# adriente/espm

Measured on AMD Instinct MI355X. Metric: MU iterations/sec, 2048ch x (512*512)px X, k=5 SmoothNMF, higher is better.
Workload: dtype f32; 1 GPU; 2048ch x (512x512)px, k=5, SmoothNMF simplex_H + Laplacian lambda=1, X stored ell, W/H fp32; n=2048, k=5, simplex_H=True, parallelism=single GPU, autotune=True, engine_policy=autotune='auto', as SmoothNMF(max_iter=10000).fit builds it, launch_plan=fused, units handed out dynamically

## Files before the change

### espm_amd/_lib.py

```python
from __future__ import annotations

import ctypes as C
import os

import torch

_HERE = os.path.dirname(os.path.abspath(__file__))
LIB_PATH = os.environ.get("ESPM_MU_LIB", os.path.join(_HERE, "lib", "libespm_mu.so"))

from . import _abi

_HEADER_TEXT = _abi.header_text()
_D = _abi.parse_defines(_HEADER_TEXT)
OK, EINVAL, ENOSOLUTION, EHIP, EUNSUPPORTED = 0, -1, -2, -3, -4
X_F32, X_BF16, X_U8, X_ELL = 0, 1, 2, 3
F64_X_U8, F64_X_BF16, F64_X_F32, F64_X_F64 = (_D["ESPM_F64_X_" + n] for n in ("U8", "BF16", "F32", "F64"))
F64_MAX_K, F64_MAXIT = _D["ESPM_F64_MAX_K"], _D["ESPM_F64_MAXIT"]
F64S_MAX_COUNT, F64S_MAX_N, F64S_WBLOCK = _D["ESPM_F64S_MAX_COUNT"], _D["ESPM_F64S_MAX_N"], _D["ESPM_F64S_WBLOCK"]
SRC_F32, SRC_F64 = 0, 1
LAYOUT_CM, LAYOUT_PM = 0, 1
ABI_VERSION = _D["ESPM_MU_ABI_VERSION"]
XCHG_HANDLE_BYTES = _D["ESPM_XCHG_HANDLE_BYTES"]
ELL_TILE, ELL_PB, ELL_PBITS, ELL_LDS_MAX = _D["ESPM_ELL_TILE"], _D["ESPM_ELL_PB"], _D["ESPM_ELL_PBITS"], _D["ESPM_ELL_LDS_MAX"]
ELL_STREAM_BYTES = _D["ESPM_ELL_STREAM_BYTES"]
ELL_BUCKETS = _D["ESPM_ELL_BUCKETS"]
ELL_HEAVY_MIN, ELL_HEAVY_MAX = _D["ESPM_ELL_HEAVY_MIN"], _D["ESPM_ELL_HEAVY_MAX"]
ELL_UNIT_ROWS, ELL_UNIT_MAX_N, ELL_PAIR_MAX_K = _D["ESPM_ELL_UNIT_ROWS"], _D["ESPM_ELL_UNIT_MAX_N"], _D["ESPM_ELL_PAIR_MAX_K"]
KP, PPAD, NPAD = _D["ESPM_KP"], _D["ESPM_PPAD"], _D["ESPM_NPAD"]
MAX_K = KP
HP_STRIDE, HS_STRIDE, HI_STRIDE = 8 + 2 * KP, 2 * KP, _D["ESPM_HI_STRIDE"]
HS_ROWSUM, HS_MAX = 0, KP
WIDE_MAX_K = 16
WIDEST_MAX_K = 32
TAIL_DEFER, TAIL_RIDE = _D["ESPM_TAIL_DEFER"], _D["ESPM_TAIL_RIDE"]
HI_KLX, HI_REG, HI_LAP, HI_SUMY, HI_BAD, HI_REL_W, HI_REL_H = (_D["ESPM_HI_" + n] for n in ("KLX", "REG", "LAP", "SUMY", "BAD", "REL_W", "REL_H"))

_vp, _i32, _i64, _f32 = C.c_void_p, C.c_int32, C.c_int64, C.c_float


class MUState(C.Structure):
    _fields_ = _abi.parse_struct(_HEADER_TEXT)

    def __init__(self, *args, **kw):
        super().__init__(*args, **kw)
        self.struct_size = C.sizeof(type(self))
        self.abi_version = ABI_VERSION


_SP = C.POINTER(MUState)
SYMBOLS = {
    "espm_mu_version": (C.c_char_p, []),
    "espm_mu_last_error": (C.c_char_p, []),
    "espm_mu_state_size": (C.c_size_t, []),
    "espm_mu_abi_version": (C.c_int, []),
    "espm_mu_state_layout": (C.c_char_p, []),
    "espm_mu_query": (C.c_int, [_SP]),
    "espm_mu_w_update_is_local": (C.c_int, [_SP]),
    "espm_mu_w_update_tail": (C.c_int, [_SP, C.c_int, C.c_int, _vp]),
    "espm_mu_pack_x": (C.c_int, [_vp, C.c_int, C.c_int, _i64, C.c_int, C.c_int, _vp, _vp, C.c_int, C.c_int, C.c_int, C.c_int, C.c_int, _vp]),
    "espm_mu_ell_count": (C.c_int, [_SP, _vp, _vp, _vp, _vp, _vp]),
    "espm_mu_ell_count_hist": (C.c_int, [_SP, _vp, _vp, _vp, _vp, _vp, _vp, _vp]),
    "espm_mu_ell_fill_hist": (C.c_int, [_SP, _vp, _vp, _vp, _vp, _vp, _vp, _vp, _vp, _vp, _vp]),
    "espm_mu_ell_plan": (C.c_int, [_SP, _vp, _vp, _vp, _vp, _vp, _vp, _vp, _vp]),
    "espm_mu_ell_fill": (C.c_int, [_SP, _vp, _vp, _vp, _vp, _vp, _vp, _vp, _vp]),
    "espm_mu_ell_heavy_count": (C.c_int, [_SP, _vp, C.c_int, C.c_int, _i64, _vp, _vp, _vp, _vp]),
    "espm_mu_ell_heavy_fill": (C.c_int, [_SP, _vp, C.c_int, C.c_int, _i64, _vp, _vp, _vp]),
    "espm_mu_hstat": (C.c_int, [_SP, C.c_int, _vp]),
    "espm_mu_build_gw": (C.c_int, [_SP, C.c_int, _vp]),
    "espm_mu_step_h": (C.c_int, [_SP, C.c_int, C.c_int, _vp]),
    "espm_mu_h_finalize": (C.c_int, [_SP, C.c_int, C.c_int, _vp]),
    "espm_mu_loss_only": (C.c_int, [_SP, C.c_int, C.c_int, _vp]),
    "espm_mu_w_accum": (C.c_int, [_SP, _vp]),
    "espm_mu_step_hw": (C.c_int, [_SP, C.c_int, _vp]),
    "espm_mu_fused_applies": (C.c_int, [_SP]),
    "espm_mu_w_reduce": (C.c_int, [_SP, _vp]),
    "espm_mu_w_reduce_finalize": (C.c_int, [_SP, C.c_int, C.c_int, _vp]),
    "espm_mu_w_finish": (C.c_int, [_SP, C.c_int, C.c_int, C.c_int, _vp]),
    "espm_mu_iterate_timed": (C.c_int, [_SP, C.c_int, _vp, _vp, _vp]),
    "espm_mu_iterate": (C.c_int, [_SP, C.c_int, C.c_int, _vp]),
    "espm_mu_shard_record_bytes": (C.c_size_t, [_SP]),
    "espm_mu_shard_pack": (C.c_int, [_SP, C.c_int, _vp, _vp]),
    "espm_mu_shard_combine": (C.c_int, [_SP, _vp, C.c_int, C.c_int, _vp]),
    "espm_mu_shard_combine_finish": (C.c_int, [_SP, _vp, C.c_int, C.c_int, C.c_int, _vp]),
    "espm_mu_w_reduce_finish": (C.c_int, [_SP, C.c_int, C.c_int, C.c_int, _vp]),
    "espm_mu_w_reduce_pack": (C.c_int, [_SP, C.c_int, C.c_int, _vp, _vp]),
    "espm_xchg_create": (C.c_int, [C.c_int, C.c_int, C.c_size_t, C.POINTER(_vp)]),
    "espm_xchg_handle": (C.c_int, [_vp, _vp]),
    "espm_xchg_connect": (C.c_int, [_vp, _vp]),
    "espm_xchg_staging": (_vp, [_vp]),
    "espm_xchg_records": (_vp, [_vp, C.c_int]),
    "espm_xchg_post": (C.c_int, [_vp, C.c_uint32, _vp]),
    "espm_xchg_wait": (C.c_int, [_vp, C.c_uint32, _vp]),
    "espm_xchg_timeouts": (C.c_int, [_vp, C.POINTER(C.c_uint32)]),
    "espm_xchg_set_order": (C.c_int, [_vp, C.c_int]),
    "espm_xchg_order": (C.c_int, [_vp]),
    "espm_xchg_destroy": (C.c_int, [_vp]),
    "espm_mu_shard_exchange_finish": (C.c_int, [_SP, _vp, C.c_uint32, C.c_int, C.c_int, _vp]),
    "espm_mu_iterate_sharded": (C.c_int, [_SP, _vp, C.POINTER(C.c_uint32), C.c_int, C.c_int, _vp]),
    "espm_mu_linesearch_terms": (C.c_int, [_SP, C.c_int, C.c_int, _vp, _vp]),
    "espm_mu_linesearch_terms_sharded": (C.c_int, [_SP, C.c_int, C.c_int, _vp, _vp, _vp, _vp]),
    "espm_surrogate_terms": (C.c_int, [_vp, _vp, C.c_int, C.c_int, C.c_int64, C.c_int, C.c_int, C.c_int, _vp, C.c_int, _vp, _vp]),
    "espm_dichotomy_simplex_acc": (C.c_int, [C.c_double, _vp, _vp, C.c_int, C.c_int, C.c_int, C.c_double, C.c_double, C.c_int, _vp, _vp, _vp]),
    "espm_dichotomy_simplex_pg": (C.c_int, [_vp, C.c_int, C.c_int, C.c_double, C.c_double, C.c_int, _vp, _vp]),
    "espm_mu_l2_step_h": (C.c_int, [_SP, C.c_int, _vp, _vp, C.c_int, _vp]),
    "espm_mu_l2_step_w": (C.c_int, [_SP, C.c_int, _vp, _vp, _vp, C.c_int, _vp]),
    "espm_mu_l2_w_partials": (C.c_int, [_SP, _vp, _vp, C.c_int, _vp]),
    "espm_mu_l2_w_finish": (C.c_int, [_SP, C.c_int, _vp, _vp, _vp]),
    "espm_simplex_root_f32": (C.c_int, [_vp, _vp, C.c_int, C.c_int, C.c_float, C.c_float, C.c_int, C.c_int, _vp, _vp, _vp, _vp]),
    "espm_dichotomy_simplex": (C.c_int, [_vp, _vp, C.c_int, C.c_int, C.c_int, C.c_double, C.c_double, C.c_int, _vp, _vp, _vp]),
    "espm_mu_laplacian": (C.c_int, [_vp, C.c_int, C.c_int, C.c_int, _i64, _vp, _vp]),
    "espm_lu_pl_scratch_bytes": (C.c_size_t, [C.c_int, C.c_int, C.c_int]),
    "espm_lu_pl": (C.c_int, [_vp, C.c_int, C.c_int, C.c_int, _i64, _vp, _vp, C.c_size_t, _vp]),
    "espm_f64_scratch_doubles": (_i64, [C.c_int, C.c_int, C.c_int, _i64]),
    "espm_f64_gw": (C.c_int, [_vp, _vp, C.c_int, C.c_int, C.c_int, C.c_double, _vp, _vp, _vp, _vp]),
    "espm_f64_hstat": (C.c_int, [_vp, C.c_int, C.c_int, C.c_double, _vp, _vp, _vp]),
    "espm_f64_h_pass": (C.c_int, [_vp, C.c_int, C.c_int, C.c_int, C.c_double, _vp, _vp, _vp, _vp, C.c_int, _vp, _vp, C.c_double,
                                  C.c_double, C.c_double, C.c_int, C.c_int, C.c_double, C.c_int, _vp, _vp, _vp, _vp, _vp, _vp, _vp]),
    "espm_f64_bisect": (C.c_int, [_vp, _vp, C.c_int, C.c_int, C.c_double, C.c_double, C.c_int, _vp, _vp, _vp, _vp, _vp]),
    "espm_f64_rel": (C.c_int, [_vp, _vp, _i64, C.c_double, _vp, _vp, _vp]),
    "espm_f64_w_accum": (C.c_int, [_vp, C.c_int, C.c_int, C.c_int, C.c_double, _vp, _vp, C.c_int, C.c_double, _vp, _vp, _vp]),
    "espm_f64_w_finish": (C.c_int, [_vp, _vp, _vp, C.c_int, C.c_int, C.c_int, _vp, _vp, C.c_int, _vp, C.c_int, C.c_double, C.c_double,
                                    C.c_int, _vp, _vp, _vp, _vp]),
    "espm_f64_sparse_scratch_doubles": (_i64, [C.c_int, C.c_int, C.c_int]),
    "espm_f64_sparse_h_pass": (C.c_int, [_vp, _vp, _vp, C.c_int, _vp, C.c_int, C.c_int, C.c_double, _vp, _vp, _vp, _vp, C.c_int, _vp, _vp,
                                         C.c_double, C.c_double, C.c_double, C.c_int, C.c_int, C.c_double, C.c_int, _vp, _vp, _vp, _vp,
                                         _vp, _vp, _vp]),
    "espm_f64_sparse_w_accum": (C.c_int, [_vp, _vp, _vp, _vp, _vp, C.c_int, C.c_int, C.c_double, _vp, _vp, C.c_int, C.c_double, _vp, _vp,
                                          _vp]),
}


class EspmError(RuntimeError):
    """HIP runtime failure or unsupported configuration reported by libespm_mu."""


class LostPeerError(EspmError):
    """A sharded fit's one-shot record exchange gave up waiting for a peer: the iterates since then are not valid
    (MUEngine.history raises it on every rank at the same read-back; the estimator restarts on the collective transport)."""


def _load(path=LIB_PATH):
    if not os.path.exists(path):
        raise ImportError(
            f"{path} is missing: the HIP library is required (no CPU fallback). Build it with "
            "`python -c 'import __graft_entry__ as g; g.build()'` at the repository root.")
    lib = C.CDLL(path)
    for name, (res, args) in SYMBOLS.items():
        fn = getattr(lib, name)
        fn.restype, fn.argtypes = res, args
    theirs, ours = lib.espm_mu_state_layout().decode(), _abi.layout_string(MUState)
    if lib.espm_mu_state_size() != C.sizeof(MUState) or lib.espm_mu_abi_version() != ABI_VERSION or theirs != ours:
        raise ImportError(f"{path} was built from another include/espm_mu.h (ABI {lib.espm_mu_abi_version()} / {lib.espm_mu_state_size()} bytes "
                          f"against {ABI_VERSION} / {C.sizeof(MUState)}): rebuild it with `python -c 'import __graft_entry__ as g; g.build()'`")
    return lib


lib = _load()


def last_error(which=None) -> str:
    return (which or lib).espm_mu_last_error().decode()


def check(rc: int, which=None) -> None:
    if rc == OK:
        return
    msg = last_error(which)
    if rc == ENOSOLUTION:
        raise ValueError(msg)
    if rc == EINVAL:
        raise ValueError(msg)
    if rc == EUNSUPPORTED:
        raise NotImplementedError(msg)
    raise EspmError(msg)


class Variant:

    def __init__(self, handle, kp, min_k, max_k):
        self.lib, self.KP, self.MIN_K, self.MAX_K = handle, kp, min_k, max_k
        self.HP_STRIDE, self.HS_STRIDE, self.HS_MAX = 8 + 2 * kp, 2 * kp, kp

    def check(self, rc):
        check(rc, self.lib)


_narrow = Variant(lib, KP, 1, MAX_K)
_wide = None
_widest = None
WIDE_LIB_PATH = os.environ.get("ESPM_MU_WIDE_LIB", os.path.join(_HERE, "lib", "libespm_mu_wide.so"))
WIDEST_LIB_PATH = os.environ.get("ESPM_MU_WIDEST_LIB", os.path.join(_HERE, "lib", "libespm_mu_wide32.so"))


def variant(k) -> Variant:
    global _wide, _widest
    if k <= MAX_K:
        return _narrow
    if k > WIDEST_MAX_K:
        raise NotImplementedError(f"n_components = {k}: the kernels are built for 1..{WIDEST_MAX_K} components")
    if k <= WIDE_MAX_K:
        if _wide is None:
            _wide = Variant(_load(WIDE_LIB_PATH), 16, MAX_K + 1, WIDE_MAX_K)
        return _wide
    if _widest is None:
        _widest = Variant(_load(WIDEST_LIB_PATH), 32, WIDE_MAX_K + 1, WIDEST_MAX_K)
    return _widest
```

### espm_amd/csrc/mu_api.hip

```cpp
#include <vector>
#include <stdarg.h>
#include <stdio.h>

#include "mu_common.hpp"
#include "mu_xchg.hpp"

namespace espm {

static thread_local char g_err[512] = "";

int set_error(int code, const char* fmt, ...) {
  va_list ap;
  va_start(ap, fmt);
  vsnprintf(g_err, sizeof(g_err), fmt, ap);
  va_end(ap);
  return code;
}

int check_hip(hipError_t e, const char* what) {
  if (e == hipSuccess) return ESPM_OK;
  return set_error(ESPM_EHIP, "%s: %s", what, hipGetErrorString(e));
}

static int roundup(int v, int m) { return (v + m - 1) / m * m; }

#define ESPM_MU_STATE_FIELDS(F) \
  F(struct_size) F(abi_version) F(n) F(m) F(k) F(p) F(nx) F(ny) F(n_pad) F(p_pad) F(x_dtype) F(tile_px) F(nblk_w) \
  F(x_tile) F(n_cm) F(h_variant) F(p_total) F(simplex_h) F(simplex_w) F(grid_mode) F(compute_loss) F(lambda_l) \
  F(sigma_l) F(eps_reg) F(log_shift) F(dicotomy_tol) F(rel_tol) F(xscale) F(gw_floor) F(x_cm) F(x_pm) F(g) \
  F(colsum_g) F(w) F(gw_s) F(colsum_gw) F(gw_a) F(gw_p) F(h) F(h_t) F(mu) F(fixed_h) F(fixed_w) F(simplex_rows) \
  F(halo_top) F(halo_bot) F(hpart) F(hstat) F(a_slab) F(a) F(w_scratch) F(hist) F(hist_len) F(cur) F(it) F(ell_h) \
  F(ell_h_off) F(ell_klc) F(ell_w) F(ell_w_off) F(chan_perm) F(ell_cbits) F(n_cg) F(pix_perm) F(g_t) F(breg_sr_px) \
  F(breg_sr_ch) F(h_rule) F(pg_gamma_w) F(pg_q) F(ell_fill_px) F(ell_fill_num) F(ell_fill_n) F(tail_mode) F(no_fused) \
  F(ell_pb) F(ell_stream) F(ell_hv_n) F(ell_hv_npx) F(ell_hv_ngrp) F(ell_hv_px) F(ell_hv_px_off) F(ell_hv_pm) F(ell_hv_klc) F(ell_hv_kl) \
  F(ell_hv_grp) F(ell_hv_grp_off) F(ell_hv_wm)

static int check_abi(const espm_mu_state* st) {
  ESPM_REQUIRE(st != nullptr, "state is NULL");
  ESPM_REQUIRE(st->struct_size == (uint32_t)sizeof(espm_mu_state) && st->abi_version == (uint32_t)ESPM_MU_ABI_VERSION,
               "espm_mu_state of %u bytes, ABI %u handed to a library built for %zu bytes, ABI %d: the binding's copy of the layout has drifted",
               st->struct_size, st->abi_version, sizeof(espm_mu_state), ESPM_MU_ABI_VERSION);
  return ESPM_OK;
}

static int check_state(const espm_mu_state* st) {
  if (int rc = check_abi(st)) return rc;
  ESPM_REQUIRE(st->n >= 1 && st->p >= 1, "n=%d, p=%d must be >= 1", st->n, st->p);
  if (st->k < ESPM_MIN_K || st->k > ESPM_MAX_K)
    return set_error(ESPM_EUNSUPPORTED, "k=%d: this build supports %d..%d components", st->k, ESPM_MIN_K, ESPM_MAX_K);
  ESPM_REQUIRE(st->n_pad == roundup(st->n, ESPM_NPAD) && st->p_pad == roundup(st->p, ESPM_PPAD),
               "n_pad/p_pad (%d, %d) do not match n, p (%d, %d); call espm_mu_query", st->n_pad, st->p_pad, st->n,
               st->p);
  ESPM_REQUIRE(st->x_dtype >= ESPM_X_F32 && st->x_dtype <= ESPM_X_ELL, "bad x_dtype %d", st->x_dtype);
  if (st->x_dtype == ESPM_X_ELL) {
    ESPM_REQUIRE(st->ell_h && st->ell_h_off && st->ell_klc && st->ell_w && st->ell_w_off && st->chan_perm && st->pix_perm,
                 "the sparse count store needs ell_h, ell_h_off, ell_klc, ell_w, ell_w_off, chan_perm and pix_perm");
    ESPM_REQUIRE((st->tile_px == 64 || st->tile_px == 128 || st->tile_px == 256 || st->tile_px == ESPM_ELL_TILE) &&
                     st->ell_pb == 2 * st->tile_px && st->nblk_w == (st->p + st->ell_pb - 1) / st->ell_pb &&
                     st->n_cg == (st->n + 63) / 64 && st->h_variant == 0,
                 "sparse count store: tile_px must be 64..%d, ell_pb 2 tile_px, nblk_w ceil(p / ell_pb), n_cg ceil(n / 64); call espm_mu_query",
                 ESPM_ELL_TILE);
  }
  ESPM_REQUIRE(st->ell_stream == 0 || (st->ell_stream == 1 && st->x_dtype == ESPM_X_ELL), "ell_stream=%d: 0, or 1 with the sparse store", st->ell_stream);
  ESPM_REQUIRE(st->ell_fill_n >= 0 && (st->ell_fill_n == 0 || (st->x_dtype == ESPM_X_ELL && st->ell_fill_px && st->ell_fill_num)),
               "ell_fill_n=%d needs the sparse store, ell_fill_px and ell_fill_num", st->ell_fill_n);
  ESPM_REQUIRE(st->ell_hv_n >= 0 && (st->ell_hv_n == 0 || (st->x_dtype == ESPM_X_ELL && st->h_rule == 0 && !st->breg_sr_px && st->ell_hv_npx >= 1 &&
                                                          st->ell_hv_npx <= st->ell_hv_n && st->ell_hv_ngrp >= 1 && st->ell_hv_ngrp <= st->ell_hv_n &&
                                                          st->ell_hv_px && st->ell_hv_px_off && st->ell_hv_pm && st->ell_hv_klc && st->ell_hv_kl &&
                                                          st->ell_hv_grp && st->ell_hv_grp_off && st->ell_hv_wm && st->ell_fill_num)),
               "ell_hv_n=%d needs the sparse store with the default H rule, 1 <= ell_hv_npx, ell_hv_ngrp <= ell_hv_n, every ell_hv_* array and "
               "ell_fill_num", st->ell_hv_n);
  ESPM_REQUIRE(st->grid_mode == 0 || (st->nx >= 1 && st->ny >= 1 && st->nx * st->ny == st->p),
               "grid %d x %d does not match p=%d", st->nx, st->ny, st->p);
  ESPM_REQUIRE(st->xscale > 0.f, "xscale must be positive");
  ESPM_REQUIRE(st->n_cm == roundup(st->n, ESPM_NCM), "n_cm must be roundup(n, %d)", ESPM_NCM);
  ESPM_REQUIRE((st->breg_sr_px == nullptr) == (st->breg_sr_ch == nullptr), "breg_sr_px and breg_sr_ch come together");
  ESPM_REQUIRE(!st->breg_sr_px || (st->m == 0 && !st->simplex_w && st->n <= 4096),
               "the Bregman variant is built for G = identity without simplex_W (and n <= 4096)");
  ESPM_REQUIRE(st->h_rule == 0 || ((st->h_rule == 1 || st->h_rule == 2) && !st->breg_sr_px), "h_rule must be 0, 1 or 2 (1, 2 not with the Bregman variant)");
  ESPM_REQUIRE(!(st->pg_gamma_w > 0.f) || (!st->simplex_w && !st->breg_sr_px && (st->m == 0 || (long)st->m * st->k <= 8192)),
               "the projected-gradient W step has no simplex over W (updates.py:368-369), no Bregman variant, and needs M k <= 8192 with a dictionary");
  ESPM_REQUIRE(st->h_variant == 0, "h_variant %d is not built (the matrix-core H-step was retired, DESIGN.md)", st->h_variant);
  ESPM_REQUIRE(st->x_tile >= 64 && ESPM_PPAD % st->x_tile == 0 && st->x_tile % st->tile_px == 0,
               "x_tile=%d must divide %d and be a multiple of tile_px=%d", st->x_tile, ESPM_PPAD, st->tile_px);
  ESPM_REQUIRE(st->m >= 0, "m must be >= 0");
  ESPM_REQUIRE(st->m == 0 || (st->g && st->colsum_g), "m=%d needs g and colsum_g", st->m);
  if (st->log_shift > 0.f && st->simplex_h && (double)st->k * (double)st->log_shift >= 1.0)
    return set_error(ESPM_ENOSOLUTION, "No solution exists! (k * log_shift >= 1)");
  return ESPM_OK;
}

static int nblk_h(const espm_mu_state* st) { return (st->p + st->tile_px - 1) / st->tile_px; }

static int ell_pre_h(const espm_mu_state* st, int src, hipStream_t s) {
  const int ld = st->ell_fill_n + (st->ell_hv_n > 0 ? st->ell_hv_npx : 0);
  if (st->ell_fill_n > 0)
    if (int rc = launch_ell_fill_num(st->gw_s, st->h[src], st->ell_fill_px, st->ell_fill_n, st->n, st->k, st->p_pad, st->log_shift,
                                     st->ell_fill_num, s, ld))
      return rc;
  return st->ell_hv_n > 0 ? launch_ell_hv_h(st, src, ld, s) : ESPM_OK;
}

static int ell_post(const espm_mu_state* st, int hnew, bool w, bool loss, hipStream_t s) {
  if (st->ell_hv_n <= 0) return ESPM_OK;
  if (hnew >= 0) return launch_ell_hv_post(st, st->h[hnew], (size_t)st->p_pad, 1, w, loss, s);
  return launch_ell_hv_post(st, st->h_t, 1, ESPM_KP, w, loss, s);
}

static bool fused_ok(const espm_mu_state* st) {
  return ESPM_MIN_K <= 8 && st->x_dtype == ESPM_X_ELL && st->h_rule == 0 && st->no_fused != 1 &&
         (st->ell_pb >= ESPM_FUSED_MIN_PB || st->nblk_w >= ESPM_FUSED_MIN_BLOCKS || st->no_fused == 3) &&
         fused_ell_lds_bytes(st->n_pad, st->k, st->ell_pb) <= ESPM_ELL_LDS_MAX;
}
static HStepArgs fused_h_args(const espm_mu_state* st, int src) {
  HStepArgs a = make_h_args(st, src, 1);
  a.rec_nb = nblk_h(st);
  return a;
}

}

using namespace espm;

extern "C" {

const char* espm_mu_version(void) { return "espm_mu 0.3 (gfx950)"; }
const char* espm_mu_last_error(void) { return g_err; }

size_t espm_mu_state_size(void) { return sizeof(espm_mu_state); }
int espm_mu_abi_version(void) { return ESPM_MU_ABI_VERSION; }

const char* espm_mu_state_layout(void) {
  static char text[4096];
  static bool done = false;
  if (!done) {
    size_t len = 0;
#define F(name)                                                                                                      \
  len += (size_t)snprintf(text + len, sizeof(text) - len, #name ":%zu:%zu;", offsetof(espm_mu_state, name), \
                          sizeof(((espm_mu_state*)nullptr)->name));
    ESPM_MU_STATE_FIELDS(F)
#undef F
    done = true;
  }
  return text;
}

int espm_mu_query(espm_mu_state* st) {
  if (int rc = check_abi(st)) return rc;
  ESPM_REQUIRE(st->n >= 1 && st->p >= 1, "n=%d, p=%d must be >= 1", st->n, st->p);
  st->n_pad = roundup(st->n, ESPM_NPAD);
  st->p_pad = roundup(st->p, ESPM_PPAD);
  int cus = 256;
  int dev = 0;
  hipDeviceProp_t prop;
  if (hipGetDevice(&dev) == hipSuccess && hipGetDeviceProperties(&prop, dev) == hipSuccess &&
      prop.multiProcessorCount > 0)
    cus = prop.multiProcessorCount;
  const int big = 256;
  st->tile_px = (ESPM_KP <= 16 && (st->p + big - 1) / big >= 2 * cus) ? big : 128;
  st->x_tile = st->tile_px;
  st->n_cm = roundup(st->n, ESPM_NCM);
  st->h_variant = 0;
  st->n_cg = (st->n + 63) / 64;
  st->ell_pb = 0;
  if (st->x_dtype == ESPM_X_ELL) {
    st->tile_px = ESPM_ELL_TILE;
    while (st->tile_px > 64 && (st->p + st->tile_px - 1) / st->tile_px < 2 * cus) st->tile_px /= 2;
    st->x_tile = st->tile_px;
    st->ell_pb = 2 * st->tile_px;
    st->nblk_w = (st->p + st->ell_pb - 1) / st->ell_pb;
    st->ell_cbits = 1;
    while ((1 << st->ell_cbits) < st->n) ++st->ell_cbits;
    if (st->ell_cbits > 14) return set_error(ESPM_EUNSUPPORTED, "sparse count store: n=%d needs more than 14 index bits", st->n);
    return ESPM_OK;
  }
  const int ychunks = (st->x_dtype != ESPM_X_F32 && ESPM_MIN_K <= 8) ? (st->n_pad + 2047) / 2048 : (st->n_pad + 1023) / 1024;
  int target = (2 * cus + ychunks - 1) / ychunks;
  int by_px = (st->p + 15) / 16;
  int nb = target < by_px ? target : by_px;
  if (nb < 1) nb = 1;
  const int ppb = (st->p + nb - 1) / nb;
  st->nblk_w = (st->p + ppb - 1) / ppb;
  return ESPM_OK;
}

int espm_mu_pack_x(const void* src, int src_dtype, int src_layout, int64_t ld, int n, int p, void* x_cm, void* x_pm,
                   int x_dtype, int n_pad, int p_pad, int x_tile, int n_cm, espm_stream_t stream) {
  ESPM_REQUIRE(src && x_pm, "pack_x: NULL pointer");
  ESPM_REQUIRE(n >= 1 && p >= 1 && n_pad == roundup(n, ESPM_NPAD) && p_pad == roundup(p, ESPM_PPAD),
               "pack_x: bad shape n=%d p=%d n_pad=%d p_pad=%d", n, p, n_pad, p_pad);
  ESPM_REQUIRE(src_dtype == ESPM_SRC_F32 || src_dtype == ESPM_SRC_F64, "pack_x: bad src_dtype %d", src_dtype);
  ESPM_REQUIRE(src_layout == ESPM_LAYOUT_CM || src_layout == ESPM_LAYOUT_PM, "pack_x: bad layout %d", src_layout);
  ESPM_REQUIRE(ld >= (src_layout == ESPM_LAYOUT_CM ? p : n), "pack_x: leading dimension too small");
  ESPM_REQUIRE(x_tile >= 64 && ESPM_PPAD % x_tile == 0, "pack_x: x_tile %d must divide %d", x_tile, ESPM_PPAD);
  ESPM_REQUIRE(n_cm == roundup(n, ESPM_NCM), "pack_x: n_cm must be roundup(n, %d)", ESPM_NCM);
  return launch_pack_x(src, src_dtype, src_layout, ld, n, p, x_cm, x_pm, x_dtype, n_pad, p_pad, x_tile, n_cm,
                       static_cast<hipStream_t>(stream));
}

static int check_ell_geometry(const espm_mu_state* st) {
  if (int rc = check_abi(st)) return rc;
  ESPM_REQUIRE(st->x_dtype == ESPM_X_ELL && st->n >= 1 && st->p >= 1 && st->n_pad == roundup(st->n, ESPM_NPAD) &&
                   st->p_pad == roundup(st->p, ESPM_PPAD) && st->n_cg == (st->n + 63) / 64 &&
                   st->ell_pb == 2 * st->tile_px && st->nblk_w == (st->p + st->ell_pb - 1) / st->ell_pb && st->ell_cbits >= 1 &&
                   st->ell_cbits <= 14 && (1 << st->ell_cbits) >= st->n &&
                   (st->tile_px == 64 || st->tile_px == 128 || st->tile_px == 256 || st->tile_px == ESPM_ELL_TILE),
               "sparse store builder: set x_dtype = ESPM_X_ELL and call espm_mu_query first");
  return ESPM_OK;
}

int espm_mu_ell_count_hist(const espm_mu_state* st, const void* x_pm_u8, int32_t* cnt_px, int32_t* cnt_bc, float* ell_klc, uint8_t* bkt_px,
                           uint8_t* bkt_bc, espm_stream_t stream) {
  if (int rc = check_ell_geometry(st)) return rc;
  ESPM_REQUIRE(x_pm_u8 && cnt_px && cnt_bc && ell_klc, "ell_count: NULL pointer");
  ESPM_REQUIRE((bkt_px == nullptr) == (bkt_bc == nullptr), "ell_count: the two histograms come together");
  return launch_ell_count(static_cast<const uint8_t*>(x_pm_u8), st->n, st->n_pad, st->p, st->p_pad, st->ell_cbits, st->n_cg,
                          st->nblk_w, st->ell_pb, cnt_px, cnt_bc, ell_klc, static_cast<hipStream_t>(stream), bkt_px, bkt_bc);
}

int espm_mu_ell_count(const espm_mu_state* st, const void* x_pm_u8, int32_t* cnt_px, int32_t* cnt_bc, float* ell_klc,
                      espm_stream_t stream) {
  return espm_mu_ell_count_hist(st, x_pm_u8, cnt_px, cnt_bc, ell_klc, nullptr, nullptr, stream);
}

int espm_mu_ell_plan(const espm_mu_state* st, const int32_t* cnt_px, const int32_t* cnt_bc, int32_t* chan_perm,
                     int32_t* pix_perm, int32_t* ell_h_off, int32_t* ell_w_off, int64_t* rows, espm_stream_t stream) {
  if (int rc = check_ell_geometry(st)) return rc;
  ESPM_REQUIRE(cnt_px && cnt_bc && chan_perm && pix_perm && ell_h_off && ell_w_off && rows, "ell_plan: NULL pointer");
  return launch_ell_plan(cnt_px, cnt_bc, st->n, st->n_cg, st->nblk_w, st->p_pad, st->tile_px, chan_perm, pix_perm, ell_h_off,
                         ell_w_off, reinterpret_cast<long long*>(rows), static_cast<hipStream_t>(stream));
}

int espm_mu_ell_fill(const espm_mu_state* st, const void* x_pm_u8, const int32_t* chan_perm, const int32_t* pix_perm,
                     const int32_t* ell_h_off, const int32_t* ell_w_off, uint32_t* ell_h, uint32_t* ell_w,
                     espm_stream_t stream) {
  return espm_mu_ell_fill_hist(st, x_pm_u8, chan_perm, pix_perm, ell_h_off, ell_w_off, ell_h, ell_w, nullptr, nullptr, stream);
}

int espm_mu_ell_fill_hist(const espm_mu_state* st, const void* x_pm_u8, const int32_t* chan_perm, const int32_t* pix_perm,
                          const int32_t* ell_h_off, const int32_t* ell_w_off, uint32_t* ell_h, uint32_t* ell_w, const uint8_t* bkt_px,
                          const uint8_t* bkt_bc, espm_stream_t stream) {
  if (int rc = check_ell_geometry(st)) return rc;
  ESPM_REQUIRE((bkt_px == nullptr) == (bkt_bc == nullptr), "ell_fill: the two histograms come together");
  ESPM_REQUIRE(x_pm_u8 && chan_perm && pix_perm && ell_h_off && ell_w_off && ell_h && ell_w, "ell_fill: NULL pointer");
  ESPM_REQUIRE(!st->x_cm || st->n_cm == roundup(st->n, ESPM_NCM), "ell_fill: x_cm is set but n_cm=%d is not n rounded up to %d", st->n_cm, ESPM_NCM);
  return launch_ell_fill(static_cast<const uint8_t*>(x_pm_u8), st->n, st->n_pad, st->p, st->p_pad, st->ell_cbits, st->n_cg,
                         st->nblk_w, st->tile_px, st->ell_pb, chan_perm, pix_perm, ell_h_off, ell_w_off, ell_h, ell_w,
                         static_cast<hipStream_t>(stream), static_cast<const uint8_t*>(st->x_cm), st->n_cm, bkt_px, bkt_bc);
}

int espm_mu_ell_heavy_count(const espm_mu_state* st, const void* x, int src_dtype, int src_layout, int64_t ld, uint8_t* x_pm_u8,
                            uint8_t* x_cm_u8, int32_t* cnt_px, espm_stream_t stream) {
  if (int rc = check_ell_geometry(st)) return rc;
  ESPM_REQUIRE(x && x_pm_u8 && cnt_px, "ell_heavy_count: NULL pointer");
  ESPM_REQUIRE(src_dtype == ESPM_SRC_F32 || src_dtype == ESPM_SRC_F64, "ell_heavy_count: bad src_dtype %d", src_dtype);
  ESPM_REQUIRE(src_layout == ESPM_LAYOUT_CM || src_layout == ESPM_LAYOUT_PM, "ell_heavy_count: bad layout %d", src_layout);
  ESPM_REQUIRE(ld >= (src_layout == ESPM_LAYOUT_CM ? st->p : st->n), "ell_heavy_count: ld=%lld too small", (long long)ld);
  ESPM_REQUIRE(!x_cm_u8 || st->n_cm == roundup(st->n, ESPM_NCM), "ell_heavy_count: x_cm is set but n_cm=%d is not n rounded up to %d", st->n_cm, ESPM_NCM);
  return launch_ell_hv_count(x, src_dtype, src_layout, ld, st->n, st->p, st->n_pad, st->n_cm, x_pm_u8, x_cm_u8, cnt_px,
                             static_cast<hipStream_t>(stream));
}

int espm_mu_ell_heavy_fill(const espm_mu_state* st, const void* x, int src_dtype, int src_layout, int64_t ld, const int32_t* px_off,
                           int32_t* hv_pm, espm_stream_t stream) {
  if (int rc = check_ell_geometry(st)) return rc;
  ESPM_REQUIRE(x && px_off && hv_pm, "ell_heavy_fill: NULL pointer");
  ESPM_REQUIRE(src_dtype == ESPM_SRC_F32 || src_dtype == ESPM_SRC_F64, "ell_heavy_fill: bad src_dtype %d", src_dtype);
  ESPM_REQUIRE(src_layout == ESPM_LAYOUT_CM || src_layout == ESPM_LAYOUT_PM, "ell_heavy_fill: bad layout %d", src_layout);
  ESPM_REQUIRE(ld >= (src_layout == ESPM_LAYOUT_CM ? st->p : st->n), "ell_heavy_fill: ld=%lld too small", (long long)ld);
  return launch_ell_hv_fill(x, src_dtype, src_layout, ld, st->n, st->p, px_off, hv_pm, static_cast<hipStream_t>(stream));
}

int espm_mu_hstat(const espm_mu_state* st, int which, espm_stream_t stream) {
  if (int rc = check_state(st)) return rc;
  ESPM_REQUIRE(which == 0 || which == 1, "which must be 0/1");
  return launch_hstat(st->h[which], st->k, st->p, st->p_pad, st->hstat[which], static_cast<hipStream_t>(stream));
}

static bool w_update_is_local(const espm_mu_state* st) {
  return st->m == 0 && !st->simplex_w && st->n >= 64 && st->w_scratch != nullptr;
}
static bool w_simplex_split(const espm_mu_state* st) {
  return st->m == 0 && st->simplex_w && !st->simplex_rows && !st->breg_sr_ch && !(st->pg_gamma_w > 0.f) && st->n >= 64 &&
         st->w_scratch != nullptr && st->n_pad % 32 == 0 && st->no_fused != 1;
}
static double* simplex_bparts(const espm_mu_state* st) {
  return reinterpret_cast<double*>(st->w_scratch) + 3 * (size_t)st->k * ((st->n_pad + 31) / 32);
}
static int w_simplex_reduce_update(const espm_mu_state* st, int src, int slot, const HFinalizeArgs* fin, WTailArgs* defer_tail, hipStream_t s);

static WFinishArgs finish_args(const espm_mu_state* st, int src, int hsrc, int slot, int update_w) {
  WFinishArgs a;
  a.g = st->m > 0 ? st->g : nullptr;
  a.g_t = st->m > 0 ? st->g_t : nullptr;
  a.colsum_g = st->colsum_g;
  a.w_old = st->w[src];
  a.w_new = update_w ? st->w[1 - src] : st->w[src];
  a.a = st->a;
  a.hstat = st->hstat[hsrc];
  a.fixed_w = st->fixed_w;
  a.simplex_rows = st->simplex_rows;
  a.scratch = st->w_scratch;
  a.breg_sr = st->breg_sr_ch;
  a.pg_gamma_w = st->pg_gamma_w;
  a.pg_q = (st->pg_q && st->pg_gamma_w > 0.f && slot >= 0) ? st->pg_q + 2 * (size_t)slot + 1 : nullptr;
  a.gw_s = st->gw_s;
  a.colsum_gw = st->colsum_gw;
  a.gw_a = nullptr;
  a.gw_p = nullptr;
  a.n_cm = st->n_cm;
  a.hist_slot = (slot >= 0 && st->hist) ? st->hist + (size_t)slot * ESPM_HI_STRIDE : nullptr;
  a.n = st->n;
  a.m = st->m;
  a.k = st->k;
  a.n_pad = st->n_pad;
  a.simplex_w = st->simplex_w;
  a.update_w = update_w;
  a.log_shift = st->log_shift;
  a.tol = ESPM_W_DICOTOMY_TOL;
  a.rel_tol = st->rel_tol;
  a.xscale = st->xscale;
  a.gw_floor = st->gw_floor;
  return a;
}

static int w_simplex_reduce_update(const espm_mu_state* st, int src, int slot, const HFinalizeArgs* fin, WTailArgs* defer_tail, hipStream_t s) {
  if (st->log_shift > 0.f && (double)st->n * (double)st->log_shift >= 1.0)
    return set_error(ESPM_ENOSOLUTION, "No solution exists! (rows * log_shift >= 1)");
  double* bparts = simplex_bparts(st);
  if (int rc = launch_w_reduce(st->a_slab, st->a, st->nblk_w, st->k * st->n_pad, fin, s, st->w[src], bparts, st->n, st->k, st->n_pad)) return rc;
  return launch_w_simplex_update(finish_args(st, src, 1 - src, slot + 1, 1), st->a, bparts, (double)ESPM_W_DICOTOMY_TOL, s, defer_tail);
}

int espm_mu_build_gw(const espm_mu_state* st, int which, espm_stream_t stream) {
  if (int rc = check_state(st)) return rc;
  ESPM_REQUIRE(which == 0 || which == 1, "which must be 0/1");
  return launch_w_finish(finish_args(st, which, 0, -1, 0), static_cast<hipStream_t>(stream));
}

int espm_mu_step_h(const espm_mu_state* st, int src, int write_h, espm_stream_t stream) {
  if (int rc = check_state(st)) return rc;
  ESPM_REQUIRE(src == 0 || src == 1, "src must be 0/1");
  if (st->x_dtype == ESPM_X_ELL) {
    HStepArgs a = make_h_args(st, src, write_h);
    if (st->tail_mode & ESPM_TAIL_RIDE) {
      ESPM_REQUIRE(st->it >= 1 && (w_update_is_local(st) || w_simplex_split(st)), "tail_mode: no local W update produced state %d", st->it);
      a.tail = make_w_tail_args(finish_args(st, 1 - src, src, st->it, 1));
      a.cs_parts = a.tail.parts;
      a.cs_nbk = a.tail.nbk;
      a.tail_on = 1;
    }
    if (int rc = ell_pre_h(st, src, static_cast<hipStream_t>(stream))) return rc;
    if (int rc = launch_h_ell(a, nblk_h(st), static_cast<hipStream_t>(stream))) return rc;
    return ell_post(st, -1, false, true, static_cast<hipStream_t>(stream));
  }
  return dispatch_h_step(make_h_args(st, src, write_h), st->x_dtype, st->tile_px, nblk_h(st),
                         static_cast<hipStream_t>(stream));
}

static HFinalizeArgs finalize_args(const espm_mu_state* st, int src, int slot, bool write_hstat) {
  HFinalizeArgs a;
  a.hpart = st->hpart;
  a.colsum_gw = st->colsum_gw;
  a.hstat_in = st->hstat[src];
  a.hstat_out = write_hstat ? st->hstat[1 - src] : nullptr;
  a.hist_slot = st->hist + (size_t)slot * ESPM_HI_STRIDE;
  a.nblk = nblk_h(st);
  a.k = st->k;
  a.compute_loss = st->compute_loss;
  a.have_prev = st->it > 0;
  a.xscale = st->xscale;
  a.pg_q = (st->pg_q && st->h_rule == 2 && write_hstat) ? st->pg_q + 2 * (size_t)slot : nullptr;
  return a;
}

int espm_mu_h_finalize(const espm_mu_state* st, int src, int slot, espm_stream_t stream) {
  if (int rc = check_state(st)) return rc;
  ESPM_REQUIRE(src == 0 || src == 1, "src must be 0/1");
  ESPM_REQUIRE(slot >= 0 && slot < st->hist_len, "history slot %d outside [0, %d)", slot, st->hist_len);
  return launch_h_finalize(finalize_args(st, src, slot, true), static_cast<hipStream_t>(stream));
}

static int h_finalize_loss_only(const espm_mu_state* st, int src, int slot, hipStream_t stream) {
  return launch_h_finalize(finalize_args(st, src, slot, false), stream);
}

int espm_mu_loss_only(const espm_mu_state* st, int src, int slot, espm_stream_t stream) {
  if (int rc = check_state(st)) return rc;
  ESPM_REQUIRE(slot >= 0 && slot < st->hist_len, "history slot %d outside [0, %d)", slot, st->hist_len);
  if (int rc = espm_mu_step_h(st, src, 0, stream)) return rc;
  return h_finalize_loss_only(st, src, slot, static_cast<hipStream_t>(stream));
}

int espm_mu_w_accum(const espm_mu_state* st, espm_stream_t stream) {
  if (int rc = check_state(st)) return rc;
  ESPM_REQUIRE(st->nblk_w >= 1, "nblk_w must be >= 1");
  if (st->x_dtype == ESPM_X_ELL) {
    if (int rc = launch_w_ell(make_w_args(st), st->k, st->nblk_w, static_cast<hipStream_t>(stream))) return rc;
    return ell_post(st, -1, true, false, static_cast<hipStream_t>(stream));
  }
  return dispatch_w_accum(make_w_args(st), st->k, st->x_dtype, st->nblk_w, static_cast<hipStream_t>(stream));
}

int espm_mu_fused_applies(const espm_mu_state* st) {
  if (check_state(st)) return 0;
  return fused_ok(st) ? 1 : 0;
}

int espm_mu_step_hw(const espm_mu_state* st, int src, espm_stream_t stream) {
  if (int rc = check_state(st)) return rc;
  ESPM_REQUIRE(src == 0 || src == 1, "src must be 0/1");
  if (!fused_ok(st)) {
    if (int rc = espm_mu_step_h(st, src, 1, stream)) return rc;
    return espm_mu_w_accum(st, stream);
  }
  hipStream_t s = static_cast<hipStream_t>(stream);
  HStepArgs a = fused_h_args(st, src);
  if (st->tail_mode & ESPM_TAIL_RIDE) {
    ESPM_REQUIRE(st->it >= 1 && (w_update_is_local(st) || w_simplex_split(st)), "tail_mode: no local W update produced state %d", st->it);
    a.tail = make_w_tail_args(finish_args(st, 1 - src, src, st->it, 1));
    a.cs_parts = a.tail.parts;
    a.cs_nbk = a.tail.nbk;
    a.tail_on = 1;
  }
  if (int rc = ell_pre_h(st, src, s)) return rc;
  if (int rc = launch_fused_ell(a, make_w_args(st), st->nblk_w, s, st->no_fused == 2, st->ell_stream)) return rc;
  return ell_post(st, 1 - src, true, true, s);
}

int espm_mu_w_reduce(const espm_mu_state* st, espm_stream_t stream) {
  if (int rc = check_state(st)) return rc;
  return launch_w_reduce(st->a_slab, st->a, st->nblk_w, st->k * st->n_pad, nullptr, static_cast<hipStream_t>(stream));
}

int espm_mu_w_reduce_finalize(const espm_mu_state* st, int src, int slot, espm_stream_t stream) {
  if (int rc = check_state(st)) return rc;
  ESPM_REQUIRE(src == 0 || src == 1, "src must be 0/1");
  ESPM_REQUIRE(slot >= 0 && slot < st->hist_len, "history slot %d outside [0, %d)", slot, st->hist_len);
  const HFinalizeArgs fin = finalize_args(st, src, slot, true);
  return launch_w_reduce(st->a_slab, st->a, st->nblk_w, st->k * st->n_pad, &fin, static_cast<hipStream_t>(stream));
}

int espm_mu_w_finish(const espm_mu_state* st, int src, int hsrc, int slot, espm_stream_t stream) {
  if (int rc = check_state(st)) return rc;
  ESPM_REQUIRE((src == 0 || src == 1) && (hsrc == 0 || hsrc == 1), "src/hsrc must be 0/1");
  ESPM_REQUIRE(slot < st->hist_len, "history slot %d outside [0, %d)", slot, st->hist_len);
  if (st->simplex_w && st->log_shift > 0.f) {
    const double rows = st->m > 0 ? st->m : st->n;
    if (!st->simplex_rows && rows * (double)st->log_shift >= 1.0)
      return set_error(ESPM_ENOSOLUTION, "No solution exists! (rows * log_shift >= 1)");
  }
  return launch_w_finish(finish_args(st, src, hsrc, slot, 1), static_cast<hipStream_t>(stream));
}

int espm_mu_w_reduce_finish(const espm_mu_state* st, int src, int slot, int with_finalize, espm_stream_t stream) {
  if (int rc = check_state(st)) return rc;
  ESPM_REQUIRE(src == 0 || src == 1, "src must be 0/1");
  ESPM_REQUIRE(slot >= 0 && slot + 1 < st->hist_len, "history slot %d + 1 outside [0, %d)", slot, st->hist_len);
  hipStream_t s = static_cast<hipStream_t>(stream);
  const HFinalizeArgs fin = finalize_args(st, src, slot, true);
  WTailArgs left_out;
  if (w_update_is_local(st)) {
    return launch_w_reduce_update(finish_args(st, src, 1 - src, slot + 1, 1), st->a_slab, (size_t)st->k * st->n_pad * sizeof(float),
                                  st->nblk_w, st->a, with_finalize ? st->hpart : nullptr, nblk_h(st), with_finalize ? nullptr : st->hstat[1 - src],
                                  0, nullptr, with_finalize ? &fin : nullptr, s,
                                  (st->tail_mode & ESPM_TAIL_DEFER) ? &left_out : nullptr);
  }
  if (w_simplex_split(st))
    return w_simplex_reduce_update(st, src, slot, with_finalize ? &fin : nullptr, (st->tail_mode & ESPM_TAIL_DEFER) ? &left_out : nullptr, s);
  if (int rc = launch_w_reduce(st->a_slab, st->a, st->nblk_w, st->k * st->n_pad, with_finalize ? &fin : nullptr, s)) return rc;
  return espm_mu_w_finish(st, src, 1 - src, slot + 1, stream);
}

int espm_mu_shard_combine_finish(const espm_mu_state* st, const void* records, int world, int src, int slot,
                                 espm_stream_t stream) {
  if (int rc = check_state(st)) return rc;
  ESPM_REQUIRE(records && world >= 1 && (src == 0 || src == 1), "shard_combine_finish: bad arguments");
  ESPM_REQUIRE(slot >= 0 && slot + 1 < st->hist_len, "history slot %d + 1 outside [0, %d)", slot, st->hist_len);
  WTailArgs left_out;
  if (w_update_is_local(st)) {
    return launch_w_reduce_update(finish_args(st, src, 1 - src, slot + 1, 1), records, espm_mu_shard_record_bytes(st), world, st->a,
                                  nullptr, 0, nullptr, (size_t)st->k * st->n_pad * sizeof(float), st->hstat[1 - src], nullptr,
                                  static_cast<hipStream_t>(stream), (st->tail_mode & ESPM_TAIL_DEFER) ? &left_out : nullptr);
  }
  if (w_simplex_split(st)) {
    if (st->log_shift > 0.f && (double)st->n * (double)st->log_shift >= 1.0)
      return set_error(ESPM_ENOSOLUTION, "No solution exists! (rows * log_shift >= 1)");
    double* bparts = simplex_bparts(st);
    if (int rc = launch_shard_combine(records, world, espm_mu_shard_record_bytes(st), st->k * st->n_pad, st->a, st->hstat[1 - src],
                                      static_cast<hipStream_t>(stream), st->w[src], bparts, st->n, st->k, st->n_pad))
      return rc;
    return launch_w_simplex_update(finish_args(st, src, 1 - src, slot + 1, 1), st->a, bparts, (double)ESPM_W_DICOTOMY_TOL,
                                   static_cast<hipStream_t>(stream), (st->tail_mode & ESPM_TAIL_DEFER) ? &left_out : nullptr);
  }
  if (int rc = espm_mu_shard_combine(st, records, world, 1 - src, stream)) return rc;
  return espm_mu_w_finish(st, src, 1 - src, slot + 1, stream);
}

int espm_mu_w_update_is_local(const espm_mu_state* st) {
  if (check_state(st)) return 0;
  return w_update_is_local(st) ? 1 : 0;
}

int espm_mu_w_update_tail(const espm_mu_state* st, int src, int slot, espm_stream_t stream) {
  if (int rc = check_state(st)) return rc;
  ESPM_REQUIRE((src == 0 || src == 1) && slot >= 0 && slot + 1 < st->hist_len && (w_update_is_local(st) || w_simplex_split(st)), "w_update_tail: bad arguments");
  return launch_w_update_tail(make_w_tail_args(finish_args(st, src, 1 - src, slot + 1, 1)), static_cast<hipStream_t>(stream));
}

static int iterate_impl(espm_mu_state* st, int n_iter, int final_loss, espm_stream_t stream, hipEvent_t* ev);

int espm_mu_iterate(espm_mu_state* st, int n_iter, int final_loss, espm_stream_t stream) { return iterate_impl(st, n_iter, final_loss, stream, nullptr); }

int espm_mu_iterate_timed(espm_mu_state* st, int n_iter, float* first_ms, float* rest_ms, espm_stream_t stream) {
  if (int rc = check_state(st)) return rc;
  ESPM_REQUIRE(n_iter >= 1 && n_iter <= 4096 && first_ms && rest_ms, "iterate_timed: 1..4096 iterations, two host arrays of that length");
  hipStream_t s = static_cast<hipStream_t>(stream);
  std::vector<hipEvent_t> ev((size_t)3 * n_iter, nullptr);
  int rc = ESPM_OK;
  for (size_t i = 0; i < ev.size() && !rc; ++i) rc = check_hip(hipEventCreate(&ev[i]), "iterate_timed: event");
  if (!rc) rc = iterate_impl(st, n_iter, 0, stream, ev.data());
  if (!rc) rc = check_hip(hipStreamSynchronize(s), "iterate_timed: synchronize");
  for (int i = 0; i < n_iter && !rc; ++i) {
    rc = check_hip(hipEventElapsedTime(first_ms + i, ev[3 * i], ev[3 * i + 1]), "iterate_timed: elapsed");
    if (!rc) rc = check_hip(hipEventElapsedTime(rest_ms + i, ev[3 * i + 1], ev[3 * i + 2]), "iterate_timed: elapsed");
  }
  for (hipEvent_t e : ev)
    if (e) (void)hipEventDestroy(e);
  return rc;
}

static int iterate_impl(espm_mu_state* st, int n_iter, int final_loss, espm_stream_t stream, hipEvent_t* ev) {
  if (int rc = check_state(st)) return rc;
  ESPM_REQUIRE(n_iter >= 0, "n_iter must be >= 0");
  ESPM_REQUIRE(st->it + n_iter < st->hist_len, "history too short: it=%d + %d >= %d", st->it, n_iter, st->hist_len);
  hipStream_t s = static_cast<hipStream_t>(stream);
  const bool split = w_simplex_split(st);
  const bool defer = st->x_dtype == ESPM_X_ELL && (w_update_is_local(st) || split) && !(st->pg_q && st->pg_gamma_w > 0.f);
  const bool fused = fused_ok(st);
  bool pending = false;
  WTailArgs tail;
  for (int i = 0; i < n_iter; ++i) {
    const int cur = st->cur, slot = st->it;
    int rc;
    if (defer) {
      HStepArgs a = fused ? fused_h_args(st, cur) : make_h_args(st, cur, 1);
      if ((rc = ell_pre_h(st, cur, s))) return rc;
      if (pending) {
        a.cs_parts = tail.parts;
        a.cs_nbk = tail.nbk;
        a.tail_on = 1;
        a.tail = tail;
      }
      if (ev && (rc = check_hip(hipEventRecord(ev[3 * i], s), "iterate_timed: record"))) return rc;
      if (fused) {
        if ((rc = launch_fused_ell(a, make_w_args(st), st->nblk_w, s, st->no_fused == 2, st->ell_stream))) return rc;
        if ((rc = ell_post(st, 1 - cur, true, true, s))) return rc;
        if (ev && (rc = check_hip(hipEventRecord(ev[3 * i + 1], s), "iterate_timed: record"))) return rc;
      } else {
        if ((rc = launch_h_ell(a, nblk_h(st), s))) return rc;
        if ((rc = ell_post(st, -1, false, true, s))) return rc;
        if (ev && (rc = check_hip(hipEventRecord(ev[3 * i + 1], s), "iterate_timed: record"))) return rc;
        if ((rc = espm_mu_w_accum(st, stream))) return rc;
      }
      const HFinalizeArgs fin = finalize_args(st, cur, slot, true);
      if (split) {
        if ((rc = w_simplex_reduce_update(st, cur, slot, &fin, &tail, s))) return rc;
      } else if ((rc = launch_w_reduce_update(finish_args(st, cur, 1 - cur, slot + 1, 1), st->a_slab, (size_t)st->k * st->n_pad * sizeof(float),
                                              st->nblk_w, st->a, st->hpart, nblk_h(st), nullptr, 0, nullptr, &fin, s, &tail))) {
        return rc;
      }
      if (ev && (rc = check_hip(hipEventRecord(ev[3 * i + 2], s), "iterate_timed: record"))) return rc;
      pending = true;
    } else {
      if (ev && (rc = check_hip(hipEventRecord(ev[3 * i], s), "iterate_timed: record"))) return rc;
      if ((rc = espm_mu_step_hw(st, cur, stream))) return rc;
      if (ev && (rc = check_hip(hipEventRecord(ev[3 * i + 1], s), "iterate_timed: record"))) return rc;
      if ((rc = espm_mu_w_reduce_finish(st, cur, slot, 1, stream))) return rc;
      if (ev && (rc = check_hip(hipEventRecord(ev[3 * i + 2], s), "iterate_timed: record"))) return rc;
    }
    st->cur = 1 - cur;
    st->it = slot + 1;
  }
  if (pending)
    if (int rc = launch_w_update_tail(tail, s)) return rc;
  if (final_loss) return espm_mu_loss_only(st, st->cur, st->it, stream);
  return ESPM_OK;
}

int espm_mu_shard_exchange_finish(const espm_mu_state* st, espm_xchg* x, uint32_t seq, int src, int slot, espm_stream_t stream) {
  if (int rc = check_state(st)) return rc;
  ESPM_REQUIRE(x && (src == 0 || src == 1), "shard_exchange_finish: bad arguments");
  ESPM_REQUIRE(slot >= 0 && slot + 1 < st->hist_len, "history slot %d + 1 outside [0, %d)", slot, st->hist_len);
  ESPM_REQUIRE(x->record_bytes == espm_mu_shard_record_bytes(st), "shard_exchange_finish: the exchange was created for records of %zu bytes, the state packs %zu",
               x->record_bytes, espm_mu_shard_record_bytes(st));
  if (!w_update_is_local(st) && st->no_fused != 1) {
    const WFinishArgs f = finish_args(st, src, 1 - src, slot + 1, 1);
    if (w_gsplit_applies(f)) {
      HFinalizeArgs fin = finalize_args(st, src, slot, true);
      double* local = reinterpret_cast<double*>(x->mailbox + (size_t)(seq & 1u) * x->world * x->record_bytes + (size_t)x->rank * x->record_bytes +
                                                (size_t)st->k * st->n_pad * 4);
      fin.hstat_out = local;
      if (int rc = launch_w_reduce(st->a_slab, st->a, st->nblk_w, st->k * st->n_pad, &fin, static_cast<hipStream_t>(stream))) return rc;
      const int with_halo_g = st->grid_mode && st->lambda_l != 0.f;
      return launch_w_gxchg_update(f, x, seq, local, st->hstat[1 - src], st->h[1 - src], st->nx, st->ny, st->p_pad, with_halo_g,
                                   static_cast<hipStream_t>(stream));
    }
  }
  if (w_simplex_split(st) && nblk_h(st) > 0) {
    if (st->log_shift > 0.f && (double)st->n * (double)st->log_shift >= 1.0)
      return set_error(ESPM_ENOSOLUTION, "No solution exists! (rows * log_shift >= 1)");
    const HFinalizeArgs fin = finalize_args(st, src, slot, true);
    WTailArgs left_out;
    const int with_halo = st->grid_mode && st->lambda_l != 0.f;
    double* bparts = simplex_bparts(st);
    if (int rc = launch_w_exchange_update(finish_args(st, src, 1 - src, slot + 1, 1), st->a_slab, (size_t)st->k * st->n_pad * sizeof(float), st->nblk_w,
                                          st->a, st->hstat[1 - src], fin, x, seq, st->h[1 - src], st->nx, st->ny, st->p_pad, with_halo,
                                          static_cast<hipStream_t>(stream), nullptr, bparts))
      return rc;
    return launch_w_simplex_update(finish_args(st, src, 1 - src, slot + 1, 1), st->a, bparts, (double)ESPM_W_DICOTOMY_TOL,
                                   static_cast<hipStream_t>(stream), (st->tail_mode & ESPM_TAIL_DEFER) ? &left_out : nullptr);
  }
  if (!w_update_is_local(st) || st->no_fused == 1) {
    if (int rc = espm_mu_w_reduce_pack(st, src, slot, x->staging, stream)) return rc;
    if (int rc = espm_xchg_post(x, seq, stream)) return rc;
    if (int rc = espm_xchg_wait(x, seq, stream)) return rc;
    return espm_mu_shard_combine_finish(st, espm_xchg_records(x, (int)(seq & 1u)), x->world, src, slot, stream);
  }
  const HFinalizeArgs fin = finalize_args(st, src, slot, true);
  WTailArgs left_out;
  const int with_halo = st->grid_mode && st->lambda_l != 0.f;
  return launch_w_exchange_update(finish_args(st, src, 1 - src, slot + 1, 1), st->a_slab, (size_t)st->k * st->n_pad * sizeof(float), st->nblk_w,
                                  st->a, st->hstat[1 - src], fin, x, seq, st->h[1 - src], st->nx, st->ny, st->p_pad, with_halo,
                                  static_cast<hipStream_t>(stream), (st->tail_mode & ESPM_TAIL_DEFER) ? &left_out : nullptr);
}

int espm_mu_iterate_sharded(espm_mu_state* st, espm_xchg* x, uint32_t* seq, int n_iter, int final_loss, espm_stream_t stream) {
  if (int rc = check_state(st)) return rc;
  ESPM_REQUIRE(x && seq && n_iter >= 0, "iterate_sharded: bad arguments");
  ESPM_REQUIRE(st->it + n_iter < st->hist_len, "history too short: it=%d + %d >= %d", st->it, n_iter, st->hist_len);
  ESPM_REQUIRE(x->record_bytes == espm_mu_shard_record_bytes(st), "iterate_sharded: the exchange was created for records of %zu bytes, the state packs %zu",
               x->record_bytes, espm_mu_shard_record_bytes(st));
  const bool defer = st->x_dtype == ESPM_X_ELL && (w_update_is_local(st) || w_simplex_split(st)) && !(st->pg_q && st->pg_gamma_w > 0.f);
  const bool with_halo = st->grid_mode && st->lambda_l != 0.f;
  const size_t off_top = (size_t)st->k * st->n_pad * 4 + ESPM_HS_STRIDE * 8, off_bot = off_top + (size_t)st->k * (st->ny > 0 ? st->ny : 0) * 4;
  bool pending = (st->tail_mode & ESPM_TAIL_RIDE) != 0;
  int rc = ESPM_OK;
  for (int i = 0; i < n_iter && !rc; ++i) {
    const int cur = st->cur, slot = st->it;
    st->tail_mode = pending ? ESPM_TAIL_RIDE : 0;
    rc = espm_mu_step_hw(st, cur, stream);
    st->tail_mode = 0;
    const uint32_t s = ++*seq;
    const unsigned char* recs = static_cast<const unsigned char*>(espm_xchg_records(x, (int)(s & 1u)));
    st->tail_mode = defer ? ESPM_TAIL_DEFER : 0;
    if (!rc) rc = espm_mu_shard_exchange_finish(st, x, s, cur, slot, stream);
    st->tail_mode = 0;
    pending = defer;
    if (with_halo) {
      st->halo_top = x->rank > 0 ? reinterpret_cast<const float*>(recs + (size_t)(x->rank - 1) * x->record_bytes + off_bot) : nullptr;
      st->halo_bot = x->rank < x->world - 1 ? reinterpret_cast<const float*>(recs + (size_t)(x->rank + 1) * x->record_bytes + off_top) : nullptr;
    }
    st->cur = 1 - cur;
    st->it = slot + 1;
  }
  if (rc) return rc;
  if (pending)
    if ((rc = espm_mu_w_update_tail(st, 1 - st->cur, st->it - 1, stream))) return rc;
  if (final_loss) return espm_mu_loss_only(st, st->cur, st->it, stream);
  return ESPM_OK;
}

int espm_dichotomy_simplex(const double* num, const double* den, int k, int p, int den_cols, double log_shift,
                           double tol, int maxit, double* nu_out, int32_t* status_out, espm_stream_t stream) {
  ESPM_REQUIRE(num && den && nu_out && status_out, "dichotomy: NULL pointer");
  ESPM_REQUIRE(k >= 1 && p >= 1 && (den_cols == 1 || den_cols == p), "dichotomy: bad shape k=%d p=%d den_cols=%d", k,
               p, den_cols);
  if (log_shift > 0 && (double)k * log_shift >= 1.0) return set_error(ESPM_ENOSOLUTION, "No solution exists!");
  return launch_dichotomy(num, den, k, p, den_cols, log_shift, tol, maxit, nu_out, status_out,
                          static_cast<hipStream_t>(stream));
}

int espm_simplex_root_f32(const float* num, const float* den, int k, int p, float log_shift, float tol, int maxit, int fast_exit,
                          float* delta_out, float* e_out, int32_t* status_out, espm_stream_t stream) {
  ESPM_REQUIRE(num && den && delta_out && e_out && status_out, "simplex_root_f32: NULL pointer");
  ESPM_REQUIRE(k >= ESPM_MIN_K && k <= ESPM_MAX_K && p >= 1, "simplex_root_f32: bad shape k=%d p=%d (this library: %d..%d components)", k, p, ESPM_MIN_K, ESPM_MAX_K);
  if (log_shift > 0 && (double)k * log_shift >= 1.0) return set_error(ESPM_ENOSOLUTION, "No solution exists!");
  return launch_simplex_root_f32(num, den, k, p, log_shift, tol, maxit, fast_exit, delta_out, e_out, status_out, static_cast<hipStream_t>(stream));
}

int espm_surrogate_terms(const float* h_old, const float* h_new, int k, int p, int64_t ld, int nx, int ny, int grid_mode, double* part,
                         int part_doubles, double* out, espm_stream_t stream) {
  ESPM_REQUIRE(h_old && h_new && part && out && k >= 1 && k <= ESPM_KP && p >= 1 && ld >= p, "surrogate_terms: bad arguments");
  ESPM_REQUIRE(!grid_mode || (nx >= 1 && ny >= 1 && (int64_t)nx * ny == p), "surrogate_terms: grid %d x %d does not match p=%d", nx, ny, p);
  ESPM_REQUIRE(part_doubles >= (4 + ESPM_KP) * ((p + 511) / 512), "surrogate_terms: scratch of %d doubles is too small", part_doubles);
  return launch_linesearch_terms(h_old, h_new, k, p, (int)ld, nx, ny, grid_mode, nullptr, nullptr, nullptr, nullptr, part, out,
                                 static_cast<hipStream_t>(stream));
}

// ... 121 lines not shown
```

### espm_amd/csrc/mu_common.hpp

```cpp
#pragma once
#include <hip/hip_runtime.h>
#include <stdint.h>

#include "espm_mu.h"

namespace espm {

constexpr int KP = ESPM_KP;
static_assert(KP == 8 || KP == 16 || KP == 32, "ESPM_KP: 8, 16 or 32");
static_assert(ESPM_MIN_K >= 1 && ESPM_MAX_K <= KP && ESPM_MIN_K <= ESPM_MAX_K, "ESPM_MIN_K .. ESPM_MAX_K must fit the stride");

#if ESPM_MIN_K <= 8
#define ESPM_K_CASES(X) X(1) X(2) X(3) X(4) X(5) X(6) X(7) X(8)
#elif ESPM_MIN_K <= 16
#define ESPM_K_CASES(X) X(9) X(10) X(11) X(12) X(13) X(14) X(15) X(16)
#else
#define ESPM_K_CASES(X) X(17) X(18) X(19) X(20) X(21) X(22) X(23) X(24) X(25) X(26) X(27) X(28) X(29) X(30) X(31) X(32)
#endif

__device__ __forceinline__ void store_row_kp(float* dst, const float (&row)[KP]) {
#pragma unroll
  for (int q = 0; q < KP / 4; ++q)
    reinterpret_cast<float4*>(dst)[q] = make_float4(row[4 * q], row[4 * q + 1], row[4 * q + 2], row[4 * q + 3]);
}
// ... 391 lines not shown
      y[u] = i < mk ? a.w_old[i] : 1.f;
    }
#pragma unroll
    for (int u = 0; u < 8; ++u) rel = fmaxf(rel, fabsf(x[u] - y[u]) / (x[u] + shift));
  }
  double r1[1] = {(double)rel};
  block_reduce<1, 0>(r1, scratch);
  if (tid == 0) a.hist_slot[ESPM_HI_REL_W] = r1[0];
}

template <typename T>
__device__ __forceinline__ T fast_rcp(T x);
template <>
__device__ __forceinline__ float fast_rcp<float>(float x) { return __builtin_amdgcn_rcpf(x); }
template <>
__device__ __forceinline__ double fast_rcp<double>(double x) { return 1.0 / x; }

template <typename T, int K>
__device__ __forceinline__ bool simplex_root(const T (&num)[K], const T (&den)[K], int k, T eps, T tol,
                                             int maxit, T& delta, T (&e)[K], bool fast_exit = false) {
  T nmax = 0, dmin_all = INFINITY, dstar = INFINITY, nsum = 0;
  bool ok = true;
#pragma unroll
  for (int i = 0; i < K; ++i) {
    if (i < k) {
      ok = ok && (num[i] >= 0) && (den[i] >= 0);
      if (num[i] > 0) dstar = fmin(dstar, den[i]);
      nmax = fmax(nmax, num[i]);
      dmin_all = fmin(dmin_all, den[i]);
      nsum += num[i];
    }
  }
  ok = ok && (nsum > 0) && (nsum < (T)INFINITY);
  if (!ok) {
    delta = 0;
#pragma unroll
    for (int i = 0; i < K; ++i) e[i] = i < k ? den[i] : (T)1;
    return false;
  }
  T lo = 0;
#pragma unroll
  for (int i = 0; i < K; ++i) {
    e[i] = i < k ? den[i] - dstar : (T)1;
    if (i < k && num[i] > 0) lo = fmax(lo, num[i] / 2 - e[i]);
  }
  T hi = (T)(2 * k) * nmax + (dstar - dmin_all);
  T x = fmax(lo, fmin(dstar, hi)), dxold = hi - lo;
  const bool fast = fast_exit && (T)(4 * K) * eps <= (T)1e-3 * tol;
  for (int it = 0; it < maxit; ++it) {
    T f = -1, fp = 0, fpp = 0;
#pragma unroll
    for (int i = 0; i < K; ++i) {
      if (i < k) {
        T inv = fast_rcp<T>(x + e[i]);
        T t = num[i] > 0 ? num[i] * inv : (T)0;
        if (t > eps) {
          const T u = t * inv;
          f += t;
          fp -= u;
          if (fast_exit) fpp += u * inv;
        } else {
          f += eps;
        }
      }
    }
    if (fabs(f) <= tol) break;
    if (f > 0) lo = x; else hi = x;
    T dx = fp < 0 ? -f * fast_rcp<T>(fp) : (T)0;
    T xn = x + dx;
    bool newton = true;
    if (!(fp < 0) || !(xn > lo && xn < hi) || fabs(dx) > (T)0.5 * fabs(dxold)) {
      dx = (hi - lo) / 2;
      xn = lo + dx;
      newton = false;
    }
    dxold = dx;
    if (xn == x) break;
    x = xn;
    if (fast && newton && (T)4 * f * f * fpp <= tol * fp * fp) break;
  }
  delta = x;
  return true;
}

__device__ __forceinline__ float hq_root(float s, float q) {
  const float r = __builtin_amdgcn_sqrtf(fmaf(s, s, q));
  return s >= 0.f ? q * __builtin_amdgcn_rcpf(r + s) : r - s;
}
template <int K>
__device__ __forceinline__ bool simplex_root_hq(float a, const float (&b)[K], const float (&c)[K], float eps, int maxit, float& nu) {
  bool ok = a > 0.f;
  float bmax = -INFINITY, bsum = 0.f;
#pragma unroll
  for (int i = 0; i < K; ++i) {
    ok = ok && c[i] >= 0.f && b[i] == b[i];
    bmax = fmaxf(bmax, b[i] * b[i] * __builtin_amdgcn_rcpf(a) + 2.f * a + 2.f * (b[i] + c[i]));
    bsum += b[i];
  }
  nu = 0.f;
  if (!ok) return false;
  float hi = (float)K * bmax * 1.5f + 1e-3f;
  float lo = -(2.f * a + bsum) * (1.1f / (float)K) - 1e-3f;
  const float target = 2.f * a, floor_g = 2.f * a * eps;
  float x = fminf(fmaxf(0.f, lo), hi), dxold = hi - lo;
  for (int it = 0; it < maxit; ++it) {
    float f = -target, fp = 0.f;
#pragma unroll
    for (int i = 0; i < K; ++i) {
      const float s = b[i] + x, q = 4.f * a * c[i];
      const float r = __builtin_amdgcn_sqrtf(fmaf(s, s, q));
      const float g = s >= 0.f ? q * __builtin_amdgcn_rcpf(r + s) : r - s;
      if (g > floor_g) {
        f += g;
        fp -= g * __builtin_amdgcn_rcpf(r);
      } else {
        f += floor_g;
      }
    }
    if (fabsf(f) <= 4e-7f * target) break;
    if (f > 0.f) lo = x; else hi = x;
    float dx = fp < 0.f ? -f * __builtin_amdgcn_rcpf(fp) : 0.f;
    float xn = x + dx;
    if (!(fp < 0.f) || !(xn > lo && xn < hi) || fabsf(dx) > 0.5f * fabsf(dxold)) {
      dx = (hi - lo) * 0.5f;
      xn = lo + dx;
    }
    dxold = dx;
    if (xn == x) break;
    x = xn;
  }
  nu = x;
  return true;
}

__device__ __forceinline__ float stencil_hl(const float* hrow, const float* halo_top, const float* halo_bot,
                                            int q, int nx, int ny, float hc) {
  const int i = q / ny, j = q - i * ny;
  float acc = 0.f;
  int deg = 0;
  if (j > 0) { acc += hrow[q - 1]; ++deg; }
  if (j < ny - 1) { acc += hrow[q + 1]; ++deg; }
  if (i > 0) { acc += hrow[q - ny]; ++deg; }
  else if (halo_top) { acc += halo_top[j]; ++deg; }
  if (i < nx - 1) { acc += hrow[q + ny]; ++deg; }
  else if (halo_bot) { acc += halo_bot[j]; ++deg; }
  return (float)deg * hc - acc;
}

struct HStepArgs {
  const void* x_cm;
  const void* x_pm;
  int mfma;
  const float* gw_s;
  const double* colsum_gw;
  const float* h_in;
  float* h_out;
  float* h_t;
  const float* mu;
  const float* fixed_h;
  const float* halo_top;
  const float* halo_bot;
  const double* hstat_in;
  double* hpart;
  int n, k, p, nx, ny, p_pad;
  int x_tile;
  int n_cm;
  const void* gw_a;
  const float* gw_p;
  int simplex_h, grid_mode, compute_loss, write_h;
  int have_prev;
  float lambda_l, sigma_l, eps_reg, log_shift, tol, xscale, rel_tol;
  double inv_count;
  const uint32_t* ell;
  const int32_t* ell_off;
  const float* ell_klc;
  const int32_t* ell_pix;
  int ell_bits, n_pad;
  int ell_tp;
  const float* l2_m;
  const float* breg_sr;
  int h_rule;
  const float* fill_num;
  int fill_n;
  const double* cs_parts;
  int cs_nbk, cs_lds_off, tail_on;
  WTailArgs tail;
  int rec_nb;
};
struct HFinalizeArgs {
  const double* hpart;
  const double* colsum_gw;
  const double* hstat_in;
  double* hstat_out;
  double* hist_slot;
  int nblk, k, compute_loss, have_prev;
  float xscale;
  double* pg_q;
};
__host__ __device__ inline int ell_pbits(int pb) {
  int b = 6;
  while ((1 << b) < pb) ++b;
  return b;
}
struct WAccumArgs {
  const void* x_pm;
  const void* x_cm;
  int x_tile, n_cm, p_pad, mfma;
  const float* gw_s;
  const float* h_t;
  float* a_slab;
  int n_pad, p, ppb;
  const uint32_t* ell;
  const int32_t* ell_off;
  const int32_t* chan_perm;
  int n_cg;
  int pb, pbits;
  int l2;
};
struct WFinishArgs {
  const float* g;
  const float* g_t;
  const float* colsum_g;
  const float* w_old;
  float* w_new;
  const float* a;
  const double* hstat;
  const float* fixed_w;
  const int32_t* simplex_rows;
  float* scratch;
  const float* breg_sr;
  float pg_gamma_w;
  double* pg_q;
  float* gw_s;
  double* colsum_gw;
  void* gw_a;
  float* gw_p;
  double* hist_slot;
  int n, m, k, n_pad, n_cm, simplex_w, update_w;
  float log_shift, tol, rel_tol, xscale, gw_floor;
};


__device__ __forceinline__ void h_finalize_body(const HFinalizeArgs& a, double* scratch) {
  constexpr int NV = ESPM_HP_NSCALAR + 2 * KP + 1;
  constexpr int V_RELH = 4 + KP, V_MAX = 5 + KP, V_RELW = 5 + 2 * KP;
  double v[NV];
#pragma unroll
  for (int i = 0; i < NV; ++i) v[i] = 0.0;
  v[V_RELW] = -1.0;
  const size_t nb = a.nblk;
  constexpr int U = KP > 8 ? 1 : 4;
  for (int b0 = threadIdx.x; b0 < a.nblk; b0 += U * 256) {
    double t[U][ESPM_HP_RELH + 1], tw[U];
#pragma unroll
    for (int u = 0; u < U; ++u) {
      const int b = b0 + u * 256;
#pragma unroll
      for (int i = 0; i <= ESPM_HP_RELH; ++i) t[u][i] = b < a.nblk ? a.hpart[i * nb + b] : 0.0;
      tw[u] = b < a.nblk ? a.hpart[(size_t)ESPM_HP_RELW * nb + b] : -1.0;
    }
#pragma unroll
    for (int u = 0; u < U; ++u) {
#pragma unroll
      for (int i = 0; i < 4 + KP; ++i) v[i] += t[u][i];
      v[V_RELH] = fmax(v[V_RELH], t[u][ESPM_HP_RELH]);
      v[V_RELW] = fmax(v[V_RELW], tw[u]);
#pragma unroll
      for (int i = 0; i < KP; ++i) v[V_MAX + i] = fmax(v[V_MAX + i], t[u][ESPM_HP_MAX + i]);
    }
  }
  block_reduce<NV, 4 + KP>(v, scratch);
  if (a.pg_q) {
    double q1[1] = {0.0};
    for (int b = threadIdx.x; b < a.nblk; b += 256) q1[0] += a.hpart[(size_t)ESPM_HP_PGQ * nb + b];
    block_reduce<1, 1>(q1, scratch);
    if (threadIdx.x == 0) *a.pg_q = q1[0];
  }
  if (threadIdx.x == 0) {
    double sumy = 0.0;
    for (int kk = 0; kk < a.k; ++kk) sumy += a.colsum_gw[kk] * a.hstat_in[ESPM_HS_ROWSUM + kk];
    if (a.compute_loss) a.hist_slot[ESPM_HI_KLX] = (double)a.xscale * 0.6931471805599453 * v[ESPM_HP_KL];
    a.hist_slot[ESPM_HI_REG] = v[ESPM_HP_REG];
    a.hist_slot[ESPM_HI_LAP] = v[ESPM_HP_LAP];
    a.hist_slot[ESPM_HI_SUMY] = sumy;
    a.hist_slot[ESPM_HI_BAD] = v[ESPM_HP_BAD];
    if (a.have_prev) a.hist_slot[ESPM_HI_REL_H] = v[V_RELH];
    if (v[V_RELW] >= 0.0) a.hist_slot[ESPM_HI_REL_W] = v[V_RELW];
    if (a.hstat_out) {
      for (int kk = 0; kk < KP; ++kk) {
        a.hstat_out[ESPM_HS_ROWSUM + kk] = v[ESPM_HP_ROWSUM + kk];
        a.hstat_out[ESPM_HS_MAX + kk] = v[V_MAX + kk];
      }
    }
  }
}

constexpr int H_FINALIZE_NV = ESPM_HP_NSCALAR + 2 * KP + 1;
constexpr int H_FINALIZE_JOBS = H_FINALIZE_NV + 2;
__device__ __forceinline__ void h_finalize_one(const HFinalizeArgs& a, int job, double* scratch) {
  constexpr int NV = H_FINALIZE_NV, V_RELH = 4 + KP, V_MAX = 5 + KP, V_RELW = 5 + 2 * KP;
  const size_t nb = a.nblk;
  if (job == NV) {
    if (threadIdx.x == 0) {
      double sumy = 0.0;
      for (int kk = 0; kk < a.k; ++kk) sumy += a.colsum_gw[kk] * a.hstat_in[ESPM_HS_ROWSUM + kk];
      a.hist_slot[ESPM_HI_SUMY] = sumy;
    }
    return;
  }
  if (job == NV + 1) {
    if (a.pg_q) {
      double q1[1] = {0.0};
      for (int b = threadIdx.x; b < a.nblk; b += 256) q1[0] += a.hpart[(size_t)ESPM_HP_PGQ * nb + b];
      block_reduce<1, 1>(q1, scratch);
      if (threadIdx.x == 0) *a.pg_q = q1[0];
    }
    return;
  }
  const bool is_sum = job < 4 + KP;
  const int field = is_sum ? job : (job == V_RELH ? ESPM_HP_RELH : (job == V_RELW ? ESPM_HP_RELW : ESPM_HP_MAX + (job - V_MAX)));
  double v[1] = {job == V_RELW ? -1.0 : 0.0};
  for (int b = threadIdx.x; b < a.nblk; b += 256) {
    const double t = a.hpart[(size_t)field * nb + b];
    v[0] = is_sum ? v[0] + t : fmax(v[0], t);
  }
  if (is_sum)
    block_reduce<1, 1>(v, scratch);
  else
    block_reduce<1, 0>(v, scratch);
  if (threadIdx.x != 0) return;
  if (job == ESPM_HP_KL) {
    if (a.compute_loss) a.hist_slot[ESPM_HI_KLX] = (double)a.xscale * 0.6931471805599453 * v[0];
  } else if (job == ESPM_HP_REG) {
    a.hist_slot[ESPM_HI_REG] = v[0];
  } else if (job == ESPM_HP_LAP) {
    a.hist_slot[ESPM_HI_LAP] = v[0];
  } else if (job == ESPM_HP_BAD) {
    a.hist_slot[ESPM_HI_BAD] = v[0];
  } else if (is_sum) {
    if (a.hstat_out) a.hstat_out[ESPM_HS_ROWSUM + (job - ESPM_HP_ROWSUM)] = v[0];
  } else if (job == V_RELH) {
    if (a.have_prev) a.hist_slot[ESPM_HI_REL_H] = v[0];
  } else if (job == V_RELW) {
    if (v[0] >= 0.0) a.hist_slot[ESPM_HI_REL_W] = v[0];
  } else {
    if (a.hstat_out) a.hstat_out[ESPM_HS_MAX + (job - V_MAX)] = v[0];
  }
}


inline HStepArgs make_h_args(const espm_mu_state* st, int src, int write_h) {
  HStepArgs a;
  a.x_cm = st->x_cm;
  a.x_pm = st->x_pm;
  a.mfma = st->no_fused == 0;
  a.gw_s = st->gw_s;
  a.colsum_gw = st->colsum_gw;
  a.h_in = st->h[src];
  a.h_out = st->h[1 - src];
  a.h_t = st->h_t;
  a.mu = st->mu;
  a.fixed_h = st->fixed_h;
  a.halo_top = st->grid_mode ? st->halo_top : nullptr;
  a.halo_bot = st->grid_mode ? st->halo_bot : nullptr;
  a.hstat_in = st->hstat[src];
  a.hpart = st->hpart;
  a.n = st->n;
  a.k = st->k;
  a.p = st->p;
  a.nx = st->nx;
  a.ny = st->ny;
  a.p_pad = st->p_pad;
  a.x_tile = st->x_tile;
  a.n_cm = st->n_cm;
  a.gw_a = st->gw_a;
  a.gw_p = st->gw_p;
  a.simplex_h = st->simplex_h;
  a.grid_mode = st->grid_mode;
  a.compute_loss = st->compute_loss;
  a.write_h = write_h;
  a.have_prev = st->it > 0;
  a.rel_tol = st->rel_tol;
  a.inv_count = 1.0 / ((double)st->k * (double)(st->p_total > 0 ? st->p_total : st->p));
  a.lambda_l = st->lambda_l;
  a.sigma_l = st->sigma_l;
  a.eps_reg = st->eps_reg;
  a.log_shift = st->log_shift;
  a.tol = st->dicotomy_tol;
  a.xscale = st->xscale;
  a.ell = st->ell_h;
  a.ell_off = st->ell_h_off;
  a.ell_klc = st->ell_klc;
  a.ell_pix = st->pix_perm;
  a.ell_bits = st->ell_cbits;
  a.ell_tp = st->tile_px;
  a.l2_m = nullptr;
  a.breg_sr = st->breg_sr_px;
  a.h_rule = st->h_rule;
  a.fill_n = st->ell_fill_n + (st->ell_hv_n > 0 ? st->ell_hv_npx : 0);
  a.fill_num = (st->x_dtype == ESPM_X_ELL && a.fill_n > 0) ? st->ell_fill_num : nullptr;
  a.cs_parts = nullptr;
  a.cs_nbk = a.cs_lds_off = a.tail_on = 0;
  a.rec_nb = 0;
  a.n_pad = st->n_pad;
  return a;
}

inline WAccumArgs make_w_args(const espm_mu_state* st) {
  WAccumArgs a;
  a.x_pm = st->x_pm;
  a.x_cm = st->x_cm;
  a.x_tile = st->x_tile;
  a.n_cm = st->n_cm;
  a.p_pad = st->p_pad;
  a.mfma = st->no_fused == 0;
  a.gw_s = st->gw_s;
  a.h_t = st->h_t;
  a.a_slab = st->a_slab;
  a.n_pad = st->n_pad;
  a.p = st->p;
  a.ppb = (st->p + st->nblk_w - 1) / st->nblk_w;
  a.ell = st->ell_w;
  a.ell_off = st->ell_w_off;
  a.chan_perm = st->chan_perm;
  a.n_cg = st->n_cg;
  a.pb = st->ell_pb > 0 ? st->ell_pb : ESPM_ELL_PB;
  a.pbits = ell_pbits(a.pb);
  a.l2 = 0;
  return a;
}

int dispatch_h_step(const HStepArgs& args, int x_dtype, int tile_px, int nblk, hipStream_t stream);
int launch_h_finalize(const HFinalizeArgs& args, hipStream_t stream);
int launch_h_ell(const HStepArgs& args, int nblk, hipStream_t stream);
int launch_fused_ell(const HStepArgs& h, const WAccumArgs& w, int nblk, hipStream_t stream, int static_units = 0, int stream_lists = 0);
size_t fused_ell_lds_bytes(int n_pad, int k, int pb);
int launch_ell_count(const uint8_t* x_pm, int n, int n_pad, int p, int p_pad, int cbits, int n_cg, int nblk, int pb,
                     int32_t* cnt_px, int32_t* cnt_bc, float* klc, hipStream_t stream, uint8_t* bkt_px = nullptr, uint8_t* bkt_bc = nullptr);
int launch_ell_plan(const int32_t* cnt_px, const int32_t* cnt_bc, int n, int n_cg, int nblk, int p_pad, int win,
                    int32_t* chan_perm, int32_t* pix_perm, int32_t* h_off, int32_t* w_off, long long* rows, hipStream_t stream);
int launch_ell_fill(const uint8_t* x_pm, int n, int n_pad, int p, int p_pad, int cbits, int n_cg, int nblk, int win, int pb,
                    const int32_t* chan_perm, const int32_t* pix_perm, const int32_t* h_off, const int32_t* w_off,
                    uint32_t* ell_h, uint32_t* ell_w, hipStream_t stream, const uint8_t* x_cm = nullptr, int n_cm = 0, const uint8_t* bkt_px = nullptr,
                    const uint8_t* bkt_bc = nullptr);
int launch_w_ell(const WAccumArgs& args, int k, int nblk, hipStream_t stream);
int launch_ell_fill_num(const float* gw_s, const float* h_in, const int32_t* fill_px, int fill_n, int n, int k, int p_pad, float fill,
                        float* fill_num, hipStream_t stream, int ld = 0);
int launch_ell_hv_count(const void* x, int src_dtype, int layout, int64_t ld, int n, int p, int n_pad, int n_cm, uint8_t* x8, uint8_t* x8c,
                        int32_t* cnt_px, hipStream_t stream);
int launch_ell_hv_fill(const void* x, int src_dtype, int layout, int64_t ld, int n, int p, const int32_t* px_off, int32_t* hv_pm,
                       hipStream_t stream);
int launch_ell_hv_h(const espm_mu_state* st, int src, int ld, hipStream_t stream);
int launch_ell_hv_post(const espm_mu_state* st, const float* h, size_t hs_k, size_t hs_p, bool w, bool loss, hipStream_t stream);
int dispatch_w_accum(const WAccumArgs& args, int k, int x_dtype, int nblk, hipStream_t stream);
int launch_w_reduce(const float* slab, float* out, int nblk, int total, const HFinalizeArgs* fused_finalize,
                    hipStream_t stream, const float* bw_old = nullptr, double* bparts = nullptr, int n = 0, int k = 0, int n_pad = 0);
int launch_w_simplex_update(const WFinishArgs& f, float* a_inout, const double* bparts, double tol, hipStream_t stream, WTailArgs* defer_tail);
int launch_w_reduce_pack(const float* slab, int nblk, int k, int n_pad, const HFinalizeArgs& fin_to_record,
                         const float* h_new, int nx, int ny, int p_pad, int with_halo, void* rec, hipStream_t stream);
int launch_w_finish(const WFinishArgs& args, hipStream_t stream);
int launch_gram(const float* m, int rows, int k, double* part, int part_cap, float* out, hipStream_t stream);
int launch_w_finish_l2(const float* a, int n, int n_pad, int m, int k, const float* g, const float* gtg, const float* hh, const float* w_old,
                       float* w_new, const float* fixed_w, float log_shift, hipStream_t stream);
int launch_w_reduce_update(const WFinishArgs& f, const void* src, size_t src_stride, int nsrc, float* a_out,
                           const double* hpart, int nblk_h, const double* hstat_rs, size_t rec_hstat_off, double* hstat_out,
                           const HFinalizeArgs* fused_finalize, hipStream_t stream, WTailArgs* defer_tail = nullptr);
int launch_w_update_tail(const WTailArgs& t, hipStream_t stream);
int launch_w_exchange_update(const WFinishArgs& f, const void* slabs, size_t slab_stride, int nslab, float* a_out, double* hstat_out,
                             const HFinalizeArgs& fin, const struct ::espm_xchg* xc, unsigned int seq, const float* h_new, int nx, int ny,
                             int p_pad, int with_halo, hipStream_t stream, WTailArgs* defer_tail, double* simplex_bparts = nullptr);
bool w_gsplit_applies(const WFinishArgs& args);
int launch_w_gxchg_update(const WFinishArgs& f, const struct ::espm_xchg* xc, unsigned int seq, const double* hstat_local, double* hstat_out,
                          const float* h_new, int nx, int ny, int p_pad, int with_halo, hipStream_t stream);
WTailArgs make_w_tail_args(const WFinishArgs& f);
int launch_pack_x(const void* src, int src_dtype, int src_layout, int64_t ld, int n, int p, void* x_cm, void* x_pm,
                  int x_dtype, int n_pad, int p_pad, int x_tile, int n_cm, hipStream_t stream);
int launch_hstat(const float* h, int k, int p, int p_pad, double* out, hipStream_t stream);
int launch_dichotomy(const double* num, const double* den, int k, int p, int den_cols, double eps, double tol,
                     int maxit, double* nu_out, int32_t* status, hipStream_t stream);
int launch_shard_pack(const float* a, const double* hstat, const float* h_new, int k, int n_pad, int nx, int ny,
                      int p_pad, int with_halo, void* rec, hipStream_t stream);
int launch_shard_combine(const void* recs, int world, size_t stride, int na, float* a_out, double* hstat_out,
                         hipStream_t stream, const float* bw_old = nullptr, double* bparts = nullptr, int n = 0, int k = 0, int n_pad = 0);
int launch_simplex_root_f32(const float* num, const float* den, int k, int p, float eps, float tol, int maxit, int fast_exit, float* delta_out,
                            float* e_out, int32_t* status, hipStream_t stream);
int launch_dichotomy_acc(double a, const double* b, const double* c, int k, int p, int b_cols, double eps, double tol, int maxit,
                         double* nu_out, int32_t* status, hipStream_t stream);
int launch_dichotomy_pg(const double* a, int k, int p, double eps, double tol, int maxit, double* nu_out, hipStream_t stream);
int launch_laplacian(const float* h, int k, int nx, int ny, int64_t ld, float* out, hipStream_t stream);
int launch_linesearch_terms(const float* h_old, const float* h_new, int k, int p, int p_pad, int nx, int ny, int grid_mode,
                            const float* old_top, const float* old_bot, const float* new_top, const float* new_bot,
                            double* part, double* out, hipStream_t stream);

}
```

### espm_amd/csrc/mu_fused.hip

```cpp
#include <stdlib.h>

#include "mu_fused_kernel.hpp"

#ifndef ESPM_ELL_UNR_H
#define ESPM_ELL_UNR_H 4
#endif
#ifndef ESPM_FUSED_SMALL_UNR_H
#define ESPM_FUSED_SMALL_UNR_H ESPM_ELL_UNR_H
#endif
#ifndef ESPM_FUSED_SMALL_UNR_W
#define ESPM_FUSED_SMALL_UNR_W ESPM_ELL_UNR_W
#endif
#ifndef ESPM_ELL_UNR_W
#define ESPM_ELL_UNR_W 4
#endif

#ifndef ESPM_FUSED_FULL_PERM_LDS
#define ESPM_FUSED_FULL_PERM_LDS 0
#endif
#define ESPM_FUSED_LDS_LIMIT (160 * 1024)
#ifndef ESPM_FUSED_SMALL_SEGS_DEFAULT
#define ESPM_FUSED_SMALL_SEGS_DEFAULT 0
#endif

// ... 8 lines not shown
    const char* env = getenv("ESPM_FUSED_PLAIN");
    return !(env && env[0] == '0');
  }();
  return on;
}
static int fused_env_small_segs() {
  static const int want = [] {
    const char* env = getenv("ESPM_FUSED_SMALL_SEGS");
    return env ? atoi(env) : ESPM_FUSED_SMALL_SEGS_DEFAULT;
  }();
  return want;
}

int launch_fused_plain(const FusedArgs& args, int k, bool loss, bool full, int nblk, size_t lds_bytes, hipStream_t stream);
int launch_fused_plain_stream(const FusedArgs& args, int k, bool loss, bool full, int nblk, size_t lds_bytes, hipStream_t stream);
#ifdef ESPM_PHASE_CLOCK
int phase_buffer_plain(unsigned long long* p);
int phase_buffer_plain_stream(unsigned long long* p);
#endif

#if ESPM_MIN_K <= 8
template <int K>
static int launch_fused_k(const FusedArgs& args_in, int nblk, hipStream_t stream) {
  FusedArgs args = args_in;
  const int pb = args.w.pb;
  const int tab_rows = args.h.n_pad > pb ? args.h.n_pad : pb;
  const bool full = pb == ESPM_ELL_PB;
  ESPM_REQUIRE(K <= 4 || tab_rows <= FixTab<K>::MAX_ROWS, "fused half-steps: a table of %d rows, at most %d from 5 components on", tab_rows, FixTab<K>::MAX_ROWS);
  const size_t red = (size_t)(ESPM_ELL_WTHREADS / 64 + 1) * (ESPM_HP_NSCALAR + 2 * K + 1) * sizeof(double);
  const size_t tail_scratch = (size_t)((ESPM_ELL_WTHREADS / 64 + 1) * (KP + 1) + 1) * sizeof(double);
  const size_t red_own = (size_t)(ESPM_ELL_WTHREADS / 64) * (ESPM_HP_NSCALAR + 2 * K + 1) * sizeof(double);
  auto part_of = [&](int segs) {
    size_t part = (size_t)segs * FusedGeom<K>::PROWS * pb * sizeof(float);
    if (red > part) part = red;
    if (tail_scratch > part) part = tail_scratch;
    return part;
  };
  size_t bytes = 0;
  auto layout = [&](size_t part, bool red_in_table) {
    const size_t tab_bytes = FixTab<K>::bytes(tab_rows);
    bytes = tab_bytes + part;
    args.cnt_lds_off = (int)bytes;
    bytes += 16 + ESPM_FUSED_MAX_UNITS * sizeof(float);
    args.meta_lds_off = (int)bytes;
    bytes += (size_t)(3 * (pb / 64) + 2 * args.w.n_cg + 1 + 3) / 4 * 16;
    args.perm_lds_off = (int)bytes;
    const size_t perm_bytes = (size_t)(pb + 64 * args.w.n_cg) * sizeof(int);
    args.perm_lds = pb != ESPM_ELL_PB || (ESPM_FUSED_FULL_PERM_LDS && bytes + perm_bytes + KP * sizeof(double) <= ESPM_FUSED_LDS_LIMIT);
    if (args.perm_lds) bytes += perm_bytes;
    args.red_lds_off = -1;
    const size_t hp_tab = FixTab<K>::bytes(pb);
    if (ESPM_FUSED_RED_ONE_BARRIER && red_in_table && hp_tab + red_own <= tab_bytes) {
      args.red_lds_off = (int)hp_tab;
    } else if (ESPM_FUSED_RED_ONE_BARRIER && bytes + red_own + 2 * KP * sizeof(double) <= ESPM_FUSED_LDS_LIMIT) {
      bytes = (bytes + 7) / 8 * 8;
      args.red_lds_off = (int)bytes;
      bytes += red_own;
    }
    if (args.h.cs_parts) {
      bytes = (bytes + 7) / 8 * 8;
      args.h.cs_lds_off = (int)bytes;
      bytes += 2 * KP * sizeof(double);
    }
  };
  args.h_segs = full ? FusedGeom<K>::S : ESPM_ELL_PB / pb;
  size_t part0 = part_of(args.h_segs);
  bool red_in_table = false;
  if (full) {
    for (int segs = FusedGeom<K>::S_MAX; segs > FusedGeom<K>::S; --segs) {
      bool ok = false;
      for (int rit = 0; rit < 2 && !ok; ++rit) {
        layout(part_of(segs), rit != 0);
        ok = bytes <= ESPM_FUSED_LDS_LIMIT && args.red_lds_off >= 0;
        if (ok) red_in_table = rit != 0;
      }
      if (ok) {
        args.h_segs = segs;
        part0 = part_of(segs);
        break;
      }
    }
  }
  const size_t slab = (size_t)K * args.w.n_pad * sizeof(float);
  args.slab_lds = 0;
  layout(part0, red_in_table);
  args.w_split = 0;
  if (ESPM_FUSED_SLAB_LDS && args.w.n_pad % 4 == 0) {
    if (slab > part0) {
      layout(slab, false);
      if (bytes > ESPM_FUSED_LDS_LIMIT || args.red_lds_off < 0) {
        layout(part0, red_in_table);
      } else {
        args.slab_lds = 1;
        const int want = fused_env_small_segs();
        const int fit = (int)(slab / ((size_t)FusedGeom<K>::PROWS * pb * sizeof(float)));
        int segs = want > 0 ? want : args.h_segs;
        if (segs > fit) segs = fit;
        if (segs > ESPM_FUSED_MAX_SEGS) segs = ESPM_FUSED_MAX_SEGS;
        if (segs > args.h_segs) args.h_segs = segs;
      }
    } else {
      args.slab_lds = args.red_lds_off >= 0;
      args.w_split = ESPM_FUSED_W_SPLIT && args.slab_lds && pb == ESPM_ELL_PB && 2 * slab <= part0;
    }
  }
  if (args.h.tail_on && !args.h.tail.pg_q) args.h.tail_on = 2;
  if (bytes > ((args.perm_lds && pb == ESPM_ELL_PB) || args.red_lds_off >= 0 ? ESPM_FUSED_LDS_LIMIT : ESPM_ELL_LDS_MAX))
    return set_error(ESPM_EUNSUPPORTED, "fused half-steps: %zu bytes of LDS exceed %d", bytes, ESPM_ELL_LDS_MAX);
  {
    const int NT = ESPM_ELL_WTHREADS;
    const int n_perm = args.perm_lds ? pb + 64 * args.w.n_cg : 0, n_woff = 2 * args.w.n_cg + 1;
    const bool staged_ok = args.h.n_pad <= 4 * NT && n_perm <= 4 * NT && n_woff <= NT && args.h.cs_nbk <= 64 && 2 * K <= NT / 64;
    const bool plain = ESPM_FUSED_PLAIN && fused_env_plain() && !args.h.fixed_h && !args.h.fill_num && !args.h.breg_sr && !args.h.l2_m &&
                       args.h.simplex_h && args.h.lambda_l != 0.f && args.h.grid_mode && args.h.have_prev && args.h.write_h && args.h.h_rule == 0 &&
                       args.h.tail_on != 1 && !args.static_units && args.slab_lds && !args.w_split && args.red_lds_off >= 0 && staged_ok &&
                       (args.perm_lds != 0) == (pb != ESPM_ELL_PB) && ESPM_FUSED_SMALL_THREADS == ESPM_ELL_WTHREADS;
    if (plain && args.stream_lists && pb == ESPM_ELL_PB) return launch_fused_plain_stream(args, K, args.h.compute_loss != 0, true, nblk, bytes, stream);
    if (plain) return launch_fused_plain(args, K, args.h.compute_loss != 0, pb == ESPM_ELL_PB, nblk, bytes, stream);
  }
  auto go = [&](auto kern, int threads) -> int {
    if (bytes > 64 * 1024)
      if (int rc = check_hip(hipFuncSetAttribute(reinterpret_cast<const void*>(kern), hipFuncAttributeMaxDynamicSharedMemorySize, (int)bytes),
                             "fused half-steps"))
        return rc;
    hipLaunchKernelGGL(kern, dim3(nblk + (args.h.tail_on == 1 ? 1 : 0)), dim3(threads), bytes, stream, args);
    return check_hip(hipGetLastError(), "fused half-steps launch");
  };
  if (pb == ESPM_ELL_PB)
    return args.h.compute_loss ? go(mu_fused_ell_kernel<K, true, ESPM_ELL_UNR_H, ESPM_ELL_UNR_W, ESPM_ELL_WTHREADS, true>, ESPM_ELL_WTHREADS)
                               : go(mu_fused_ell_kernel<K, false, ESPM_ELL_UNR_H, ESPM_ELL_UNR_W, ESPM_ELL_WTHREADS, true>, ESPM_ELL_WTHREADS);
  return args.h.compute_loss ? go(mu_fused_ell_kernel<K, true, ESPM_FUSED_SMALL_UNR_H, ESPM_FUSED_SMALL_UNR_W, ESPM_FUSED_SMALL_THREADS, false>, ESPM_FUSED_SMALL_THREADS)
                             : go(mu_fused_ell_kernel<K, false, ESPM_FUSED_SMALL_UNR_H, ESPM_FUSED_SMALL_UNR_W, ESPM_FUSED_SMALL_THREADS, false>, ESPM_FUSED_SMALL_THREADS);
}
#endif

size_t fused_ell_lds_bytes(int n_pad, int k, int pb) {
  if (pb < 128 || pb > ESPM_ELL_PB || (pb & (pb - 1))) return (size_t)-1;
  const int tab_rows = n_pad > pb ? n_pad : pb;
  const bool fixed = k > 4 && k >= ESPM_FIXTAB_MIN_K;
  if (fixed && tab_rows > ESPM_TAB2_BASE / 16) return (size_t)-1;
  const int wb = k <= 4 ? 0 : (k == 5 ? 1 : (k == 6 ? 2 : 4));
  const size_t tab_bytes = fixed ? (size_t)ESPM_TAB2_BASE + (size_t)16 * tab_rows : (size_t)(4 + wb) * 4 * tab_rows;
  const int seg = pb == ESPM_ELL_PB ? (k <= 4 ? 4 : (k <= 6 ? 3 : 2)) : ESPM_ELL_PB / pb;
  const int n_cg = (n_pad + 63) / 64;
  size_t part = (size_t)seg * k * pb * 4;
  const size_t red = (size_t)(ESPM_ELL_WTHREADS / 64 + 1) * (ESPM_HP_NSCALAR + 2 * k + 1) * sizeof(double);
  const size_t tail_scratch = (size_t)((ESPM_ELL_WTHREADS / 64 + 1) * (KP + 1) + 1) * sizeof(double);
  if (red > part) part = red;
  if (tail_scratch > part) part = tail_scratch;
  return tab_bytes + part + 16 + ESPM_FUSED_MAX_UNITS * sizeof(float) + (size_t)(3 * (pb / 64) + 2 * n_cg + 4) / 4 * 16 + 2 * KP * sizeof(double) + 8 +
         (pb != ESPM_ELL_PB ? (size_t)(pb + 64 * n_cg) * sizeof(int) : 0);
}

int launch_fused_ell(const HStepArgs& h, const WAccumArgs& w, int nblk, hipStream_t stream, int static_units, int stream_lists) {
  ESPM_REQUIRE(h.ell && h.ell_off && h.ell_klc && h.ell_pix && w.ell && w.ell_off && w.chan_perm, "fused half-steps: the sparse store's lists are missing");
  ESPM_REQUIRE(w.pb >= 128 && w.pb <= ESPM_ELL_PB && (w.pb & (w.pb - 1)) == 0 && 2 * h.ell_tp == w.pb && h.h_rule == 0 && h.write_h && !h.l2_m,
               "fused half-steps: blocks of two H tiles (tile_px=%d, ell_pb=%d), the default H rule, write_h", h.ell_tp, w.pb);
  ESPM_REQUIRE(nblk == (h.p + w.pb - 1) / w.pb && w.n_cg >= 1, "fused half-steps: nblk_w=%d must be ceil(p / %d)", nblk, w.pb);
  FusedArgs fa;
  fa.h = h;
  fa.w = w;
  fa.static_units = static_units;
  fa.stream_lists = stream_lists;
  switch (h.k) {
#if ESPM_MIN_K <= 8
#define ESPM_X(KK) case KK: return launch_fused_k<KK>(fa, nblk, stream);
    ESPM_K_CASES(ESPM_X)
#undef ESPM_X
#endif
  }
  return set_error(ESPM_EUNSUPPORTED, "fused half-steps: k=%d not built", h.k);
}

}

#ifdef ESPM_PHASE_CLOCK
extern "C" int espm_debug_phase_buffer(void* dev_ptr) {
  unsigned long long* p = static_cast<unsigned long long*>(dev_ptr);
  if (int rc = espm::phase_buffer_plain(p)) return rc;
  if (int rc = espm::phase_buffer_plain_stream(p)) return rc;
  return espm::check_hip(hipMemcpyToSymbol(HIP_SYMBOL(espm::espm_phase_buf), &p, sizeof(p)), "phase buffer");
}
#endif
```

### espm_amd/csrc/mu_fused_kernel.hpp

```cpp
#pragma once
#include "mu_ell_kernel.hpp"

#ifndef ESPM_FUSED_SMALL_THREADS
#define ESPM_FUSED_SMALL_THREADS 1024
#endif
#ifndef ESPM_FUSED_SMALL_PREFETCH
#define ESPM_FUSED_SMALL_PREFETCH 1
#endif
#ifndef ESPM_FUSED_CUT2
#define ESPM_FUSED_CUT2 60
#endif
#ifndef ESPM_FUSED_FIRST_PREFETCH
#define ESPM_FUSED_FIRST_PREFETCH 1
#endif
#ifndef ESPM_FUSED_FULL_PREFETCH
#define ESPM_FUSED_FULL_PREFETCH 1
#endif
#ifndef ESPM_FUSED_RED_ONE_BARRIER
#define ESPM_FUSED_RED_ONE_BARRIER 1
#endif
#ifndef ESPM_FUSED_SMALL_PRIO
#define ESPM_FUSED_SMALL_PRIO 4
#endif
#ifndef ESPM_FUSED_FULL_PRIO
#define ESPM_FUSED_FULL_PRIO 12
#endif
#ifndef ESPM_FUSED_PROLOGUE_BATCH
#define ESPM_FUSED_PROLOGUE_BATCH 1
#endif

#ifndef ESPM_FUSED_SUM_BATCHED
#define ESPM_FUSED_SUM_BATCHED 1
#endif
#ifndef ESPM_FUSED_SLAB_LDS
#define ESPM_FUSED_SLAB_LDS 1
#endif
#ifndef ESPM_FUSED_MAX_SEGS
#define ESPM_FUSED_MAX_SEGS 8
#endif
#ifndef ESPM_FUSED_SMALL_SKEW
#define ESPM_FUSED_SMALL_SKEW 0
#endif
#ifndef ESPM_FUSED_W_SPLIT
#define ESPM_FUSED_W_SPLIT 0
#endif
#ifndef ESPM_FUSED_SLAB_WT
#define ESPM_FUSED_SLAB_WT 1
#endif

namespace espm {

struct FusedArgs {
  HStepArgs h;
  WAccumArgs w;
  int cnt_lds_off;
  int meta_lds_off;
  int perm_lds_off;
  int static_units;
  int red_lds_off;
  int perm_lds;
  int h_segs;
  int w_split;
  int stream_lists;
  int slab_lds;
};

#ifndef ESPM_FUSED_CUT4_A
#define ESPM_FUSED_CUT4_A 45
#endif
#ifndef ESPM_FUSED_CUT4_B
#define ESPM_FUSED_CUT4_B 75
#endif
#ifndef ESPM_FUSED_CUT4_C
#define ESPM_FUSED_CUT4_C 92
#endif
#define ESPM_FUSED_MAX_UNITS 64
template <int K>
struct FusedGeom {
  static constexpr int S = K <= 4 ? 4 : (K <= 6 ? 3 : 2);
  static constexpr int S_MAX = K <= 6 ? 4 : 3;
  static constexpr int PROWS = K;
  static constexpr int MIN_SPLIT = 48;
  static __device__ __forceinline__ int seg_begin(int len, int s) {
    if (len < MIN_SPLIT) return s == 0 ? 0 : len;
    constexpr int cut4[5] = {0, ESPM_FUSED_CUT4_A, ESPM_FUSED_CUT4_B, ESPM_FUSED_CUT4_C, 100}, cut3[4] = {0, 45, 80, 100}, cut2[3] = {0, ESPM_FUSED_CUT2, 100};
    const int c = S == 4 ? cut4[s] : (S == 3 ? cut3[s] : cut2[s]);
    return (int)((long)len * c / 100);
  }
  static __device__ __forceinline__ int seg_begin_rt(int len, int s, int segs) {
    if (len < MIN_SPLIT) return s == 0 ? 0 : len;
    constexpr int cut4[5] = {0, ESPM_FUSED_CUT4_A, ESPM_FUSED_CUT4_B, ESPM_FUSED_CUT4_C, 100}, cut3[4] = {0, 45, 80, 100}, cut2[3] = {0, ESPM_FUSED_CUT2, 100};
    const int c = segs == 4 ? cut4[s] : (segs == 3 ? cut3[s] : cut2[s]);
    return (int)((long)len * c / 100);
  }
  static __device__ __forceinline__ int seg_begin_even(int len, int s, int segs) {
    if (len < MIN_SPLIT) return s == 0 ? 0 : len;
    if constexpr (ESPM_FUSED_SMALL_SKEW != 0) {
      if (segs > 1) return (int)(((long)len * s * (100L * segs + (long)ESPM_FUSED_SMALL_SKEW * (segs - s))) / (100L * segs * segs));
    }
    return (int)((long)len * s / segs);
  }
};

template <int K, bool LOSS, int UNR_H, int UNR_W, int NT, bool FULL, bool PLAIN = false, bool STREAM = false>
__global__ __launch_bounds__(NT) void mu_fused_ell_kernel(const FusedArgs fa) {
  static_assert(!FULL || NT == ESPM_ELL_WTHREADS, "full geometry: 1024 threads");
  static_assert(FULL || !STREAM, "streamed lists: the full geometry (an image below it fits the last-level cache)");
  static_assert(ESPM_ELL_PB == 2 * ESPM_ELL_TILE && ESPM_ELL_WTHREADS == ESPM_ELL_PB, "full geometry: a workgroup is two H tiles, one thread per pixel");
  const int PB = FULL ? ESPM_ELL_PB : fa.w.pb;
  const int PBITS = FULL ? ESPM_ELL_PBITS : fa.w.pbits;
  const int TP = PB / 2;
  const int GPT_SHIFT = PBITS - 7;
  constexpr int PROWS = FusedGeom<K>::PROWS;
  constexpr bool S_RT = FULL && FusedGeom<K>::S_MAX > FusedGeom<K>::S;
  const int S = (FULL && !S_RT) ? FusedGeom<K>::S : fa.h_segs;
  constexpr int PF = FULL ? ESPM_FUSED_FULL_PREFETCH : ESPM_FUSED_SMALL_PREFETCH;
  constexpr bool WALK_PP = FULL && K <= ESPM_ELL_WALK_PP_MAX_K;
  constexpr int PRIO = FULL ? (K >= 5 ? ESPM_FUSED_FULL_PRIO : 0) : ESPM_FUSED_SMALL_PRIO;
  const int NGRP = PB / 64;
  const HStepArgs& a = fa.h;
  extern __shared__ __attribute__((aligned(16))) float smem[];
  float* tab = smem;
  ell_table_at_lds_zero(tab);
  ESPM_PHASE_STAMP(0);
  ESPM_PHASE_WHERE();
  const int tab_rows = a.n_pad > PB ? a.n_pad : PB;
  float* part = smem + FixTab<K>::bytes(tab_rows) / sizeof(float);
  int* cnt = reinterpret_cast<int*>(reinterpret_cast<unsigned char*>(smem) + fa.cnt_lds_off);
  float* ukl = reinterpret_cast<float*>(cnt + 4);
  if (!PLAIN && a.tail_on == 1 && blockIdx.x == gridDim.x - 1) {
    w_tail_body<(10 * ESPM_ELL_WTHREADS) / NT>(a.tail, reinterpret_cast<double*>(smem));
    ESPM_PHASE_STAMP(7);
    return;
  }
  double* cs_lds = a.cs_parts ? reinterpret_cast<double*>(reinterpret_cast<unsigned char*>(smem) + a.cs_lds_off) : nullptr;
  int* meta = reinterpret_cast<int*>(reinterpret_cast<unsigned char*>(smem) + fa.meta_lds_off);
  int* lpix = reinterpret_cast<int*>(reinterpret_cast<unsigned char*>(smem) + fa.perm_lds_off);
  int* lchan = lpix + PB;
  const bool perm_lds = PLAIN ? !FULL : (!FULL || fa.perm_lds);
  const bool spread = a.tail_on == 2 && cs_lds;
  constexpr int RW = 2;
  const int rw_n = a.tail.n * a.tail.k, rw_per = (rw_n + (int)gridDim.x - 1) / (int)gridDim.x;
  const int rw_lo = min(rw_n, (int)blockIdx.x * rw_per), rw_hi = min(rw_n, rw_lo + rw_per);
  const bool rw_staged = rw_per <= RW * NT;
  float rwn[RW], rwo[RW];
#pragma unroll
  for (int u = 0; u < RW; ++u) rwn[u] = rwo[u] = 1.f;
  constexpr bool OWN_H = PLAIN && !FULL && ESPM_FUSED_SMALL_SKEW != 0;
  constexpr bool PREF_W = PLAIN && !FULL && K <= 6 && ESPM_FUSED_FIRST_PREFETCH != 0;
  const int wave_id = __builtin_amdgcn_readfirstlane((int)(threadIdx.x >> 6));
  bool staged = false;
  if constexpr (ESPM_FUSED_PROLOGUE_BATCH) {
    constexpr int TR = 4, PC = 4;
    const int n_perm = perm_lds ? PB + 64 * fa.w.n_cg : 0, n_woff = 2 * fa.w.n_cg + 1;
    staged = PLAIN || (a.n_pad <= TR * NT && n_perm <= PC * NT && n_woff <= NT && a.cs_nbk <= 64 && 2 * K <= NT / 64);
    if (staged) {
      float4 tlo[TR], thi[TR];
#pragma unroll
      for (int i = 0; i < TR; ++i) {
        const int r = threadIdx.x + i * NT;
        const float* src = a.gw_s + (size_t)min(r, a.n_pad - 1) * KP;
        tlo[i] = *reinterpret_cast<const float4*>(src);
        thi[i] = K > 4 ? *reinterpret_cast<const float4*>(src + 4) : make_float4(0.f, 0.f, 0.f, 0.f);
      }
      int pv[PC];
#pragma unroll
      for (int i = 0; i < PC; ++i) {
        const int j = threadIdx.x + i * NT;
        pv[i] = 0;
        if (j < n_perm) pv[i] = j < PB ? a.ell_pix[(size_t)blockIdx.x * PB + j] : fa.w.chan_perm[(size_t)blockIdx.x * fa.w.n_cg * 64 + (j - PB)];
      }
      int mh = 0, mw = 0;
      if ((int)threadIdx.x < 3 * NGRP) {
        const int gi = threadIdx.x / 3, j = threadIdx.x - 3 * gi;
        const bool tile_ok = blockIdx.x * PB + (gi >> GPT_SHIFT) * TP < a.p_pad;
        mh = tile_ok ? a.ell_off[2 * (blockIdx.x * NGRP + gi) + j] : 0;
      }
      if ((int)threadIdx.x < n_woff) mw = fa.w.ell_off[(size_t)2 * blockIdx.x * fa.w.n_cg + threadIdx.x];
      double csv = 0.0;
      const int cw = threadIdx.x >> 6;
      if (cs_lds && cw < K && (int)(threadIdx.x & 63) < a.cs_nbk) csv = a.cs_parts[(size_t)cw * a.cs_nbk + (threadIdx.x & 63)];
      if (spread && cw >= K && cw < 2 * K && (int)(threadIdx.x & 63) < a.cs_nbk)
        csv = a.cs_parts[(size_t)K * a.cs_nbk + (size_t)(cw - K) * a.cs_nbk + (threadIdx.x & 63)];
      if (spread && rw_staged) {
#pragma unroll
        for (int u = 0; u < RW; ++u) {
          const int i = rw_lo + (int)threadIdx.x + u * NT;
          rwn[u] = i < rw_hi ? a.tail.w_new[i] : 1.f;
          rwo[u] = i < rw_hi ? a.tail.w_old[i] : 1.f;
        }
      }
#pragma unroll
      for (int i = 0; i < TR; ++i) {
        const int r = threadIdx.x + i * NT;
        if (r < a.n_pad) FixTab<K>::put(tab, a.n_pad, r, tlo[i], thi[i]);
      }
#pragma unroll
      for (int i = 0; i < PC; ++i) {
        const int j = threadIdx.x + i * NT;
        if (j < n_perm) lpix[j] = pv[i];
      }
      if ((int)threadIdx.x < 3 * NGRP) meta[threadIdx.x] = mh;
      if ((int)threadIdx.x < n_woff) meta[3 * NGRP + threadIdx.x] = mw;
      if (cs_lds && cw < (spread ? 2 * K : K)) {
        csv = wave_sum(csv);
        if ((threadIdx.x & 63) == 0) (cw < K ? cs_lds : cs_lds + KP - K)[cw] = csv;
      }
      if (threadIdx.x == 0) {
        cnt[0] = OWN_H ? NT / 64 : 0;
        cnt[1] = PREF_W ? NT / 64 : 0;
      }
    }
  }
  if (!PLAIN && !staged) {
    if (cs_lds) {
      for (int kk = threadIdx.x >> 6; kk < (spread ? 2 * K : K); kk += NT / 64) {
        double v = 0.0;
        for (int j = threadIdx.x & 63; j < a.cs_nbk; j += 64) v += a.cs_parts[(size_t)kk * a.cs_nbk + j];
        v = wave_sum(v);
        if ((threadIdx.x & 63) == 0) (kk < K ? cs_lds : cs_lds + KP - K)[kk] = v;
      }
    }
    for (int r = threadIdx.x; r < a.n_pad; r += NT) FixTab<K>::put_row(tab, a.n_pad, r, a.gw_s + (size_t)r * KP);
    if (threadIdx.x == 0) cnt[0] = cnt[1] = 0;
    if ((int)threadIdx.x < 3 * NGRP) {
      const int gi = threadIdx.x / 3, j = threadIdx.x - 3 * gi;
      const bool tile_ok = blockIdx.x * PB + (gi >> GPT_SHIFT) * TP < a.p_pad;
      meta[threadIdx.x] = tile_ok ? a.ell_off[2 * (blockIdx.x * NGRP + gi) + j] : 0;
    }
    for (int i = threadIdx.x; i <= 2 * fa.w.n_cg; i += NT) meta[3 * NGRP + i] = fa.w.ell_off[(size_t)2 * blockIdx.x * fa.w.n_cg + i];
    if (perm_lds) {
      for (int i = threadIdx.x; i < PB; i += NT) lpix[i] = a.ell_pix[(size_t)blockIdx.x * PB + i];
      for (int i = threadIdx.x; i < 64 * fa.w.n_cg; i += NT) lchan[i] = fa.w.chan_perm[(size_t)blockIdx.x * fa.w.n_cg * 64 + i];
    }
  }
  __syncthreads();
  ESPM_PHASE_STAMP(1);
  float relw = -1.f;
  if (spread) {
    if (blockIdx.x == 0 && threadIdx.x < KP) a.tail.colsum_gw[threadIdx.x] = (int)threadIdx.x < K ? cs_lds[threadIdx.x] : 0.0;
    if (a.tail.hist_slot) {
      double sw = 0.0;
#pragma unroll
      for (int kk = 0; kk < K; ++kk) sw += cs_lds[KP + kk];
      const float shift = (float)((double)a.tail.rel_tol * (sw / (double)rw_n));
      relw = 0.f;
      if (rw_staged && (PLAIN || staged)) {
#pragma unroll
        for (int u = 0; u < RW; ++u)
          if (rw_lo + (int)threadIdx.x + u * NT < rw_hi) relw = fmaxf(relw, fabsf(rwn[u] - rwo[u]) / (rwn[u] + shift));
      } else {
        for (int i = rw_lo + (int)threadIdx.x; i < rw_hi; i += NT) {
          const float x = a.tail.w_new[i], y = a.tail.w_old[i];
          relw = fmaxf(relw, fabsf(x - y) / (x + shift));
        }
      }
    }
  }
  const int lane = threadIdx.x & 63;
  const int blk0 = blockIdx.x * PB;
  int own_next[2] = {(int)(threadIdx.x >> 6), (int)(threadIdx.x >> 6)};
  auto next_unit = [&](int which) {
    if (!PLAIN && fa.static_units) {
      const int u = own_next[which];
      own_next[which] += NT / 64;
      return __builtin_amdgcn_readfirstlane(u);
    }
    int u = 0;
    if (lane == 0) u = __hip_atomic_fetch_add(cnt + which, 1, __ATOMIC_RELAXED, __HIP_MEMORY_SCOPE_WORKGROUP);
    return __builtin_amdgcn_readfirstlane(u);
  };

  for (int u = OWN_H ? wave_id : next_unit(0); u < NGRP * S; u = next_unit(0)) {
    const int seg = u / NGRP, gi = u - seg * NGRP;
    const int grp = blk0 / 64 + gi;
    float acc[K];
#pragma unroll
    for (int kk = 0; kk < K; ++kk) acc[kk] = 0.f;
    float kl = 0.f;
    int lp = lane;
    if (blk0 + (gi >> GPT_SHIFT) * TP < a.p_pad) {
      lp = perm_lds ? lpix[gi * 64 + lane] : a.ell_pix[grp * 64 + lane];
      const int beg = meta[3 * gi], mid = meta[3 * gi + 1] - beg, len = meta[3 * gi + 2] - beg;
      const int x0 = FULL ? (S_RT ? FusedGeom<K>::seg_begin_rt(len, seg, S) : FusedGeom<K>::seg_begin(len, seg)) : FusedGeom<K>::seg_begin_even(len, seg, S);
      const int x1 = FULL ? (S_RT ? FusedGeom<K>::seg_begin_rt(len, seg + 1, S) : FusedGeom<K>::seg_begin(len, seg + 1)) : FusedGeom<K>::seg_begin_even(len, seg + 1, S);
      if (x0 < x1) {
        const int px = blk0 + (gi >> GPT_SHIFT) * TP + lp;
        float hk[K];
#pragma unroll
        for (int kk = 0; kk < K; ++kk) hk[kk] = a.h_in[(size_t)kk * a.p_pad + px];
        const uint32_t* lrow = a.ell + (size_t)beg * 64 + lane;
        ell_h_rows<K, LOSS, UNR_H, PF, PRIO, STREAM, true, WALK_PP>(lrow, x0, x1, mid, tab, a.n_pad, a.ell_bits, hk, acc, kl);
        if constexpr (PRIO > 0) __builtin_amdgcn_s_setprio(0);
      }
    }
    float* dst = part + (size_t)seg * PROWS * PB + (gi >> GPT_SHIFT) * TP + lp;
#pragma unroll
    for (int kk = 0; kk < K; ++kk) dst[(size_t)kk * PB] = acc[kk];
    if constexpr (LOSS) {
      const float klw = wave_sum(kl);
      if (lane == 0) ukl[u] = klw;
    } else if (lane == 0) {
      ukl[u] = 0.f;
    }
  }
  ESPM_PHASE_STAMP(2);
  ESPM_WAVE_STAMP(8);
  uint32_t fw_rows[PF][UNR_W];
  float fw_gw[K];
  int fw_c = -1, fw_kind = 0;
  auto request_w = [&]() {
    if constexpr (PREF_W) {
      if (wave_id < fa.w.n_cg) {
        const int cg = wave_id;
        fw_c = perm_lds ? lchan[cg * 64 + lane] : fa.w.chan_perm[((size_t)blockIdx.x * fa.w.n_cg + cg) * 64 + lane];
        const float* gsrc = fa.w.gw_s + (size_t)(fw_c < 0 ? 0 : fw_c) * KP;
#pragma unroll
        for (int kk = 0; kk < K; ++kk) fw_gw[kk] = gsrc[kk];
        const int* off = meta + 3 * NGRP + 2 * cg;
        const int beg = off[0], mid = off[1], end = off[2];
        const uint32_t* lrow = fa.w.ell + (size_t)beg * 64 + lane;
        if (ell_walk_request<UNR_W, PF, STREAM>(lrow, mid - beg, fw_rows)) fw_kind = 1;
        else if (mid == beg && ell_walk_request<UNR_W, PF, STREAM>(lrow, end - mid, fw_rows)) fw_kind = 2;
      }
    }
  };
  h_epilogue<K, true, 0, ESPM_FUSED_SUM_BATCHED ? (FULL ? FusedGeom<K>::S_MAX : ESPM_FUSED_MAX_SEGS) : 0, PLAIN>(
      a, part, S, PB, blk0, 0.f, cs_lds, tab, PB, false,
      (PLAIN || fa.red_lds_off >= 0) ? reinterpret_cast<double*>(reinterpret_cast<unsigned char*>(smem) + fa.red_lds_off) : nullptr, relw, request_w,
      ukl, NGRP * S);

  ESPM_PHASE_STAMP(5);
  const WAccumArgs& w = fa.w;
  const int b = blockIdx.x;
  const bool w_split = !PLAIN && ESPM_FUSED_W_SPLIT && fa.w_split;
  const bool slab_lds = PLAIN || (ESPM_FUSED_SLAB_LDS && fa.slab_lds);
  const int w_units = w_split ? 2 * w.n_cg : w.n_cg;
  bool first_w = PREF_W;
  for (int wu = PREF_W ? wave_id : next_unit(1); wu < w_units; wu = next_unit(1), first_w = false) {
    const int cg = w_split ? wu >> 1 : wu, whalf = w_split ? wu & 1 : 0;
    const int c = (PREF_W && first_w) ? fw_c : (perm_lds ? lchan[cg * 64 + lane] : w.chan_perm[((size_t)b * w.n_cg + cg) * 64 + lane]);
    const float* gsrc = w.gw_s + (size_t)(c < 0 ? 0 : c) * KP;
    float gw[K], acc[K];
    if (PREF_W && first_w) {
#pragma unroll
      for (int kk = 0; kk < K; ++kk) gw[kk] = fw_gw[kk];
    } else {
#pragma unroll
// ... 69 lines not shown
```

### espm_amd/csrc/mu_w_step.hip

```cpp
#include <atomic>
#include <stdio.h>
#include <stdlib.h>

#include "mu_w_kernel.hpp"
#include "mu_w_mfma_kernel.hpp"
#include "mu_xchg.hpp"

#ifndef ESPM_MFMA_MIN_K
#define ESPM_MFMA_MIN_K 9
#endif

namespace espm {

struct WReduceArgs {
  const float* slab;
  float* out;
  int nblk, total, nred_blocks, fuse_finalize;
  HFinalizeArgs fin;
  const float* halo_h;
  float* halo_top;
  float* halo_bot;
  int halo_k, halo_nx, halo_ny, halo_ppad;
  const float* bw_old;
  double* bparts;
  int bn, bk, bn_pad;
};

__global__ __launch_bounds__(256) void w_reduce_kernel(const WReduceArgs a) {
  __shared__ double fscratch[5 * (ESPM_HP_NSCALAR + 2 * KP + 1)];
  __shared__ float s_part[8][32];
  if ((int)blockIdx.x >= a.nred_blocks) {
    const int job = (int)blockIdx.x - a.nred_blocks;
    if (a.halo_top && job == H_FINALIZE_NV) {
      for (int e = threadIdx.x; e < a.halo_k * a.halo_ny; e += 256) {
        const int kk = e / a.halo_ny, j = e - kk * a.halo_ny;
        a.halo_top[e] = a.halo_h[(size_t)kk * a.halo_ppad + j];
        a.halo_bot[e] = a.halo_h[(size_t)kk * a.halo_ppad + (size_t)(a.halo_nx - 1) * a.halo_ny + j];
      }
    }
    h_finalize_one(a.fin, job, fscratch);
    return;
  }
  const int col = threadIdx.x & 31, grp = threadIdx.x >> 5;
  const int e = blockIdx.x * 32 + col;
  float acc[8];
#pragma unroll
  for (int u = 0; u < 8; ++u) acc[u] = 0.f;
  if (e < a.total) {
    int b = grp;
    for (; b + 56 < a.nblk; b += 64) {
#pragma unroll
      for (int u = 0; u < 8; ++u) acc[u] += a.slab[(size_t)(b + 8 * u) * a.total + e];
    }
    for (int u = 0; b < a.nblk; b += 8, ++u) acc[u & 7] += a.slab[(size_t)b * a.total + e];
  }
  s_part[grp][col] = ((acc[0] + acc[1]) + (acc[2] + acc[3])) + ((acc[4] + acc[5]) + (acc[6] + acc[7]));
  __syncthreads();
  if (grp == 0) {
    float t = 0.f;
    if (e < a.total) {
#pragma unroll
      for (int g = 0; g < 8; ++g) t += s_part[g][col];
      a.out[e] = t;
    }
    if (a.bparts) {
      const int kk = e / a.bn_pad, c = e - kk * a.bn_pad;
      const float num = (e < a.total && c < a.bn) ? a.bw_old[(size_t)c * a.bk + kk] * t : 0.f;
      double sum = num > 0.f ? (double)num : 0.0, cnt = num > 0.f ? 1.0 : 0.0;
      float mx = fmaxf(num, 0.f);
#pragma unroll
      for (int off = 16; off >= 1; off >>= 1) {
        sum += __shfl_xor(sum, off, 64);
        cnt += __shfl_xor(cnt, off, 64);
        mx = fmaxf(mx, __shfl_xor(mx, off, 64));
      }
      if (col == 0) {
        a.bparts[3 * (size_t)blockIdx.x] = sum;
        a.bparts[3 * (size_t)blockIdx.x + 1] = (double)mx;
        a.bparts[3 * (size_t)blockIdx.x + 2] = cnt;
      }
    }
  }
}

constexpr int WF_THREADS = 1024;
#ifndef ESPM_WF_FEW_THREADS
#define ESPM_WF_FEW_THREADS 512
#endif
constexpr int WF_FEW_THREADS = ESPM_WF_FEW_THREADS;
#ifndef ESPM_WF_HALF_MAX_K
#define ESPM_WF_HALF_MAX_K 8
#endif
constexpr int WF_HALF_MAX_K = ESPM_WF_HALF_MAX_K;

struct WUpdateArgs {
  const unsigned char* src;
  size_t src_stride;
  int nsrc, n, n_pad, k, nbk;
  float* a_out;
  const double* hpart;
  const double* hstat_rs;
  int nblk_h;
  size_t rec_hstat_off;
  double* hstat_out;
  const float* w_old;
  float* w_new;
  const float* fixed_w;
  const float* breg_sr;
  float pg_gamma_w;
  int pg_track;
  float* gw_s;
  double* parts;
  float log_shift, gw_floor, xscale;
  int fuse_finalize;
  HFinalizeArgs fin;
};

__device__ __forceinline__ void w_update_preload(const WUpdateArgs& a, int kk, int c, bool mine, float& wo, float& fx) {
  wo = 1.f;
  fx = -1.f;
  if (mine && c < a.n) {
    wo = a.w_old[(size_t)c * a.k + kk];
    if (a.fixed_w) fx = a.fixed_w[(size_t)c * a.k + kk];
  }
}
__device__ __forceinline__ void w_update_entries(const WUpdateArgs& a, int kk, int c, int e, bool owns, float t, double rs, int nwg, int wg,
                                                 float wo_pre, float fx_pre) {
  double cs = 0.0, sw = 0.0, qw = 0.0;
  if (owns) {
    a.a_out[e] = t;
    if (c < a.n) {
      const float wo = wo_pre;
      float v;
      if (a.pg_gamma_w > 0.f) {
        v = fmaxf(wo - ((float)rs - t) / a.pg_gamma_w, a.log_shift);
        const double dw = (double)v - (double)wo;
        qw = dw * (double)((float)rs - t) + (double)a.pg_gamma_w * dw * dw;
      } else if (a.breg_sr) {
        const float sr = a.xscale * a.breg_sr[c];
        v = fmaxf((sr * wo) / (((float)rs - t) * wo + sr), a.log_shift);
      } else {
        v = fmaxf((wo * t) / (float)rs, a.log_shift);
      }
      if (fx_pre >= 0.f) v = fx_pre;
      a.w_new[(size_t)c * a.k + kk] = v;
      const float gv = fmaxf(v, a.gw_floor);
      a.gw_s[(size_t)c * KP + kk] = gv * (1.f / a.xscale);
      cs = (double)gv;
      sw = (double)v;
    } else {
      a.gw_s[(size_t)c * KP + kk] = 1.f;
    }
  }
  cs = wave_sum(cs);
  sw = wave_sum(sw);
  if (a.pg_track) qw = wave_sum(qw);
  if (threadIdx.x == 0) {
    a.parts[wg] = cs;
    a.parts[nwg + wg] = sw;
    if (a.pg_track) a.parts[2 * nwg + wg] = qw;
  }
}

__global__ __launch_bounds__(256) void w_reduce_update_kernel(const WUpdateArgs a) {
  __shared__ double fscratch[5 * (ESPM_HP_NSCALAR + 2 * KP + 1)];
  __shared__ float s_part[8][32];
  __shared__ double s_rsw[4];
  const int nwg = a.k * a.nbk;
  if ((int)blockIdx.x >= nwg) {
#ifndef ESPM_EXPERIMENT_NO_FINALIZE
    h_finalize_one(a.fin, (int)blockIdx.x - nwg, fscratch);
#endif
    return;
  }
  const int kk = blockIdx.x / a.nbk, j = blockIdx.x - kk * a.nbk;
  const int col = threadIdx.x & 31, grp = threadIdx.x >> 5;
  const int c = 32 * j + col;
  const int e = kk * a.n_pad + c;
  auto src = [&](int b) { return reinterpret_cast<const float*>(a.src + (size_t)b * a.src_stride)[e]; };
  constexpr int INFLIGHT = 32;
  float v[INFLIGHT];
  const bool live = c < a.n_pad;
#pragma unroll
  for (int u = 0; u < INFLIGHT; ++u) {
    const int b = grp + 8 * u;
    v[u] = (live && b < a.nsrc) ? src(b) : 0.f;
  }
  float wo_pre, fx_pre;
  w_update_preload(a, kk, c, threadIdx.x < 32, wo_pre, fx_pre);
  double rsp = 0.0;
  if (a.hpart) {
    const size_t nb = a.nblk_h;
    for (int b = threadIdx.x; b < a.nblk_h; b += 256) rsp += a.hpart[(ESPM_HP_ROWSUM + kk) * nb + b];
  }
  float acc[8];
#pragma unroll
  for (int u = 0; u < 8; ++u) acc[u] = ((v[u] + v[u + 8]) + v[u + 16]) + v[u + 24];
  if (live) {
    int b = grp + 8 * INFLIGHT;
    for (; b + 56 < a.nsrc; b += 64) {
#pragma unroll
      for (int u = 0; u < 8; ++u) acc[u] += src(b + 8 * u);
    }
    for (int u = 0; b < a.nsrc; b += 8, ++u) acc[u & 7] += src(b);
  }
  s_part[grp][col] = ((acc[0] + acc[1]) + (acc[2] + acc[3])) + ((acc[4] + acc[5]) + (acc[6] + acc[7]));
  double rs = 0.0;
  if (a.hpart) {
    rsp = wave_sum(rsp);
    if ((threadIdx.x & 63) == 0) s_rsw[threadIdx.x >> 6] = rsp;
    __syncthreads();
    rs = ((s_rsw[0] + s_rsw[1]) + s_rsw[2]) + s_rsw[3];
  } else if (a.hstat_rs) {
    rs = a.hstat_rs[ESPM_HS_ROWSUM + kk];
    __syncthreads();
  } else {
    for (int r = 0; r < a.nsrc; ++r)
      rs += reinterpret_cast<const double*>(a.src + (size_t)r * a.src_stride + a.rec_hstat_off)[ESPM_HS_ROWSUM + kk];
    if (blockIdx.x == 0 && threadIdx.x < ESPM_HS_STRIDE) {
      double t = 0.0;
      for (int r = 0; r < a.nsrc; ++r) {
        const double v2 = reinterpret_cast<const double*>(a.src + (size_t)r * a.src_stride + a.rec_hstat_off)[threadIdx.x];
        t = (int)threadIdx.x < ESPM_HS_MAX ? t + v2 : fmax(t, v2);
      }
      a.hstat_out[threadIdx.x] = t;
    }
    __syncthreads();
  }
  if (threadIdx.x < 64) {
    float t = 0.f;
    const bool owns = grp == 0 && c < a.n_pad;
    if (owns) {
#pragma unroll
      for (int g = 0; g < 8; ++g) t += s_part[g][col];
    }
    w_update_entries(a, kk, c, e, owns, t, rs, nwg, blockIdx.x, wo_pre, fx_pre);
  }
}

struct WSimplexArgs {
  WUpdateArgs u;
  const double* bparts;
  const double* hstat;
  double rows;
  double tol;
};

__global__ __launch_bounds__(64) void w_simplex_update_kernel(const WSimplexArgs x) {
  const WUpdateArgs& a = x.u;
  const int nwg = a.k * a.nbk;
  const int kk = blockIdx.x / a.nbk, j = blockIdx.x - kk * a.nbk;
  const int lane = threadIdx.x;
  const int c = 32 * j + (lane & 31);
  const int e = kk * a.n_pad + c;
  const bool owns = lane < 32 && c < a.n_pad;
  const float t_e = owns ? a.a_out[e] : 0.f;
  float wo_pre, fx_pre;
  w_update_preload(a, kk, c, owns, wo_pre, fx_pre);
  double ssum[KP], smax[KP], spos[KP], rs[KP];
#pragma unroll
  for (int q = 0; q < KP; ++q) {
    ssum[q] = 0.0; smax[q] = 0.0; spos[q] = 0.0; rs[q] = 1.0;
    if (q < a.k) {
      double s1 = 0.0, s3 = 0.0, s2 = 0.0;
      for (int b = lane; b < a.nbk; b += 64) {
        const double* p = x.bparts + 3 * ((size_t)q * a.nbk + b);
        s1 += p[0];
        s2 = fmax(s2, p[1]);
        s3 += p[2];
      }
      ssum[q] = wave_sum(s1);
      smax[q] = wave_max(s2);
      spos[q] = wave_sum(s3);
      rs[q] = x.hstat[ESPM_HS_ROWSUM + q];
    }
  }
  const double eps = (double)a.log_shift;
  double root[KP], fder[KP], ad[KP], width[KP], uu[KP], cst[KP];
  bool solve[KP];
#pragma unroll
  for (int q = 0; q < KP; ++q) {
    solve[q] = q < a.k && ssum[q] > 0.0 && ssum[q] < INFINITY;
    const double den = (double)(float)rs[q];
    const double lo = smax[q] / 2 - den;
    const double hi = x.rows * smax[q] / 0.5 - den;
    cst[q] = (x.rows - spos[q]) * eps;
    ad[q] = lo + den;
    width[q] = hi - lo;
    root[q] = solve[q] ? (fabs(cst[q]) <= 1e-11 ? ssum[q] : ssum[q] / (1.0 - cst[q])) : 1.0;
    fder[q] = solve[q] ? -ssum[q] / (root[q] * root[q]) : 0.0;
    uu[q] = solve[q] ? fmin(fmax((root[q] - ad[q]) / width[q], 0.0), 1.0) : 0.5;
  }
  auto mid_frac = [](double u1, int t) {
    const double scale = ldexp(1.0, t - 1);
    const double cell = fmin(floor(u1 * scale), scale - 1.0);
    return ldexp(2.0 * cell + 1.0, -t);
  };
  unsigned long long mc[2], mb[2];
  for (int hf = 0; hf < 2; ++hf) {
    const int t = 1 + lane + 64 * hf;
    double est = 0.0;
#pragma unroll
    for (int q = 0; q < KP; ++q)
      if (q < a.k) est = fmax(est, fabs(fder[q] * ((ad[q] + width[q] * mid_frac(uu[q], t)) - root[q])));
    const bool certain = t <= 101 && (est <= 0.99 * x.tol || t == 101);
    const bool band = t <= 101 && !certain && est <= 1.01 * x.tol;
    mc[hf] = __ballot(certain);
    mb[hf] = __ballot(band);
  }
  int t_stop = 101;
  for (;;) {
    const unsigned long long w0 = mc[0] | mb[0], w1 = mc[1] | mb[1];
    if (!w0 && !w1) break;
    const int hf = w0 ? 0 : 1;
    const int bit = __ffsll((long long)(hf ? w1 : w0)) - 1;
    const int t = 1 + bit + 64 * hf;
    if ((mc[hf] >> bit) & 1ull) { t_stop = t; break; }
    double worst = 0.0;
#pragma unroll
    for (int q = 0; q < KP; ++q)
      if (q < a.k && fder[q] != 0.0) {
        const double d = ad[q] + width[q] * mid_frac(uu[q], t);
        worst = fmax(worst, fabs(ssum[q] / d + cst[q] - 1.0));
      }
    if (worst <= x.tol) { t_stop = t; break; }
    mb[hf] &= ~(1ull << bit);
  }
  double delta = rs[0];
#pragma unroll
  for (int q = 0; q < KP; ++q)
    if (q == kk) delta = solve[q] ? ad[q] + width[q] * mid_frac(uu[q], t_stop) : (double)(float)rs[q];
  w_update_entries(a, kk, c, e, owns, t_e, delta, nwg, blockIdx.x, wo_pre, fx_pre);
}

#ifndef ESPM_XCHG_SMALL_WORLD
#define ESPM_XCHG_SMALL_WORLD 8
#endif
struct WExchangeArgs {
  WUpdateArgs u;
  unsigned char* mbox[16];
  int world, rank, nfl, with_halo;
  size_t rec_bytes, slot_base, wgflags_off, gran_off, err_off, hstat_off, top_off, bot_off;
  unsigned int seq;
  long long max_ticks;
  int release;
  const float* halo_h;
  int halo_k, halo_nx, halo_ny, halo_ppad;
  double* bparts;
};

__device__ __forceinline__ void xchg_store_flag(unsigned int* flag, unsigned int seq, int release) {
  if (release) __hip_atomic_store(flag, seq, __ATOMIC_RELEASE, __HIP_MEMORY_SCOPE_SYSTEM);
  else __hip_atomic_store(flag, seq, __ATOMIC_RELAXED, __HIP_MEMORY_SCOPE_SYSTEM);
}

__device__ __forceinline__ void xchg_wait_flag(const unsigned int* flag, unsigned int seq, long long max_ticks, unsigned int* err) {
  const long long t0 = wall_clock64();
  while ((int)(__hip_atomic_load(flag, __ATOMIC_RELAXED, __HIP_MEMORY_SCOPE_SYSTEM) - seq) < 0) {
    if (wall_clock64() - t0 > max_ticks) {
      atomicAdd(err, 1u);
      break;
    }
    __builtin_amdgcn_s_sleep(2);
  }
}

template <int MAXW>
__global__ __launch_bounds__(256) void w_exchange_update_kernel(const WExchangeArgs x) {
  const WUpdateArgs& a = x.u;
  __shared__ double fscratch[5 * (ESPM_HP_NSCALAR + 2 * KP + 1)];
  __shared__ float s_part[8][32];
  const int nwg = a.k * a.nbk;
  auto record = [&](int dst, int src_rank) { return x.mbox[dst] + x.slot_base + (size_t)src_rank * x.rec_bytes; };
  auto flag = [&](int dst, int src_rank, int idx) {
    return reinterpret_cast<unsigned int*>(x.mbox[dst] + x.wgflags_off + ((size_t)src_rank * x.nfl + idx) * sizeof(unsigned int));
  };
  const size_t GRAN = (size_t)34 * x.nfl + 2 * ESPM_HS_STRIDE;
  auto gran = [&](int dst, int src_rank, int g) {
    return reinterpret_cast<unsigned long long*>(x.mbox[dst] + x.gran_off) + (size_t)src_rank * GRAN + g;
  };
  constexpr int NJ = H_FINALIZE_JOBS;
  if ((int)blockIdx.x < NJ) {
    const int job = (int)blockIdx.x;
    const bool halo_job = job == H_FINALIZE_NV;
    if (halo_job && x.with_halo) {
      for (int d = -1; d <= 1; ++d) {
        const int r = x.rank + d;
        if (r < 0 || r >= x.world) continue;
        float* top = reinterpret_cast<float*>(record(r, x.rank) + x.top_off);
// ... 865 lines not shown
      }
      row[kk] = v;
    }
    store_row_kp(a.gw_s + (size_t)c * KP, row);
  }
  block_reduce<KP, KP>(cs, scratch);
  if (tid == 0)
    for (int kk = 0; kk < KP; ++kk) a.colsum_gw[kk] = cs[kk];
}

template <int K>
static int dispatch_w_k(const WAccumArgs& args, int x_dtype, int nblk, hipStream_t stream) {
  if (args.l2 && x_dtype != ESPM_X_F32) return set_error(ESPM_EUNSUPPORTED, "the l2 W accumulation needs the f32 store");
  constexpr int CH8 = K <= 8 ? 8 : 4;
  if (K >= ESPM_MFMA_MIN_K && args.mfma && args.x_cm && args.n_pad % 8 == 0) {
    const dim3 grid(nblk, (args.n_pad + 4 * 16 * MF_CT - 1) / (4 * 16 * MF_CT));
    if (x_dtype == ESPM_X_U8) {
      hipLaunchKernelGGL((w_accum_mfma_kernel<K, uint8_t>), grid, dim3(256), 0, stream, args);
    } else if (x_dtype == ESPM_X_BF16) {
      hipLaunchKernelGGL((w_accum_mfma_kernel<K, bf16_t>), grid, dim3(256), 0, stream, args);
    } else if (args.l2) {
      hipLaunchKernelGGL((w_accum_mfma_l2_kernel<K>), grid, dim3(256), 0, stream, args);
    } else {
      hipLaunchKernelGGL((w_accum_mfma_kernel<K, float>), grid, dim3(256), 0, stream, args);
    }
    return check_hip(hipGetLastError(), "w_accum (mfma) launch");
  }
  if constexpr (K > 16) {
    if (x_dtype != ESPM_X_F32)
      return set_error(ESPM_EUNSUPPORTED, "w_accum: %d components on the 8-bit / bf16 store run on the matrix cores only (no_fused = 0, n_pad a multiple of 8)", K);
  }
  if (x_dtype == ESPM_X_U8) {
    if constexpr (K <= 16) {
      dim3 grid(nblk, (args.n_pad + 4 * 64 * CH8 - 1) / (4 * 64 * CH8));
      hipLaunchKernelGGL((w_accum_kernel<K, uint8_t, CH8, 4, 3>), grid, dim3(256), 0, stream, args);
    }
  } else if (x_dtype == ESPM_X_BF16) {
    if constexpr (K <= 16) {
      dim3 grid(nblk, (args.n_pad + 4 * 64 * CH8 - 1) / (4 * 64 * CH8));
      hipLaunchKernelGGL((w_accum_kernel<K, bf16_t, CH8, 4, 0>), grid, dim3(256), 0, stream, args);
    }
  } else {
    dim3 grid(nblk, (args.n_pad + 4 * 64 * 4 - 1) / (4 * 64 * 4));
    if (args.l2)
      hipLaunchKernelGGL((w_accum_kernel<K, float, 4, 4, 0, true>), grid, dim3(256), 0, stream, args);
    else
      hipLaunchKernelGGL((w_accum_kernel<K, float, 4, 4, 0>), grid, dim3(256), 0, stream, args);
  }
  return check_hip(hipGetLastError(), "w_accum launch");
}

int dispatch_w_accum(const WAccumArgs& args, int k, int x_dtype, int nblk, hipStream_t stream) {
  switch (k) {
#define ESPM_X(KK) case KK: return dispatch_w_k<KK>(args, x_dtype, nblk, stream);
    ESPM_K_CASES(ESPM_X)
#undef ESPM_X
  }
  return set_error(ESPM_EUNSUPPORTED, "w_accum: k=%d not built (%d..%d)", k, ESPM_MIN_K, ESPM_MAX_K);
}

int launch_w_reduce(const float* slab, float* out, int nblk, int total, const HFinalizeArgs* fused_finalize,
                    hipStream_t stream, const float* bw_old, double* bparts, int n, int k, int n_pad) {
  WReduceArgs a;
  a.bw_old = bw_old;
  a.bparts = bparts;
  a.bn = n;
  a.bk = k;
  a.bn_pad = n_pad;
  a.slab = slab;
  a.out = out;
  a.nblk = nblk;
  a.total = total;
  a.nred_blocks = (total + 31) / 32;
  a.fuse_finalize = fused_finalize != nullptr;
  if (fused_finalize) a.fin = *fused_finalize;
  a.halo_h = nullptr;
  a.halo_top = a.halo_bot = nullptr;
  a.halo_k = a.halo_nx = a.halo_ny = a.halo_ppad = 0;
  hipLaunchKernelGGL(w_reduce_kernel, dim3(a.nred_blocks + (fused_finalize ? H_FINALIZE_JOBS : 0)), dim3(256), 0, stream, a);
  return check_hip(hipGetLastError(), "w_reduce launch");
}

int launch_w_reduce_pack(const float* slab, int nblk, int k, int n_pad, const HFinalizeArgs& fin_to_record,
                         const float* h_new, int nx, int ny, int p_pad, int with_halo, void* rec, hipStream_t stream) {
  WReduceArgs a;
  unsigned char* r = static_cast<unsigned char*>(rec);
  const int na = k * n_pad;
  a.slab = slab;
  a.out = reinterpret_cast<float*>(r);
  a.nblk = nblk;
  a.total = na;
  a.nred_blocks = (na + 31) / 32;
  a.fuse_finalize = 1;
  a.fin = fin_to_record;
  a.halo_h = h_new;
  a.halo_top = with_halo ? reinterpret_cast<float*>(r + (size_t)na * 4 + ESPM_HS_STRIDE * 8) : nullptr;
  a.halo_bot = with_halo ? a.halo_top + (size_t)k * ny : nullptr;
  a.halo_k = k;
  a.halo_nx = nx;
  a.halo_ny = ny;
  a.halo_ppad = p_pad;
  a.bw_old = nullptr;
  a.bparts = nullptr;
  a.bn = a.bk = a.bn_pad = 0;
  hipLaunchKernelGGL(w_reduce_kernel, dim3(a.nred_blocks + H_FINALIZE_JOBS), dim3(256), 0, stream, a);
  return check_hip(hipGetLastError(), "w_reduce_pack launch");
}

WTailArgs make_w_tail_args(const WFinishArgs& f) {
  WTailArgs t;
  t.parts = reinterpret_cast<const double*>(f.scratch);
  t.w_old = f.w_old;
  t.w_new = f.w_new;
  t.colsum_gw = f.colsum_gw;
  t.hist_slot = f.hist_slot;
  t.pg_q = f.pg_q;
  t.n = f.n;
  t.k = f.k;
  t.nbk = (f.n_pad + 31) / 32;
  t.rel_tol = f.rel_tol;
  return t;
}

int launch_w_reduce_update(const WFinishArgs& f, const void* src, size_t src_stride, int nsrc, float* a_out,
                           const double* hpart, int nblk_h, const double* hstat_rs, size_t rec_hstat_off, double* hstat_out,
                           const HFinalizeArgs* fused_finalize, hipStream_t stream, WTailArgs* defer_tail) {
  WUpdateArgs a;
  a.src = static_cast<const unsigned char*>(src);
  a.src_stride = src_stride;
  a.nsrc = nsrc;
  a.n = f.n;
  a.n_pad = f.n_pad;
  a.k = f.k;
  a.nbk = (f.n_pad + 31) / 32;
  a.a_out = a_out;
  a.hpart = hpart;
  a.hstat_rs = hstat_rs;
  a.nblk_h = nblk_h;
  a.rec_hstat_off = rec_hstat_off;
  a.hstat_out = hstat_out;
  a.w_old = f.w_old;
  a.w_new = f.w_new;
  a.fixed_w = f.fixed_w;
  a.breg_sr = f.breg_sr;
  a.pg_gamma_w = f.pg_gamma_w;
  a.pg_track = f.pg_q != nullptr;
  a.gw_s = f.gw_s;
  a.parts = reinterpret_cast<double*>(f.scratch);
  a.log_shift = f.log_shift;
  a.gw_floor = f.gw_floor;
  a.xscale = f.xscale;
  a.fuse_finalize = fused_finalize != nullptr;
  if (fused_finalize) a.fin = *fused_finalize;
  hipLaunchKernelGGL(w_reduce_update_kernel, dim3(a.k * a.nbk + (fused_finalize ? H_FINALIZE_JOBS : 0)), dim3(256), 0, stream, a);
  const WTailArgs t = make_w_tail_args(f);
  if (defer_tail)
    *defer_tail = t;
  else
    hipLaunchKernelGGL(w_update_tail_kernel, dim3(1), dim3(WT_THREADS), 0, stream, t);
  return check_hip(hipGetLastError(), "w_reduce_update launch");
}

int launch_w_simplex_update(const WFinishArgs& f, float* a_inout, const double* bparts, double tol, hipStream_t stream, WTailArgs* defer_tail) {
  WSimplexArgs x;
  WUpdateArgs& a = x.u;
  a.src = nullptr;
  a.src_stride = 0;
  a.nsrc = 0;
  a.n = f.n;
  a.n_pad = f.n_pad;
  a.k = f.k;
  a.nbk = (f.n_pad + 31) / 32;
  a.a_out = a_inout;
  a.hpart = nullptr;
  a.hstat_rs = nullptr;
  a.nblk_h = 0;
  a.rec_hstat_off = 0;
  a.hstat_out = nullptr;
  a.w_old = f.w_old;
  a.w_new = f.w_new;
  a.fixed_w = f.fixed_w;
  a.breg_sr = nullptr;
  a.pg_gamma_w = 0.f;
  a.pg_track = 0;
  a.gw_s = f.gw_s;
  a.parts = reinterpret_cast<double*>(f.scratch);
  a.log_shift = f.log_shift;
  a.gw_floor = f.gw_floor;
  a.xscale = f.xscale;
  a.fuse_finalize = 0;
  x.bparts = bparts;
  x.hstat = f.hstat;
  x.rows = (double)f.n;
  x.tol = tol;
  hipLaunchKernelGGL(w_simplex_update_kernel, dim3(a.k * a.nbk), dim3(64), 0, stream, x);
  if (int rc = check_hip(hipGetLastError(), "w_simplex_update launch")) return rc;
  const WTailArgs t = make_w_tail_args(f);
  if (defer_tail)
    *defer_tail = t;
  else
    hipLaunchKernelGGL(w_update_tail_kernel, dim3(1), dim3(WT_THREADS), 0, stream, t);
  return check_hip(hipGetLastError(), "w_simplex_update tail launch");
}

int launch_w_exchange_update(const WFinishArgs& f, const void* slabs, size_t slab_stride, int nslab, float* a_out, double* hstat_out,
                             const HFinalizeArgs& fin, const espm_xchg* xc, unsigned int seq, const float* h_new, int nx, int ny, int p_pad,
                             int with_halo, hipStream_t stream, WTailArgs* defer_tail, double* bparts) {
  WExchangeArgs x;
  x.bparts = bparts;
  WUpdateArgs& a = x.u;
  a.src = static_cast<const unsigned char*>(slabs);
  a.src_stride = slab_stride;
  a.nsrc = nslab;
  a.n = f.n;
  a.n_pad = f.n_pad;
  a.k = f.k;
  a.nbk = (f.n_pad + 31) / 32;
  a.a_out = a_out;
  a.hpart = fin.hpart;
  a.hstat_rs = nullptr;
  a.nblk_h = fin.nblk;
  a.rec_hstat_off = 0;
  a.hstat_out = hstat_out;
  a.w_old = f.w_old;
  a.w_new = f.w_new;
  a.fixed_w = f.fixed_w;
  a.breg_sr = f.breg_sr;
  a.pg_gamma_w = f.pg_gamma_w;
  a.pg_track = f.pg_q != nullptr;
  a.gw_s = f.gw_s;
  a.parts = reinterpret_cast<double*>(f.scratch);
  a.log_shift = f.log_shift;
  a.gw_floor = f.gw_floor;
  a.xscale = f.xscale;
  a.fuse_finalize = 1;
  a.fin = fin;
  const int nwg = a.k * a.nbk;
  ESPM_REQUIRE(nwg + 1 <= xc->wgflags, "exchange: %d reduction workgroups, the mailbox holds flags for %d", nwg, xc->wgflags - 1);
  for (int r = 0; r < 16; ++r) x.mbox[r] = r < xc->world ? xc->peers[r] : nullptr;
  for (int r = 0; r < xc->world; ++r) ESPM_REQUIRE(x.mbox[r], "exchange: rank %d is not connected (espm_xchg_connect)", r);
  x.world = xc->world;
  x.rank = xc->rank;
  x.nfl = xc->wgflags;
  x.with_halo = with_halo;
  x.rec_bytes = xc->record_bytes;
  x.slot_base = (size_t)(seq & 1u) * xc->world * xc->record_bytes;
  x.wgflags_off = xc->off_wgflags;
  x.gran_off = xc->off_gran + (size_t)(seq & 1u) * xc->world * ((size_t)34 * xc->wgflags + 2 * ESPM_HS_STRIDE) * sizeof(unsigned long long);
  x.err_off = xc->off_err;
  x.hstat_off = (size_t)f.k * f.n_pad * 4;
  x.top_off = x.hstat_off + ESPM_HS_STRIDE * 8;
  x.bot_off = x.top_off + (size_t)f.k * (ny > 0 ? ny : 0) * 4;
  x.seq = seq;
  x.max_ticks = 200000000LL;
  x.release = xc->order;
  x.halo_h = h_new;
  x.halo_k = f.k;
  x.halo_nx = nx;
  x.halo_ny = ny;
  x.halo_ppad = p_pad;
  a.fin.hstat_out = reinterpret_cast<double*>(xc->mailbox + x.slot_base + (size_t)xc->rank * xc->record_bytes + x.hstat_off);
  if (xc->world <= ESPM_XCHG_SMALL_WORLD)
    hipLaunchKernelGGL(w_exchange_update_kernel<ESPM_XCHG_SMALL_WORLD>, dim3(nwg + H_FINALIZE_JOBS), dim3(256), 0, stream, x);
  else
    hipLaunchKernelGGL(w_exchange_update_kernel<16>, dim3(nwg + H_FINALIZE_JOBS), dim3(256), 0, stream, x);
  if (bparts) return check_hip(hipGetLastError(), "w_exchange_update launch");
  const WTailArgs t = make_w_tail_args(f);
  if (defer_tail)
    *defer_tail = t;
  else
    hipLaunchKernelGGL(w_update_tail_kernel, dim3(1), dim3(WT_THREADS), 0, stream, t);
  return check_hip(hipGetLastError(), "w_exchange_update launch");
}

int launch_w_update_tail(const WTailArgs& t, hipStream_t stream) {
  hipLaunchKernelGGL(w_update_tail_kernel, dim3(1), dim3(WT_THREADS), 0, stream, t);
  return check_hip(hipGetLastError(), "w_update_tail launch");
}

template <int KK, int NT>
static void launch_fast(const WFinishArgs& args, int rows, int crows, size_t lds, hipStream_t stream) {
  if (crows > rows && rows <= 1) {
    if (crows <= 2)
      hipLaunchKernelGGL((w_finish_fast_kernel<KK, 1, NT, 2>), dim3(1), dim3(NT), lds, stream, args);
    else
      hipLaunchKernelGGL((w_finish_fast_kernel<KK, 1, NT, 4>), dim3(1), dim3(NT), lds, stream, args);
    return;
  }
  if (crows > rows) rows = crows;
  if constexpr (NT == 256) {
    if (rows > 4) {
      hipLaunchKernelGGL((w_finish_fast_kernel<KK, 8, NT>), dim3(1), dim3(NT), lds, stream, args);
      return;
    }
  }
  if (rows <= 1)
    hipLaunchKernelGGL((w_finish_fast_kernel<KK, 1, NT>), dim3(1), dim3(NT), lds, stream, args);
  else if (rows <= 2)
    hipLaunchKernelGGL((w_finish_fast_kernel<KK, 2, NT>), dim3(1), dim3(NT), lds, stream, args);
  else
    hipLaunchKernelGGL((w_finish_fast_kernel<KK, 4, NT>), dim3(1), dim3(NT), lds, stream, args);
}

__global__ __launch_bounds__(256) void w_gfinish_update_kernel(const WFinishArgs a) {
  __shared__ float s_wave[4];
  const int e = blockIdx.x, mm = e / a.k, kk = e - mm * a.k;
  const float* gt = a.g_t + (size_t)mm * a.n_pad;
// ... 630 lines not shown
```

### espm_amd/engine.py

```python
from __future__ import annotations

import ctypes as C
import os
import sys
import time

import numpy as np
import torch

from . import _lib
from ._lib import MUState
from .store import CODES, StoreFacts, choose_store

AUTOTUNE_MIN_ITERS = 5000


def _ptr(t):
    return C.c_void_p(t.data_ptr()) if t is not None else C.c_void_p(None)


def _stream():
    return C.c_void_p(torch.cuda.current_stream().cuda_stream)


# ... 178 lines not shown
        if x_store in ("auto", "ell"):
            unfilled = (not self.bregman and ((empty_ch is not None and bool(empty_ch.any()))
                                              or (empty_px is not None and bool(empty_px.any()))))
            if unfilled:
                _set_lines(Xd, layout, empty_px, empty_ch, 0)
            heavy_on = os.environ.get("ESPM_ELL_HEAVY", "1") != "0"
            facts = _scan_x(Xd, None if unfilled else x_facts, heavy_on)
            n_heavy, nnz = facts.n_heavy, facts.nnz
            code, dense_code, note, warn = choose_store(self.n, self.p, self.k, x_store, facts, h_rule=h_rule, bregman=self.bregman,
                                                        pg_gamma_w=pg_gamma_w, heavy_on=heavy_on)
            if warn:
                import warnings
                warnings.warn("espm_amd: " + note, RuntimeWarning, stacklevel=4)
            flag = torch.tensor([code, dense_code], device=self.device, dtype=torch.int32)
            self._tick("storage type (integer counts, bf16-exact, density)")
            if group is not None:
                torch.distributed.all_reduce(flag, op=torch.distributed.ReduceOp.MIN, group=group)
            flag = flag[:1] if int(flag[0]) == 3 else flag.min().reshape(1)
            if unfilled and int(flag.item()) != 3:
                _set_lines(Xd, layout, empty_px, empty_ch, log_shift)
                flag.fill_(0)
            if x_store == "ell" and int(flag.item()) != 3:
                raise ValueError("x_store='ell' needs integer counts <= 2^24 (above 255: the default H rule, no Bregman variant, no "
                                 "projected-gradient W step), n <= 16384 and a GW table that fits in LDS (12- or 16-float rows from 9 components on)")
            refill = unfilled and int(flag.item()) == 3 and masks_given
            x_store = CODES[int(flag.item())]
        if int(h_rule) != 0 and x_store in ("u8", "bf16"):
            x_store = "f32"
        if x_store not in CODES:
            raise ValueError("x_store must be 'auto', 'ell', 'u8', 'bf16' or 'f32'")
        return x_store, note, n_heavy, nnz, refill

    def _geometry(self, shape_2d, tile_px, x_tile):
        p, x_store = self.p, self.x_store
        st = MUState()
        st.n, st.p, st.k = self.n, p, self.k
        st.x_dtype = {"u8": _lib.X_U8, "bf16": _lib.X_BF16, "f32": _lib.X_F32, "ell": _lib.X_ELL}[x_store]
        if shape_2d is not None:
            nx, ny = int(shape_2d[0]), int(shape_2d[1])
            if nx * ny != p:
                raise ValueError(f"shape_2d {shape_2d} does not match the {p} pixels of X")
            st.nx, st.ny, st.grid_mode = nx, ny, 1
        else:
            st.nx, st.ny, st.grid_mode = 0, 0, 0
        self._check(self.lib.espm_mu_query(C.byref(st)))
        force_tile = tile_px if tile_px is not None else (int(os.environ["ESPM_FORCE_ELL_TILE"]) if os.environ.get("ESPM_FORCE_ELL_TILE") else None)
        if x_store == "ell" and force_tile in (64, 128, 256, 512):
            st.tile_px = st.x_tile = int(force_tile)
            st.ell_pb = 2 * st.tile_px
            st.nblk_w = (p + st.ell_pb - 1) // st.ell_pb
        if x_store != "ell":
            if tile_px is not None:
                st.tile_px = int(tile_px)
                st.x_tile = int(tile_px)
            if x_tile is not None:
                st.x_tile = int(x_tile)
        p_total = torch.tensor([p], dtype=torch.int64, device=self.device)
        if self.group is not None:
            torch.distributed.all_reduce(p_total, group=self.group)
        st.p_total = int(p_total.item())
        self.p_total = st.p_total
        return st

    def _build_store(self, Xd, layout, n_heavy, nnz, empty_px):
        st, dev, k = self.st, self.device, self.k
        self.ell = None
        self.fill_px = self.fill_num = None
        torch_builder = self.x_store == "ell" and os.environ.get("ESPM_ELL_BUILDER", "hip") == "torch"
        if not torch_builder:
            Xc = Xd.contiguous()
            src = (_ptr(Xc), _lib.SRC_F64 if Xc.dtype == torch.float64 else _lib.SRC_F32, _lib.LAYOUT_PM if layout == "pm" else _lib.LAYOUT_CM,
                   Xc.shape[1])
        if self.x_store == "ell":
            from . import ell as _ell
            self.x_cm = self.x_pm = None
            if torch_builder:
                self.ell = _ell.build(Xd if layout == "pm" else Xd.t(), st.p_pad, st.ell_cbits, st.tile_px)
            else:
                self.ell = self._build_ell(src, n_heavy, nnz)
                self._tick("sparse store build")
            assert self.ell["n_cg"] == st.n_cg and self.ell["nblk_w"] == st.nblk_w
            fill_n = 0
            if empty_px is not None and bool(empty_px.any()):
                idx = torch.nonzero(empty_px).flatten()
                if idx.numel() >= 1 << 24:
                    raise NotImplementedError("more than 2^24 pixels without counts")
                fill_n = idx.numel()
                self.fill_px = idx.to(torch.int32).contiguous()
                self.ell["klc"][idx] = -(torch.arange(idx.numel(), device=dev, dtype=torch.float32) + 1.0)
            hv = self.ell.get("hv")
            npx = hv["npx"] if hv is not None else 0
            if hv is not None:
                if fill_n + npx >= 1 << 24:
                    raise NotImplementedError("more than 2^24 pixels without counts or with counts above 255")
                hpx = hv["px"].long()
                self.hv_klc = self.ell["klc"][hpx].clone()
                self.hv_kl = torch.zeros(npx, dtype=torch.float64, device=dev)
                self.ell["klc"][hpx] = -(torch.arange(npx, device=dev, dtype=torch.float32) + float(fill_n + 1))
            if fill_n + npx > 0:
                self.fill_num = torch.zeros((k, fill_n + npx), dtype=torch.float32, device=dev)
            self.x_bytes = 4 * (self.ell["ell_h"].numel() + self.ell["ell_w"].numel()) + (16 * hv["n"] if hv is not None else 0)
        else:
            xt = {"u8": torch.uint8, "bf16": torch.bfloat16, "f32": torch.float32}[self.x_store]
            self.x_cm = torch.empty((st.p_pad // st.x_tile, st.n_cm, st.x_tile), dtype=xt, device=dev)
            self.x_pm = torch.empty((self.p, st.n_pad), dtype=xt, device=dev)
            self._check(self.lib.espm_mu_pack_x(*src, self.n, self.p, _ptr(self.x_cm), _ptr(self.x_pm), st.x_dtype, st.n_pad, st.p_pad,
                                                st.x_tile, st.n_cm, _stream()))
            self.x_bytes = self.x_cm.numel() * self.x_cm.element_size() + self.x_pm.numel() * self.x_pm.element_size()

    def _ingest_G(self, G):
        st, dev = self.st, self.device
        if G is not None:
            Gh = np.ascontiguousarray(np.asarray(G, dtype=np.float32))
            if Gh.ndim != 2 or Gh.shape[0] != self.n:
                raise ValueError(f"G must be (n={self.n}, m), got {Gh.shape}")
            self.m = Gh.shape[1]
            self.g = torch.from_numpy(Gh).to(dev)
            self.g_t = torch.zeros((self.m, st.n_pad), dtype=torch.float32, device=dev)
            self.g_t[:, :self.n] = self.g.t()
            self.colsum_g = torch.from_numpy(np.asarray(G, dtype=np.float64).sum(axis=0).astype(np.float32)).to(dev)
            st.m = self.m
        else:
            self.m, self.g, self.colsum_g, self.g_t = 0, None, None, None
            st.m = 0
        self.M = self.m if self.m > 0 else self.n

    def _set_hyper_parameters(self, *, simplex_H, simplex_W, compute_loss, lambda_L, sigmaL, h_rule, pg_gamma_w, epsilon_reg, log_shift,
                              dicotomy_tol, tol, xscale, gw_floor, mu):
        st = self.st
        st.simplex_h, st.simplex_w = int(bool(simplex_H)), int(bool(simplex_W))
        st.compute_loss = int(bool(compute_loss))
        st.lambda_l, st.sigma_l = float(lambda_L), float(sigmaL)
        st.h_rule = int(h_rule)
        st.pg_gamma_w = float(pg_gamma_w)
        st.eps_reg, st.log_shift = float(epsilon_reg), float(log_shift)
        st.dicotomy_tol, st.rel_tol = float(dicotomy_tol), float(tol)
        self.rel_tol = float(tol)
        st.xscale, st.gw_floor = float(xscale), float(gw_floor)
        self.lambda_L, self.xscale = float(lambda_L), float(xscale)
        mu_arr = np.asarray(mu, dtype=np.float64)
        if mu_arr.ndim == 0 and float(mu_arr) == 0.0:
            self.mu = None
        else:
            self.mu = torch.from_numpy(np.broadcast_to(mu_arr, (self.k,)).astype(np.float32).copy()).to(self.device)

    def _allocate(self, max_iter, fixed_H, fixed_W, simplex_rows, simplex_W, log_shift, breg_px, with_pg_q):
        st, dev, k = self.st, self.device, self.k
        f32 = dict(dtype=torch.float32, device=dev)
        f64 = dict(dtype=torch.float64, device=dev)
        self.w = [torch.zeros((self.M, k), **f32) for _ in range(2)]
        self.h = [torch.ones((k, st.p_pad), **f32) for _ in range(2)]
        self.h_t = torch.zeros((self.p, self.V.KP), **f32)
        self.gw_s = torch.zeros((st.n_pad, self.V.KP), **f32)
        self.colsum_gw = torch.zeros(self.V.KP, **f64)
        nblk_h = (self.p + st.tile_px - 1) // st.tile_px
        self.hpart = torch.zeros((nblk_h, self.V.HP_STRIDE), **f64)
        self.hstat = [torch.zeros(self.V.HS_STRIDE, **f64) for _ in range(2)]
        self._tick("rest up to the state buffers")
        self.a_slab = torch.zeros((st.nblk_w, k, st.n_pad), **f32)
        self.a = torch.zeros((k, st.n_pad), **f32)
        self.w_scratch = torch.zeros((2, self.M, k), **f32)
        self.hist_len = int(max_iter) + 3
        self.hist = torch.zeros((self.hist_len, _lib.HI_STRIDE), **f64)
        self.frob = torch.zeros(self.hist_len, **f64) if self.frobenius else None
        self.fixed_h = self._pad_h(fixed_H) if fixed_H is not None else None
        self.fixed_w = (torch.from_numpy(np.ascontiguousarray(np.asarray(fixed_W, dtype=np.float32))).to(dev)
                        if fixed_W is not None else None)
        if simplex_rows is not None:
            mask = np.zeros(self.M, dtype=np.int32)
            mask[np.asarray(simplex_rows)] = 1
            self.simplex_rows = torch.from_numpy(mask).to(dev)
            if log_shift > 0 and simplex_W and mask.sum() * log_shift >= 1:
                raise ValueError("No solution exists!")
        else:
            self.simplex_rows = None
        if self.bregman:
            self.breg_px = torch.zeros(st.p_pad, **f32)
            self.breg_px[:self.p] = breg_px
        self.pg_q = torch.zeros((self.hist_len, 2), **f64) if with_pg_q else None

    def _bind(self):
        st = self.st
        if self.ell is None:
            st.x_cm, st.x_pm = self.x_cm.data_ptr(), self.x_pm.data_ptr()
        else:
            st.x_cm = st.x_pm = None
            st.ell_h, st.ell_h_off, st.ell_klc = (self.ell[key].data_ptr() for key in ("ell_h", "ell_h_off", "klc"))
            if self.fill_px is not None:
                st.ell_fill_px, st.ell_fill_n = self.fill_px.data_ptr(), int(self.fill_px.numel())
            if self.fill_num is not None:
                st.ell_fill_num = self.fill_num.data_ptr()
            hv = self.ell.get("hv")
            if hv is not None:
                st.ell_hv_n, st.ell_hv_npx, st.ell_hv_ngrp = hv["n"], hv["npx"], hv["ngrp"]
                st.ell_hv_px, st.ell_hv_px_off, st.ell_hv_pm = (hv[key].data_ptr() for key in ("px", "px_off", "pm"))
                st.ell_hv_grp, st.ell_hv_grp_off, st.ell_hv_wm = (hv[key].data_ptr() for key in ("grp", "grp_off", "wm"))
                st.ell_hv_klc, st.ell_hv_kl = self.hv_klc.data_ptr(), self.hv_kl.data_ptr()
            st.ell_w, st.ell_w_off, st.chan_perm = (self.ell[key].data_ptr() for key in ("ell_w", "ell_w_off", "chan_perm"))
            st.pix_perm = self.ell["pix_perm"].data_ptr()
        st.g = self.g.data_ptr() if self.g is not None else None
        st.g_t = self.g_t.data_ptr() if self.g_t is not None else None
        st.colsum_g = self.colsum_g.data_ptr() if self.colsum_g is not None else None
        st.w[0], st.w[1] = self.w[0].data_ptr(), self.w[1].data_ptr()
        st.h[0], st.h[1] = self.h[0].data_ptr(), self.h[1].data_ptr()
        st.gw_s, st.colsum_gw, st.h_t = self.gw_s.data_ptr(), self.colsum_gw.data_ptr(), self.h_t.data_ptr()
        st.gw_a, st.gw_p = None, None
        st.mu = self.mu.data_ptr() if self.mu is not None else None
        st.fixed_h = self.fixed_h.data_ptr() if self.fixed_h is not None else None
        st.fixed_w = self.fixed_w.data_ptr() if self.fixed_w is not None else None
        st.simplex_rows = self.simplex_rows.data_ptr() if self.simplex_rows is not None else None
        st.halo_top = st.halo_bot = None
        if self.bregman:
            st.breg_sr_px, st.breg_sr_ch = self.breg_px.data_ptr(), self._breg_ch.data_ptr()
        else:
            st.breg_sr_px = st.breg_sr_ch = None
        st.hpart = self.hpart.data_ptr()
        st.hstat[0], st.hstat[1] = self.hstat[0].data_ptr(), self.hstat[1].data_ptr()
        st.a_slab, st.a, st.w_scratch = self.a_slab.data_ptr(), self.a.data_ptr(), self.w_scratch.data_ptr()
        st.hist, st.hist_len = self.hist.data_ptr(), self.hist_len
        st.pg_q = self.pg_q.data_ptr() if self.pg_q is not None else None
        st.cur, st.it = 0, 0

    def _launch_policy(self, fused, autotune, max_iter):
        st = self.st
        if os.environ.get("ESPM_FUSED"):
            fused = {"0": False, "1": True}.get(os.environ["ESPM_FUSED"], os.environ["ESPM_FUSED"])
        st.no_fused = {"static": 2, "always": 3}.get(fused, 0 if fused else 1)
        limit = float(os.environ["ESPM_ELL_STREAM_MB"]) * 2 ** 20 if os.environ.get("ESPM_ELL_STREAM_MB") else _lib.ELL_STREAM_BYTES
        st.ell_stream = int(self.x_store == "ell" and self.x_bytes > limit)
        self._accum_done = False
        self._autotune = (int(max_iter) >= AUTOTUNE_MIN_ITERS) if autotune == "auto" else bool(autotune)
        self.plan_timings = None

    def _build_ell(self, src, n_heavy, nnz):
        st, dev = self.st, self.device
        i32 = dict(dtype=torch.int32, device=dev)
        x8 = torch.empty((self.p, st.n_pad), dtype=torch.uint8, device=dev)
        x8c = torch.empty((st.p_pad // _lib.PPAD, st.n_cm, _lib.PPAD), dtype=torch.uint8, device=dev) if os.environ.get("ESPM_ELL_BUILD_CM") != "0" else None
        self._check(self.lib.espm_mu_pack_x(*src, self.n, self.p, _ptr(x8c) if x8c is not None else None, _ptr(x8), _lib.X_U8, st.n_pad,
                                            st.p_pad, _lib.PPAD, st.n_cm, _stream()))
        hv = None
        if n_heavy:
            hv_cnt = torch.empty(self.p, **i32)
            self._check(self.lib.espm_mu_ell_heavy_count(C.byref(st), *src, _ptr(x8), _ptr(x8c) if x8c is not None else None, _ptr(hv_cnt),
                                                         _stream()))
            hv_off = torch.zeros(self.p + 1, **i32)
            hv_off[1:] = torch.cumsum(hv_cnt, 0)
            n_hv = int(hv_off[-1])
            if n_hv:
                pm = torch.empty((n_hv, 2), **i32)
                self._check(self.lib.espm_mu_ell_heavy_fill(C.byref(st), *src, _ptr(hv_off), _ptr(pm), _stream()))
                q = torch.repeat_interleave(torch.arange(self.p, device=dev), hv_cnt.long())
                from . import ell as _ell
                hv = _ell.heavy_orders(q, pm[:, 0].long(), pm[:, 1].long(), self.n, st.ell_pb)
        cnt_px = torch.empty((2, st.p_pad), **i32)
        cnt_bc = torch.empty((2, st.nblk_w, st.n_cg * 64), **i32)
        klc = torch.empty(st.p_pad, dtype=torch.float32, device=dev)
        hist = os.environ.get("ESPM_ELL_BUILD_HIST") != "0"
        bkt_px = torch.empty((st.p_pad, _lib.ELL_BUCKETS), dtype=torch.uint8, device=dev) if hist else None
        bkt_bc = torch.empty((st.nblk_w, st.n_cg * 64, _lib.ELL_BUCKETS), dtype=torch.uint8, device=dev) if hist else None
        self._check(self.lib.espm_mu_ell_count_hist(C.byref(st), _ptr(x8), _ptr(cnt_px), _ptr(cnt_bc), _ptr(klc),
                                                    _ptr(bkt_px) if hist else None, _ptr(bkt_bc) if hist else None, _stream()))
        chan_perm = torch.empty((st.nblk_w, st.n_cg * 64), **i32)
        pix_perm = torch.empty(st.p_pad, **i32)
        h_off = torch.empty(2 * (st.p_pad // 64) + 1, **i32)
        w_off = torch.empty(2 * st.nblk_w * st.n_cg + 1, **i32)
        rows = torch.zeros(2, dtype=torch.int64, device=dev)
        self._check(self.lib.espm_mu_ell_plan(C.byref(st), _ptr(cnt_px), _ptr(cnt_bc), _ptr(chan_perm), _ptr(pix_perm), _ptr(h_off),
                                   _ptr(w_off), _ptr(rows), _stream()))
        rows_h, rows_w = (int(v) for v in rows.cpu())
        if max(rows_h, rows_w) * 64 >= 2 ** 31:
            raise ValueError("sparse count store: the lists exceed 2^31 dwords")
        ell_h = torch.zeros(max(rows_h, 1) * 64, **i32)
        ell_w = torch.zeros(max(rows_w, 1) * 64, **i32)
        st.x_cm = x8c.data_ptr() if x8c is not None else None
        try:
            self._check(self.lib.espm_mu_ell_fill_hist(C.byref(st), _ptr(x8), _ptr(chan_perm), _ptr(pix_perm), _ptr(h_off), _ptr(w_off),
                                                       _ptr(ell_h), _ptr(ell_w), _ptr(bkt_px) if hist else None, _ptr(bkt_bc) if hist else None, _stream()))
        finally:
            st.x_cm = None
        torch.cuda.current_stream().synchronize()
        out = dict(ell_h=ell_h, ell_h_off=h_off, klc=klc, pix_perm=pix_perm, ell_w=ell_w, ell_w_off=w_off, chan_perm=chan_perm, n_cg=st.n_cg,
                   nblk_w=st.nblk_w, nnz=nnz, entries_h=int(cnt_px[0].sum()), entries_w=int(cnt_bc[0].sum()), rows_h=rows_h,
                   rows_w=rows_w, unit_rows_h=int((h_off[1::2] - h_off[0:-1:2]).sum()),
                   unit_rows_w=int((w_off[1::2] - w_off[0:-1:2]).sum()))
        if hv is not None:
            out["hv"] = hv
        return out

    def _pad_h(self, H):
        Hh = np.asarray(H, dtype=np.float32)
        if Hh.shape != (self.k, self.p):
            raise ValueError(f"expected an array of shape {(self.k, self.p)}, got {Hh.shape}")
        out = torch.full((self.k, self.st.p_pad), -1.0, dtype=torch.float32, device=self.device)
        out[:, :self.p] = torch.from_numpy(np.ascontiguousarray(Hh)).to(self.device)
        return out

    def load_state(self, W, H):
        st = self.st

        def as_f32(a, shape, name):
            if isinstance(a, torch.Tensor):
                t = a.to(device=self.device, dtype=torch.float32)
            else:
                t = torch.from_numpy(np.ascontiguousarray(np.asarray(a, dtype=np.float32)))
            if tuple(t.shape) != shape:
                raise ValueError(f"{name} must be {shape}, got {tuple(t.shape)}")
            return t
        Wt = as_f32(W, (self.M, self.k), "W")
        Ht = as_f32(H, (self.k, self.p), "H")
        st.cur, st.it = 0, 0
        self._pending_finalize = None
        self._pending_tail = False
        self._accum_done = False
        self.hist.zero_()
        self.w[0].copy_(Wt)
        self.h[0][:, :self.p].copy_(Ht)
        self._check(self.lib.espm_mu_build_gw(C.byref(st), 0, _stream()))
        self._check(self.lib.espm_mu_hstat(C.byref(st), 0, _stream()))
        if self.sharded:
            self._globalize_hstat(0)
            self._exchange_halo_only(0)
        if self._autotune:
            self._autotune = False
            self.autotune_plan()

    PLANS = {0: "fused, units handed out dynamically", 2: "fused, fixed unit assignment", 1: "H-step and W accumulation as two launches"}

    def autotune_plan(self, iters=48, warm=4):
        st = self.st
        if self.sharded or self.frobenius or self.ell is None:
            return None
        keep = st.no_fused
        st.no_fused = 0
        if not bool(self.lib.espm_mu_fused_applies(C.byref(st))):
            st.no_fused = keep
            return None
        iters = int(os.environ.get("ESPM_AUTOTUNE_ITERS", iters))
        iters = min(iters, self.hist_len - st.it - 2 - warm)
        if iters < 4:
            st.no_fused = keep
            return None
        tensors = [self.w[0], self.w[1], self.h[0], self.h[1], self.gw_s, self.colsum_gw, self.hstat[0], self.hstat[1], self.hist,
                   self.w_scratch, self.hpart]
        saved = [t.clone() for t in tensors]
        state = (st.cur, st.it)

        def restore():
            for t, sv in zip(tensors, saved):
                t.copy_(sv)
            st.cur, st.it = state
        rounds = 3
        per = max(iters // rounds, 2)
        st.no_fused = 0
        self._check(self.lib.espm_mu_iterate(C.byref(st), min(2 * iters, self.hist_len - st.it - 2), 0, _stream()))
        restore()
        total = {plan: 0.0 for plan in self.PLANS}
        for _ in range(rounds):
            for plan in self.PLANS:
# ... 417 lines not shown
```

### include/espm_mu.h

```cpp
#ifndef ESPM_MU_H
#define ESPM_MU_H

#include <stddef.h>
#include <stdint.h>

#ifdef __cplusplus
extern "C" {
#endif

typedef void* espm_stream_t;

typedef enum espm_status {
  ESPM_OK = 0,
  ESPM_EINVAL = -1,
  ESPM_ENOSOLUTION = -2,
  ESPM_EHIP = -3,
  ESPM_EUNSUPPORTED = -4
} espm_status;

enum { ESPM_X_F32 = 0, ESPM_X_BF16 = 1, ESPM_X_U8 = 2 ,
       ESPM_X_ELL = 3  };
enum { ESPM_SRC_F32 = 0, ESPM_SRC_F64 = 1 };
enum { ESPM_LAYOUT_CM = 0 , ESPM_LAYOUT_PM = 1  };

#ifndef ESPM_KP
#define ESPM_KP 8
#endif
#ifndef ESPM_MAX_K
#define ESPM_MAX_K ESPM_KP
#endif
#ifndef ESPM_MIN_K
#define ESPM_MIN_K 1
#endif
#define ESPM_PPAD 512
#define ESPM_NPAD 8
#define ESPM_ELL_TILE 512
#define ESPM_ELL_PB 1024
#define ESPM_ELL_PBITS 10
#define ESPM_ELL_UNIT_ROWS 8
#define ESPM_ELL_UNIT_MAX_N 4080
#define ESPM_ELL_PAIR_MAX_K 6
#define ESPM_ELL_STREAM_BYTES (256 << 20)
#define ESPM_FUSED_MIN_PB 512
#define ESPM_FUSED_MIN_BLOCKS 192
#define ESPM_ELL_HEAVY_MIN 256
#define ESPM_ELL_HEAVY_MAX (1 << 24)
#define ESPM_ELL_WTHREADS 1024
#ifndef ESPM_ELL_BUCKETS
#define ESPM_ELL_BUCKETS 16
#endif
#define ESPM_ELL_LDS_MAX (160 * 1024)
#define ESPM_NCM 16
#define ESPM_W_DICOTOMY_TOL 1e-5f
#define ESPM_TAIL_DEFER 1
#define ESPM_TAIL_RIDE 2

#define ESPM_HP_KL 0
#define ESPM_HP_REG 1
#define ESPM_HP_LAP 2
#define ESPM_HP_BAD 3
#define ESPM_HP_ROWSUM 4
#define ESPM_HP_MAX (4 + ESPM_KP)
#define ESPM_HP_RELH (4 + 2 * ESPM_KP)
#define ESPM_HP_PGQ (5 + 2 * ESPM_KP)
#define ESPM_HP_RELW (6 + 2 * ESPM_KP)
#define ESPM_HP_NSCALAR 5
#define ESPM_HP_STRIDE (8 + 2 * ESPM_KP)

#define ESPM_HS_ROWSUM 0
#define ESPM_HS_MAX ESPM_KP
#define ESPM_HS_STRIDE (2 * ESPM_KP)

#define ESPM_HI_KLX 0
#define ESPM_HI_REG 1
#define ESPM_HI_LAP 2
#define ESPM_HI_SUMY 3
#define ESPM_HI_BAD 4
#define ESPM_HI_REL_W 5
#define ESPM_HI_REL_H 6
#define ESPM_HI_STRIDE 8

#define ESPM_MU_ABI_VERSION 5

typedef struct espm_mu_state {
  uint32_t struct_size;
  uint32_t abi_version;
  int32_t n;
  int32_t m;
  int32_t k;
  int32_t p;
  int32_t nx, ny;
  int32_t n_pad;
  int32_t p_pad;
  int32_t x_dtype;
  int32_t tile_px;
  int32_t nblk_w;
  int32_t x_tile;
  int32_t n_cm;
  int32_t h_variant;
  int64_t p_total;
  int32_t simplex_h, simplex_w;
  int32_t grid_mode;
  int32_t compute_loss;
  float lambda_l, sigma_l, eps_reg, log_shift, dicotomy_tol, rel_tol;
  float xscale;
  float gw_floor;
  const void* x_cm;
  const void* x_pm;
  const float* g;
  const float* colsum_g;
  float* w[2];
  float* gw_s;
  double* colsum_gw;
  void* gw_a;
  float* gw_p;
  float* h[2];
  float* h_t;
  const float* mu;
  const float* fixed_h;
  const float* fixed_w;
  const int32_t* simplex_rows;
  const float* halo_top;
  const float* halo_bot;
  double* hpart;
  double* hstat[2];
  float* a_slab;
  float* a;
  float* w_scratch;
  double* hist;
  int32_t hist_len;
  int32_t cur;
  int32_t it;
  const uint32_t* ell_h;
  const int32_t* ell_h_off;
  const float* ell_klc;
  const uint32_t* ell_w;
  const int32_t* ell_w_off;
  const int32_t* chan_perm;
  int32_t ell_cbits;
  int32_t n_cg;
  const int32_t* pix_perm;
  const float* g_t;
  const float* breg_sr_px;
  const float* breg_sr_ch;
  int32_t h_rule;
  float pg_gamma_w;
  double* pg_q;
  const int32_t* ell_fill_px;
  float* ell_fill_num;
  int32_t ell_fill_n;
  int32_t tail_mode;
  int32_t no_fused;
  int32_t ell_pb;
  int32_t ell_stream;
  int32_t ell_hv_n;
  int32_t ell_hv_npx;
  int32_t ell_hv_ngrp;
  const int32_t* ell_hv_px;
  const int32_t* ell_hv_px_off;
  const int32_t* ell_hv_pm;
  const float* ell_hv_klc;
  double* ell_hv_kl;
  const int32_t* ell_hv_grp;
  const int32_t* ell_hv_grp_off;
  const int32_t* ell_hv_wm;
} espm_mu_state;

const char* espm_mu_version(void);
const char* espm_mu_last_error(void);
size_t espm_mu_state_size(void);
int espm_mu_abi_version(void);
const char* espm_mu_state_layout(void);

int espm_mu_query(espm_mu_state* st);

int espm_mu_pack_x(const void* src, int src_dtype, int src_layout, int64_t ld, int n, int p,
                   void* x_cm, void* x_pm, int x_dtype, int n_pad, int p_pad, int x_tile, int n_cm,
                   espm_stream_t stream);

int espm_mu_ell_count(const espm_mu_state* st, const void* x_pm_u8, int32_t* cnt_px, int32_t* cnt_bc, float* ell_klc,
                      espm_stream_t stream);
int espm_mu_ell_count_hist(const espm_mu_state* st, const void* x_pm_u8, int32_t* cnt_px, int32_t* cnt_bc, float* ell_klc, uint8_t* bkt_px,
                           uint8_t* bkt_bc, espm_stream_t stream);
int espm_mu_ell_fill_hist(const espm_mu_state* st, const void* x_pm_u8, const int32_t* chan_perm, const int32_t* pix_perm,
                          const int32_t* ell_h_off, const int32_t* ell_w_off, uint32_t* ell_h, uint32_t* ell_w, const uint8_t* bkt_px,
                          const uint8_t* bkt_bc, espm_stream_t stream);
int espm_mu_ell_plan(const espm_mu_state* st, const int32_t* cnt_px, const int32_t* cnt_bc, int32_t* chan_perm,
                     int32_t* pix_perm, int32_t* ell_h_off, int32_t* ell_w_off, int64_t* rows, espm_stream_t stream);
int espm_mu_ell_fill(const espm_mu_state* st, const void* x_pm_u8, const int32_t* chan_perm, const int32_t* pix_perm,
                     const int32_t* ell_h_off, const int32_t* ell_w_off, uint32_t* ell_h, uint32_t* ell_w,
                     espm_stream_t stream);
int espm_mu_ell_heavy_count(const espm_mu_state* st, const void* x, int src_dtype, int src_layout, int64_t ld, uint8_t* x_pm_u8,
                            uint8_t* x_cm_u8, int32_t* cnt_px, espm_stream_t stream);
int espm_mu_ell_heavy_fill(const espm_mu_state* st, const void* x, int src_dtype, int src_layout, int64_t ld, const int32_t* px_off,
                           int32_t* hv_pm, espm_stream_t stream);

int espm_mu_hstat(const espm_mu_state* st, int which, espm_stream_t stream);

int espm_mu_build_gw(const espm_mu_state* st, int which, espm_stream_t stream);

int espm_mu_step_h(const espm_mu_state* st, int src, int write_h, espm_stream_t stream);

int espm_mu_h_finalize(const espm_mu_state* st, int src, int slot, espm_stream_t stream);

int espm_mu_loss_only(const espm_mu_state* st, int src, int slot, espm_stream_t stream);

int espm_mu_w_accum(const espm_mu_state* st, espm_stream_t stream);
int espm_mu_step_hw(const espm_mu_state* st, int src, espm_stream_t stream);
int espm_mu_fused_applies(const espm_mu_state* st);
int espm_mu_w_reduce(const espm_mu_state* st, espm_stream_t stream);
int espm_mu_w_reduce_finalize(const espm_mu_state* st, int src, int slot, espm_stream_t stream);
int espm_mu_w_finish(const espm_mu_state* st, int src, int hsrc, int slot, espm_stream_t stream);

int espm_mu_w_reduce_finish(const espm_mu_state* st, int src, int slot, int with_finalize, espm_stream_t stream);

int espm_mu_iterate(espm_mu_state* st, int n_iter, int final_loss, espm_stream_t stream);
int espm_mu_w_update_is_local(const espm_mu_state* st);
int espm_mu_w_update_tail(const espm_mu_state* st, int src, int slot, espm_stream_t stream);

size_t espm_mu_shard_record_bytes(const espm_mu_state* st);
int espm_mu_shard_pack(const espm_mu_state* st, int hnew, void* record, espm_stream_t stream);
int espm_mu_w_reduce_pack(const espm_mu_state* st, int src, int slot, void* record, espm_stream_t stream);
int espm_mu_shard_combine(const espm_mu_state* st, const void* records, int world, int hnew,
                          espm_stream_t stream);
int espm_mu_shard_combine_finish(const espm_mu_state* st, const void* records, int world, int src, int slot,
                                 espm_stream_t stream);

typedef struct espm_xchg espm_xchg;
#define ESPM_XCHG_HANDLE_BYTES 64
int espm_xchg_create(int world, int rank, size_t record_bytes, espm_xchg** out);
int espm_xchg_handle(const espm_xchg* x, void* handle_out );
int espm_xchg_connect(espm_xchg* x, const void* handles );
void* espm_xchg_staging(const espm_xchg* x);
const void* espm_xchg_records(const espm_xchg* x, int parity);
int espm_xchg_post(espm_xchg* x, uint32_t seq, espm_stream_t stream);
int espm_xchg_wait(espm_xchg* x, uint32_t seq, espm_stream_t stream);
int espm_xchg_timeouts(const espm_xchg* x, uint32_t* count_out);
int espm_xchg_set_order(espm_xchg* x, int release);
int espm_xchg_order(const espm_xchg* x);
int espm_xchg_destroy(espm_xchg* x);

int espm_mu_shard_exchange_finish(const espm_mu_state* st, espm_xchg* x, uint32_t seq, int src, int slot, espm_stream_t stream);

int espm_mu_iterate_timed(espm_mu_state* st, int n_iter, float* first_ms, float* rest_ms, espm_stream_t stream);

int espm_mu_iterate_sharded(espm_mu_state* st, espm_xchg* x, uint32_t* seq, int n_iter, int final_loss, espm_stream_t stream);

int espm_dichotomy_simplex(const double* num, const double* den, int k, int p, int den_cols,
                           double log_shift, double tol, int maxit, double* nu_out,
                           int32_t* status_out, espm_stream_t stream);

int espm_simplex_root_f32(const float* num, const float* den, int k, int p, float log_shift, float tol, int maxit, int fast_exit,
                          float* delta_out, float* e_out, int32_t* status_out, espm_stream_t stream);

int espm_dichotomy_simplex_acc(double a, const double* b, const double* minus_c, int k, int p, int b_cols, double log_shift,
                               double tol, int maxit, double* nu_out, int32_t* status_out, espm_stream_t stream);
int espm_dichotomy_simplex_pg(const double* a, int k, int p, double log_shift, double tol, int maxit, double* nu_out,
                              espm_stream_t stream);

int espm_mu_l2_step_h(const espm_mu_state* st, int src, float* work, double* scratch, int scratch_doubles, espm_stream_t stream);
int espm_mu_l2_step_w(const espm_mu_state* st, int src, const float* gtg, float* work, double* scratch, int scratch_doubles,
                      espm_stream_t stream);
int espm_mu_l2_w_partials(const espm_mu_state* st, float* work, double* scratch, int scratch_doubles, espm_stream_t stream);
int espm_mu_l2_w_finish(const espm_mu_state* st, int src, const float* gtg, const float* work, espm_stream_t stream);

int espm_mu_linesearch_terms(const espm_mu_state* st, int hold, int hnew, double* out, espm_stream_t stream);

int espm_mu_linesearch_terms_sharded(const espm_mu_state* st, int hold, int hnew, const float* old_halo_top, const float* old_halo_bot,
                                     double* out, espm_stream_t stream);

int espm_surrogate_terms(const float* h_old, const float* h_new, int k, int p, int64_t ld, int nx, int ny, int grid_mode, double* part,
                         int part_doubles, double* out, espm_stream_t stream);

int espm_mu_laplacian(const float* h, int k, int nx, int ny, int64_t ld, float* out,
                      espm_stream_t stream);

size_t espm_lu_pl_scratch_bytes(int m, int r, int dtype);
int espm_lu_pl(const void* a, int dtype, int m, int r, int64_t ld, void* out, void* scratch, size_t scratch_bytes, espm_stream_t stream);

#define ESPM_F64_MAX_K 8
#define ESPM_F64_BLOCK 256
#define ESPM_F64_CHUNK 2048
#define ESPM_F64_WCHUNK 4096
#define ESPM_F64_MAXIT 127
#define ESPM_F64_X_U8 0
#define ESPM_F64_X_BF16 1
#define ESPM_F64_X_F32 2
#define ESPM_F64_X_F64 3

int64_t espm_f64_scratch_doubles(int n, int p, int k, int64_t count);
int espm_f64_gw(const double* g, const double* w, int n, int m, int k, double log_shift, double* gw, double* colsum, int32_t* small,
                espm_stream_t stream);
int espm_f64_hstat(const double* h, int k, int p, double log_shift, double* scratch, double* out, espm_stream_t stream);
int espm_f64_h_pass(const void* x, int x_type, int n, int p, double xscale, const double* gw, const double* colsum_gw,
                    const int32_t* gw_small, const double* h, int k, const double* hstat, const double* mu, double eps_reg,
                    double lambda_L, double sigma, int nx, int ny, double log_shift, int mode, const double* fixed_h, double* h_out,
                    double* num, double* den, double* scratch, double* hist_row, espm_stream_t stream);
int espm_f64_bisect(const double* num, const double* den, int k, int p, double log_shift, double tol, int maxit,
                    const double* fixed_h, double* h_out, uint64_t* mask, int32_t* status, espm_stream_t stream);
int espm_f64_rel(const double* a, const double* b, int64_t count, double tol, double* scratch, double* out, espm_stream_t stream);
int espm_f64_w_accum(const void* x, int x_type, int n, int p, double xscale, const double* gw, const double* h, int k, double log_shift,
                     double* scratch, double* rh, espm_stream_t stream);
int espm_f64_w_finish(const double* rh, const double* g, const double* colsum_g, int n, int m, int k, const double* w,
                      const double* hstat, int simplex, const uint8_t* rows, int nrows, double log_shift, double tol, int maxit,
                      const double* fixed_w, double* w_out, int32_t* status, espm_stream_t stream);

#define ESPM_F64S_MAX_COUNT 65535
#define ESPM_F64S_MAX_N 65536
#define ESPM_F64S_HBLOCK 512
#define ESPM_F64S_WBLOCK 65536
#define ESPM_F64S_LDS_BYTES 163840

int64_t espm_f64_sparse_scratch_doubles(int n, int p, int k);
int espm_f64_sparse_h_pass(const uint32_t* h_elem, const int64_t* h_off, const int32_t* ec, int n_ec, const uint8_t* ep_flag, int n, int p,
                           double xscale, const double* gw, const double* colsum_gw, const int32_t* gw_small, const double* h, int k,
                           const double* hstat, const double* mu, double eps_reg, double lambda_L, double sigma, int nx, int ny,
                           double log_shift, int mode, const double* fixed_h, double* h_out, double* num, double* den, double* scratch,
                           double* hist_row, espm_stream_t stream);
int espm_f64_sparse_w_accum(const uint32_t* w_elem, const int64_t* w_off, const uint8_t* ec_flag, const int32_t* ep, const int32_t* ep_off,
                            int n, int p, double xscale, const double* gw, const double* h, int k, double log_shift, double* scratch,
                            double* rh, espm_stream_t stream);

#ifdef __cplusplus
}
#endif
#endif
```

Baseline: 7613 it/s.

## Keep a prebuilt LDS table image of gw and widen the W reduce-update kernel

Adds a global buffer that stores the gw values already in the fused kernel's LDS table layout. The W update writes into it alongside gw_s, so each fused workgroup can copy the image straight into LDS with float4 loads instead of scattering rows through FixTab::put. Separately adds a wider W reduce-update kernel that reads partial sums as float4 over more columns per block, and makes it the default. Both are selectable through environment variables. The cost is extra global writes in the W update and some added register pressure in the fused kernel's staging phase.

```diff
diff --git a/espm_amd/_lib.py b/espm_amd/_lib.py
--- a/espm_amd/_lib.py
+++ b/espm_amd/_lib.py
@@ -67,6 +67,8 @@
     "espm_mu_ell_heavy_fill": (C.c_int, [_SP, _vp, C.c_int, C.c_int, _i64, _vp, _vp, _vp]),
     "espm_mu_hstat": (C.c_int, [_SP, C.c_int, _vp]),
     "espm_mu_build_gw": (C.c_int, [_SP, C.c_int, _vp]),
+    "espm_mu_gw_tab_bytes": (C.c_size_t, [C.c_int, C.c_int]),
+    "espm_mu_build_gw_tab": (C.c_int, [_SP, _vp]),
     "espm_mu_step_h": (C.c_int, [_SP, C.c_int, C.c_int, _vp]),
     "espm_mu_h_finalize": (C.c_int, [_SP, C.c_int, C.c_int, _vp]),
     "espm_mu_loss_only": (C.c_int, [_SP, C.c_int, C.c_int, _vp]),
diff --git a/espm_amd/csrc/mu_api.hip b/espm_amd/csrc/mu_api.hip
--- a/espm_amd/csrc/mu_api.hip
+++ b/espm_amd/csrc/mu_api.hip
@@ -33,7 +33,7 @@
   F(ell_h_off) F(ell_klc) F(ell_w) F(ell_w_off) F(chan_perm) F(ell_cbits) F(n_cg) F(pix_perm) F(g_t) F(breg_sr_px) \
   F(breg_sr_ch) F(h_rule) F(pg_gamma_w) F(pg_q) F(ell_fill_px) F(ell_fill_num) F(ell_fill_n) F(tail_mode) F(no_fused) \
   F(ell_pb) F(ell_stream) F(ell_hv_n) F(ell_hv_npx) F(ell_hv_ngrp) F(ell_hv_px) F(ell_hv_px_off) F(ell_hv_pm) F(ell_hv_klc) F(ell_hv_kl) \
-  F(ell_hv_grp) F(ell_hv_grp_off) F(ell_hv_wm)
+  F(ell_hv_grp) F(ell_hv_grp_off) F(ell_hv_wm) F(gw_tab)
 
 static int check_abi(const espm_mu_state* st) {
   ESPM_REQUIRE(st != nullptr, "state is NULL");
@@ -107,6 +107,9 @@
   return launch_ell_hv_post(st, st->h_t, 1, ESPM_KP, w, loss, s);
 }
 
+#ifndef ESPM_FUSED_TAB_IMAGE_DEFAULT
+#define ESPM_FUSED_TAB_IMAGE_DEFAULT 1
+#endif
 static bool fused_ok(const espm_mu_state* st) {
   return ESPM_MIN_K <= 8 && st->x_dtype == ESPM_X_ELL && st->h_rule == 0 && st->no_fused != 1 &&
          (st->ell_pb >= ESPM_FUSED_MIN_PB || st->nblk_w >= ESPM_FUSED_MIN_BLOCKS || st->no_fused == 3) &&
@@ -305,6 +308,7 @@
   a.pg_gamma_w = st->pg_gamma_w;
   a.pg_q = (st->pg_q && st->pg_gamma_w > 0.f && slot >= 0) ? st->pg_q + 2 * (size_t)slot + 1 : nullptr;
   a.gw_s = st->gw_s;
+  a.gw_tab = (st->gw_tab && gw_tab_bytes(st->n_pad, st->k) > 0) ? st->gw_tab : nullptr;
   a.colsum_gw = st->colsum_gw;
   a.gw_a = nullptr;
   a.gw_p = nullptr;
@@ -338,6 +342,14 @@
   return launch_w_finish(finish_args(st, which, 0, -1, 0), static_cast<hipStream_t>(stream));
 }
 
+size_t espm_mu_gw_tab_bytes(int n_pad, int k) { return gw_tab_bytes(n_pad, k); }
+
+int espm_mu_build_gw_tab(const espm_mu_state* st, espm_stream_t stream) {
+  if (int rc = check_state(st)) return rc;
+  ESPM_REQUIRE(st->gw_tab, "build_gw_tab: the state has no gw_tab");
+  return launch_gw_tab_build(st->gw_s, st->gw_tab, st->n_pad, st->k, static_cast<hipStream_t>(stream));
+}
+
 int espm_mu_step_h(const espm_mu_state* st, int src, int write_h, espm_stream_t stream) {
   if (int rc = check_state(st)) return rc;
   ESPM_REQUIRE(src == 0 || src == 1, "src must be 0/1");
@@ -540,11 +552,17 @@
   const bool fused = fused_ok(st);
   bool pending = false;
   WTailArgs tail;
+  static const bool tab_env = [] { const char* e = getenv("ESPM_FUSED_TAB_IMAGE"); return e ? e[0] != '0' : ESPM_FUSED_TAB_IMAGE_DEFAULT != 0; }();
+  const bool tab_kept = defer && !split && n_iter > 0 && st->gw_tab && gw_tab_bytes(st->n_pad, st->k) > 0;
+  const bool tab_img = tab_kept && tab_env && fused;
+  if (tab_kept)
+    if (int rc = launch_gw_tab_build(st->gw_s, st->gw_tab, st->n_pad, st->k, s)) return rc;
   for (int i = 0; i < n_iter; ++i) {
     const int cur = st->cur, slot = st->it;
     int rc;
     if (defer) {
       HStepArgs a = fused ? fused_h_args(st, cur) : make_h_args(st, cur, 1);
+      if (tab_img) a.gw_tab = st->gw_tab;
       if ((rc = ell_pre_h(st, cur, s))) return rc;
       if (pending) {
         a.cs_parts = tail.parts;
diff --git a/espm_amd/csrc/mu_common.hpp b/espm_amd/csrc/mu_common.hpp
--- a/espm_amd/csrc/mu_common.hpp
+++ b/espm_amd/csrc/mu_common.hpp
@@ -567,6 +567,7 @@
   const void* x_pm;
   int mfma;
   const float* gw_s;
+  const float* gw_tab;
   const double* colsum_gw;
   const float* h_in;
   float* h_out;
@@ -647,6 +648,7 @@
   float pg_gamma_w;
   double* pg_q;
   float* gw_s;
+  float* gw_tab;
   double* colsum_gw;
   void* gw_a;
   float* gw_p;
@@ -770,6 +772,7 @@
   a.x_pm = st->x_pm;
   a.mfma = st->no_fused == 0;
   a.gw_s = st->gw_s;
+  a.gw_tab = nullptr;
   a.colsum_gw = st->colsum_gw;
   a.h_in = st->h[src];
   a.h_out = st->h[1 - src];
@@ -881,6 +884,10 @@
                            const double* hpart, int nblk_h, const double* hstat_rs, size_t rec_hstat_off, double* hstat_out,
                            const HFinalizeArgs* fused_finalize, hipStream_t stream, WTailArgs* defer_tail = nullptr);
 int launch_w_update_tail(const WTailArgs& t, hipStream_t stream);
+size_t gw_tab_bytes(int n_pad, int k);
+int launch_gw_tab_build(const float* gw_s, float* gw_tab, int n_pad, int k, hipStream_t stream);
+struct GwTabGeom { int lo, hi, hi_stride; };
+GwTabGeom gw_tab_geom(int n_pad, int k);
 int launch_w_exchange_update(const WFinishArgs& f, const void* slabs, size_t slab_stride, int nslab, float* a_out, double* hstat_out,
                              const HFinalizeArgs& fin, const struct ::espm_xchg* xc, unsigned int seq, const float* h_new, int nx, int ny,
                              int p_pad, int with_halo, hipStream_t stream, WTailArgs* defer_tail, double* simplex_bparts = nullptr);
diff --git a/espm_amd/csrc/mu_fused.hip b/espm_amd/csrc/mu_fused.hip
--- a/espm_amd/csrc/mu_fused.hip
+++ b/espm_amd/csrc/mu_fused.hip
@@ -184,6 +184,56 @@
          (pb != ESPM_ELL_PB ? (size_t)(pb + 64 * n_cg) * sizeof(int) : 0);
 }
 
+#if ESPM_MIN_K <= 8
+template <int K>
+__global__ __launch_bounds__(256) void gw_tab_build_kernel(const float* __restrict__ gw_s, float* __restrict__ tab, int n_pad) {
+  const int r = blockIdx.x * 256 + threadIdx.x;
+  if (r < n_pad) FixTab<K>::put_row(tab, n_pad, r, gw_s + (size_t)r * KP);
+}
+#endif
+
+size_t gw_tab_bytes(int n_pad, int k) {
+  if (n_pad < 1 || n_pad % 4 != 0) return 0;
+  switch (k) {
+#if ESPM_MIN_K <= 8
+#define ESPM_X(KK) case KK: return n_pad <= FixTab<KK>::MAX_ROWS ? FixTab<KK>::bytes(n_pad) : 0;
+    ESPM_K_CASES(ESPM_X)
+#undef ESPM_X
+#endif
+  }
+  return 0;
+}
+
+GwTabGeom gw_tab_geom(int n_pad, int k) {
+  GwTabGeom g = {0, 0, 0};
+  switch (k) {
+#if ESPM_MIN_K <= 8
+#define ESPM_X(KK)                                                                                   \
+  case KK:                                                                                           \
+    if (FixTab<KK>::TWO && FixTab<KK>::FIXED) g = GwTabGeom{0, ESPM_TAB2_BASE / 4, 4};                \
+    else g = GwTabGeom{LdsTabGeom<KK>::WB * n_pad, 0, LdsTabGeom<KK>::WB >= 4 ? 4 : LdsTabGeom<KK>::WB}; \
+    break;
+    ESPM_K_CASES(ESPM_X)
+#undef ESPM_X
+#endif
+  }
+  return g;
+}
+
+int launch_gw_tab_build(const float* gw_s, float* gw_tab, int n_pad, int k, hipStream_t stream) {
+  const size_t bytes = gw_tab_bytes(n_pad, k);
+  ESPM_REQUIRE(gw_s && gw_tab && bytes > 0, "table image: no table of %d rows for k=%d", n_pad, k);
+  if (int rc = check_hip(hipMemsetAsync(gw_tab, 0, bytes, stream), "table image: clear")) return rc;
+  switch (k) {
+#if ESPM_MIN_K <= 8
+#define ESPM_X(KK) case KK: hipLaunchKernelGGL(gw_tab_build_kernel<KK>, dim3((n_pad + 255) / 256), dim3(256), 0, stream, gw_s, gw_tab, n_pad); break;
+    ESPM_K_CASES(ESPM_X)
+#undef ESPM_X
+#endif
+  }
+  return check_hip(hipGetLastError(), "table image launch");
+}
+
 int launch_fused_ell(const HStepArgs& h, const WAccumArgs& w, int nblk, hipStream_t stream, int static_units, int stream_lists) {
   ESPM_REQUIRE(h.ell && h.ell_off && h.ell_klc && h.ell_pix && w.ell && w.ell_off && w.chan_perm, "fused half-steps: the sparse store's lists are missing");
   ESPM_REQUIRE(w.pb >= 128 && w.pb <= ESPM_ELL_PB && (w.pb & (w.pb - 1)) == 0 && 2 * h.ell_tp == w.pb && h.h_rule == 0 && h.write_h && !h.l2_m,
diff --git a/espm_amd/csrc/mu_fused_kernel.hpp b/espm_amd/csrc/mu_fused_kernel.hpp
--- a/espm_amd/csrc/mu_fused_kernel.hpp
+++ b/espm_amd/csrc/mu_fused_kernel.hpp
@@ -155,13 +155,28 @@
     const int n_perm = perm_lds ? PB + 64 * fa.w.n_cg : 0, n_woff = 2 * fa.w.n_cg + 1;
     staged = PLAIN || (a.n_pad <= TR * NT && n_perm <= PC * NT && n_woff <= NT && a.cs_nbk <= 64 && 2 * K <= NT / 64);
     if (staged) {
-      float4 tlo[TR], thi[TR];
-#pragma unroll
-      for (int i = 0; i < TR; ++i) {
-        const int r = threadIdx.x + i * NT;
-        const float* src = a.gw_s + (size_t)min(r, a.n_pad - 1) * KP;
-        tlo[i] = *reinterpret_cast<const float4*>(src);
-        thi[i] = K > 4 ? *reinterpret_cast<const float4*>(src + 4) : make_float4(0.f, 0.f, 0.f, 0.f);
+      constexpr bool TAB2 = FixTab<K>::TWO && FixTab<K>::FIXED;
+      constexpr int NCH = TAB2 ? 2 * TR : 4 + LdsTabGeom<K>::WB;
+      const bool tab_img = PLAIN && a.gw_tab != nullptr;
+      const int n_chunk = TAB2 ? 2 * a.n_pad : (4 + LdsTabGeom<K>::WB) * (a.n_pad / 4);
+      float4 tlo[TR], thi[TR], tch[PLAIN ? NCH : 1];
+      if (tab_img) {
+        if constexpr (PLAIN) {
+#pragma unroll
+          for (int i = 0; i < NCH; ++i) {
+            const int j = threadIdx.x + i * NT;
+            const int jc = TAB2 && j >= a.n_pad ? ESPM_TAB2_BASE / 16 + (j - a.n_pad) : j;
+            tch[i] = j < n_chunk ? reinterpret_cast<const float4*>(a.gw_tab)[jc] : make_float4(0.f, 0.f, 0.f, 0.f);
+          }
+        }
+      } else {
+#pragma unroll
+        for (int i = 0; i < TR; ++i) {
+          const int r = threadIdx.x + i * NT;
+          const float* src = a.gw_s + (size_t)min(r, a.n_pad - 1) * KP;
+          tlo[i] = *reinterpret_cast<const float4*>(src);
+          thi[i] = K > 4 ? *reinterpret_cast<const float4*>(src + 4) : make_float4(0.f, 0.f, 0.f, 0.f);
+        }
       }
       int pv[PC];
 #pragma unroll
@@ -190,10 +205,21 @@
           rwo[u] = i < rw_hi ? a.tail.w_old[i] : 1.f;
         }
       }
-#pragma unroll
-      for (int i = 0; i < TR; ++i) {
-        const int r = threadIdx.x + i * NT;
-        if (r < a.n_pad) FixTab<K>::put(tab, a.n_pad, r, tlo[i], thi[i]);
+      if (tab_img) {
+        if constexpr (PLAIN) {
+#pragma unroll
+          for (int i = 0; i < NCH; ++i) {
+            const int j = threadIdx.x + i * NT;
+            const int jc = TAB2 && j >= a.n_pad ? ESPM_TAB2_BASE / 16 + (j - a.n_pad) : j;
+            if (j < n_chunk) reinterpret_cast<float4*>(tab)[jc] = tch[i];
+          }
+        }
+      } else {
+#pragma unroll
+        for (int i = 0; i < TR; ++i) {
+          const int r = threadIdx.x + i * NT;
+          if (r < a.n_pad) FixTab<K>::put(tab, a.n_pad, r, tlo[i], thi[i]);
+        }
       }
 #pragma unroll
       for (int i = 0; i < PC; ++i) {
diff --git a/espm_amd/csrc/mu_w_step.hip b/espm_amd/csrc/mu_w_step.hip
--- a/espm_amd/csrc/mu_w_step.hip
+++ b/espm_amd/csrc/mu_w_step.hip
@@ -1,11 +1,15 @@
 #include <atomic>
 #include <stdio.h>
+#include <stdint.h>
 #include <stdlib.h>
 
 #include "mu_w_kernel.hpp"
 #include "mu_w_mfma_kernel.hpp"
 #include "mu_xchg.hpp"
 
+#ifndef ESPM_W_REDUCE_WIDE_DEFAULT
+#define ESPM_W_REDUCE_WIDE_DEFAULT 2
+#endif
 #ifndef ESPM_MFMA_MIN_K
 #define ESPM_MFMA_MIN_K 9
 #endif
@@ -110,6 +114,8 @@
   float pg_gamma_w;
   int pg_track;
   float* gw_s;
+  float* gw_tab = nullptr;
+  int tab_lo = 0, tab_hi = 0, tab_hi_stride = 0;
   double* parts;
   float log_shift, gw_floor, xscale;
   int fuse_finalize;
@@ -124,11 +130,12 @@
     if (a.fixed_w) fx = a.fixed_w[(size_t)c * a.k + kk];
   }
 }
-__device__ __forceinline__ void w_update_entries(const WUpdateArgs& a, int kk, int c, int e, bool owns, float t, double rs, int nwg, int wg,
-                                                 float wo_pre, float fx_pre) {
-  double cs = 0.0, sw = 0.0, qw = 0.0;
+__device__ __forceinline__ void w_update_one(const WUpdateArgs& a, int kk, int c, int e, bool owns, float t, double rs, float wo_pre, float fx_pre,
+                                             double& cs, double& sw, double& qw) {
+  cs = 0.0; sw = 0.0; qw = 0.0;
   if (owns) {
     a.a_out[e] = t;
+    float* tabp = a.gw_tab ? a.gw_tab + ((kk < 4 ? a.tab_lo + 4 * c : a.tab_hi + a.tab_hi_stride * c) + (kk & 3)) : nullptr;
     if (c < a.n) {
       const float wo = wo_pre;
       float v;
@@ -145,13 +152,21 @@
       if (fx_pre >= 0.f) v = fx_pre;
       a.w_new[(size_t)c * a.k + kk] = v;
       const float gv = fmaxf(v, a.gw_floor);
-      a.gw_s[(size_t)c * KP + kk] = gv * (1.f / a.xscale);
+      const float gs = gv * (1.f / a.xscale);
+      a.gw_s[(size_t)c * KP + kk] = gs;
+      if (tabp) *tabp = gs;
       cs = (double)gv;
       sw = (double)v;
     } else {
       a.gw_s[(size_t)c * KP + kk] = 1.f;
-    }
-  }
+      if (tabp) *tabp = 1.f;
+    }
+  }
+}
+__device__ __forceinline__ void w_update_entries(const WUpdateArgs& a, int kk, int c, int e, bool owns, float t, double rs, int nwg, int wg,
+                                                 float wo_pre, float fx_pre) {
+  double cs, sw, qw;
+  w_update_one(a, kk, c, e, owns, t, rs, wo_pre, fx_pre, cs, sw, qw);
   cs = wave_sum(cs);
   sw = wave_sum(sw);
   if (a.pg_track) qw = wave_sum(qw);
@@ -235,6 +250,102 @@
       for (int g = 0; g < 8; ++g) t += s_part[g][col];
     }
     w_update_entries(a, kk, c, e, owns, t, rs, nwg, blockIdx.x, wo_pre, fx_pre);
+  }
+}
+
+template <int SPLIT>
+__global__ __launch_bounds__(256) void w_reduce_update_wide_kernel(const WUpdateArgs a) {
+  constexpr int QPW = 32 / SPLIT, EPW = 4 * QPW, NACC = 8 / SPLIT;
+  __shared__ double fscratch[5 * (ESPM_HP_NSCALAR + 2 * KP + 1)];
+  __shared__ __attribute__((aligned(16))) float s_part[8 * SPLIT][EPW];
+  __shared__ double s_rsw[4];
+  const int nbq = (a.n_pad + EPW - 1) / EPW, nwg = a.k * nbq;
+  if ((int)blockIdx.x >= nwg) {
+    h_finalize_one(a.fin, (int)blockIdx.x - nwg, fscratch);
+    return;
+  }
+  const int kk = blockIdx.x / nbq, j = blockIdx.x - kk * nbq;
+  const int q = threadIdx.x % QPW, r = threadIdx.x / QPW, grp = r & 7, half = r >> 3;
+  const int c0 = EPW * j + 4 * q;
+  const bool live = c0 < a.n_pad;
+  const size_t e0 = (size_t)kk * a.n_pad + c0;
+  auto src = [&](int b) { return *reinterpret_cast<const float4*>(a.src + (size_t)b * a.src_stride + 4 * e0); };
+  const float4 zero4 = make_float4(0.f, 0.f, 0.f, 0.f);
+  const int b0 = grp + 8 * NACC * half;
+  float4 v[NACC][4];
+#pragma unroll
+  for (int i = 0; i < NACC; ++i)
+#pragma unroll
+    for (int m = 0; m < 4; ++m) {
+      const int b = b0 + 8 * i + 64 * m;
+      v[i][m] = (live && b < a.nsrc) ? src(b) : zero4;
+    }
+  const int c = EPW * j + (int)threadIdx.x;
+  const bool updates = (int)threadIdx.x < EPW;
+  float wo_pre, fx_pre;
+  w_update_preload(a, kk, c, updates, wo_pre, fx_pre);
+  double rsp = 0.0;
+  {
+    const size_t nb = a.nblk_h;
+    for (int b = threadIdx.x; b < a.nblk_h; b += 256) rsp += a.hpart[(ESPM_HP_ROWSUM + kk) * nb + b];
+  }
+  float4 acc[NACC];
+#pragma unroll
+  for (int i = 0; i < NACC; ++i) {
+    acc[i].x = ((v[i][0].x + v[i][1].x) + v[i][2].x) + v[i][3].x;
+    acc[i].y = ((v[i][0].y + v[i][1].y) + v[i][2].y) + v[i][3].y;
+    acc[i].z = ((v[i][0].z + v[i][1].z) + v[i][2].z) + v[i][3].z;
+    acc[i].w = ((v[i][0].w + v[i][1].w) + v[i][2].w) + v[i][3].w;
+  }
+  if (live) {
+    for (int m = 4; b0 + 64 * m < a.nsrc; ++m) {
+#pragma unroll
+      for (int i = 0; i < NACC; ++i) {
+        const int b = b0 + 8 * i + 64 * m;
+        if (b < a.nsrc) {
+          const float4 x = src(b);
+          acc[i].x += x.x; acc[i].y += x.y; acc[i].z += x.z; acc[i].w += x.w;
+        }
+      }
+    }
+  }
+  float4 p;
+  if constexpr (SPLIT == 1) {
+    p.x = ((acc[0].x + acc[1].x) + (acc[2].x + acc[3].x)) + ((acc[4].x + acc[5].x) + (acc[6].x + acc[7].x));
+    p.y = ((acc[0].y + acc[1].y) + (acc[2].y + acc[3].y)) + ((acc[4].y + acc[5].y) + (acc[6].y + acc[7].y));
+    p.z = ((acc[0].z + acc[1].z) + (acc[2].z + acc[3].z)) + ((acc[4].z + acc[5].z) + (acc[6].z + acc[7].z));
+    p.w = ((acc[0].w + acc[1].w) + (acc[2].w + acc[3].w)) + ((acc[4].w + acc[5].w) + (acc[6].w + acc[7].w));
+  } else {
+    p.x = (acc[0].x + acc[1].x) + (acc[2].x + acc[3].x);
+    p.y = (acc[0].y + acc[1].y) + (acc[2].y + acc[3].y);
+    p.z = (acc[0].z + acc[1].z) + (acc[2].z + acc[3].z);
+    p.w = (acc[0].w + acc[1].w) + (acc[2].w + acc[3].w);
+  }
+  *reinterpret_cast<float4*>(&s_part[r][4 * q]) = p;
+  rsp = wave_sum(rsp);
+  if ((threadIdx.x & 63) == 0) s_rsw[threadIdx.x >> 6] = rsp;
+  __syncthreads();
+  if (!updates) return;
+  const double rs = ((s_rsw[0] + s_rsw[1]) + s_rsw[2]) + s_rsw[3];
+  const bool owns = c < a.n_pad;
+  float t = 0.f;
+#pragma unroll
+  for (int g = 0; g < 8; ++g) {
+    if constexpr (SPLIT == 1) t += s_part[g][threadIdx.x];
+    else t += s_part[g][threadIdx.x] + s_part[8 + g][threadIdx.x];
+  }
+  double cs, sw, qw;
+  w_update_one(a, kk, c, (int)e0 - 4 * q + (int)threadIdx.x, owns, t, rs, wo_pre, fx_pre, cs, sw, qw);
+#pragma unroll
+  for (int off = 1; off <= 16; off <<= 1) {
+    cs += __shfl_xor(cs, off, 64);
+    sw += __shfl_xor(sw, off, 64);
+  }
+  const int j32 = c >> 5;
+  if ((threadIdx.x & 31) == 0 && j32 < a.nbk) {
+    const int nwg32 = a.k * a.nbk;
+    a.parts[kk * a.nbk + j32] = cs;
+    a.parts[nwg32 + kk * a.nbk + j32] = sw;
   }
 }
 
@@ -1406,7 +1517,22 @@
   a.xscale = f.xscale;
   a.fuse_finalize = fused_finalize != nullptr;
   if (fused_finalize) a.fin = *fused_finalize;
-  hipLaunchKernelGGL(w_reduce_update_kernel, dim3(a.k * a.nbk + (fused_finalize ? H_FINALIZE_JOBS : 0)), dim3(256), 0, stream, a);
+  if (f.gw_tab) {
+    const GwTabGeom tg = gw_tab_geom(f.n_pad, f.k);
+    a.gw_tab = f.gw_tab;
+    a.tab_lo = tg.lo;
+    a.tab_hi = tg.hi;
+    a.tab_hi_stride = tg.hi_stride;
+  }
+  static const int wide_env = [] { const char* e = getenv("ESPM_W_REDUCE_WIDE"); return e ? atoi(e) : ESPM_W_REDUCE_WIDE_DEFAULT; }();
+  const bool wide = wide_env > 0 && hpart && fused_finalize && !(f.pg_gamma_w > 0.f) && !f.breg_sr && f.n_pad % 4 == 0 && src_stride % 16 == 0 &&
+                    reinterpret_cast<uintptr_t>(src) % 16 == 0;
+  if (wide && wide_env == 1)
+    hipLaunchKernelGGL(w_reduce_update_wide_kernel<1>, dim3(a.k * ((a.n_pad + 127) / 128) + H_FINALIZE_JOBS), dim3(256), 0, stream, a);
+  else if (wide)
+    hipLaunchKernelGGL(w_reduce_update_wide_kernel<2>, dim3(a.k * ((a.n_pad + 63) / 64) + H_FINALIZE_JOBS), dim3(256), 0, stream, a);
+  else
+    hipLaunchKernelGGL(w_reduce_update_kernel, dim3(a.k * a.nbk + (fused_finalize ? H_FINALIZE_JOBS : 0)), dim3(256), 0, stream, a);
   const WTailArgs t = make_w_tail_args(f);
   if (defer_tail)
     *defer_tail = t;
diff --git a/espm_amd/engine.py b/espm_amd/engine.py
--- a/espm_amd/engine.py
+++ b/espm_amd/engine.py
@@ -354,6 +354,8 @@
         self.h = [torch.ones((k, st.p_pad), **f32) for _ in range(2)]
         self.h_t = torch.zeros((self.p, self.V.KP), **f32)
         self.gw_s = torch.zeros((st.n_pad, self.V.KP), **f32)
+        tab_bytes = int(self.lib.espm_mu_gw_tab_bytes(st.n_pad, k)) if self.ell is not None else 0
+        self.gw_tab = torch.zeros(tab_bytes // 4, **f32) if tab_bytes else None
         self.colsum_gw = torch.zeros(self.V.KP, **f64)
         nblk_h = (self.p + st.tile_px - 1) // st.tile_px
         self.hpart = torch.zeros((nblk_h, self.V.HP_STRIDE), **f64)
@@ -407,6 +409,7 @@
         st.h[0], st.h[1] = self.h[0].data_ptr(), self.h[1].data_ptr()
         st.gw_s, st.colsum_gw, st.h_t = self.gw_s.data_ptr(), self.colsum_gw.data_ptr(), self.h_t.data_ptr()
         st.gw_a, st.gw_p = None, None
+        st.gw_tab = self.gw_tab.data_ptr() if self.gw_tab is not None else None
         st.mu = self.mu.data_ptr() if self.mu is not None else None
         st.fixed_h = self.fixed_h.data_ptr() if self.fixed_h is not None else None
         st.fixed_w = self.fixed_w.data_ptr() if self.fixed_w is not None else None
diff --git a/include/espm_mu.h b/include/espm_mu.h
--- a/include/espm_mu.h
+++ b/include/espm_mu.h
@@ -80,7 +80,7 @@
 #define ESPM_HI_REL_H 6
 #define ESPM_HI_STRIDE 8
 
-#define ESPM_MU_ABI_VERSION 5
+#define ESPM_MU_ABI_VERSION 6
 
 typedef struct espm_mu_state {
   uint32_t struct_size;
@@ -164,6 +164,7 @@
   const int32_t* ell_hv_grp;
   const int32_t* ell_hv_grp_off;
   const int32_t* ell_hv_wm;
+  float* gw_tab;
 } espm_mu_state;
 
 const char* espm_mu_version(void);
@@ -198,6 +199,8 @@
 int espm_mu_hstat(const espm_mu_state* st, int which, espm_stream_t stream);
 
 int espm_mu_build_gw(const espm_mu_state* st, int which, espm_stream_t stream);
+size_t espm_mu_gw_tab_bytes(int n_pad, int k);
+int espm_mu_build_gw_tab(const espm_mu_state* st, espm_stream_t stream);
 
 int espm_mu_step_h(const espm_mu_state* st, int src, int write_h, espm_stream_t stream);
 
```

After: 7619 it/s (median of 2 runs). About the same (+0.1%).
